# chaitjo/efficient-gnns

Measured on NVIDIA H100. Metric: edges aggregated/s (fwd+bwd), 3-layer GCN student + logit-KD, ARXIV-shape, higher is better.
Workload: dtype f32

## Files before the change

efficient-gnns_b200/csrc/common.cuh:

```cuda
#pragma once
#include <cuda_runtime.h>
#include <stdint.h>

#include "b200gnn.h"

namespace b200gnn {

void set_cuda_error(cudaError_t e);
void count_launch(int n = 1);

inline int check_launch() {
  cudaError_t e = cudaGetLastError();
  if (e != cudaSuccess) {
    set_cuda_error(e);
    return B200GNN_ERR_CUDA;
  }
  count_launch();
  return B200GNN_OK;
}

constexpr unsigned FULL_MASK = 0xffffffffu;

__device__ __forceinline__ void adam_update(float& p, float& m, float& v, float g, float b1, float b2, float eps,
                                            float step_size, float inv_sqrt_bc2) {
  const float mi = b1 * m + (1.f - b1) * g;
  const float vi = b2 * v + (1.f - b2) * g * g;
  m = mi; v = vi;
  p -= step_size * mi / (sqrtf(vi) * inv_sqrt_bc2 + eps);
}

template <typename V> struct VecTraits;
template <> struct VecTraits<float> { static constexpr int W = 1; };
template <> struct VecTraits<float2> { static constexpr int W = 2; };
template <> struct VecTraits<float4> { static constexpr int W = 4; };

__device__ __forceinline__ void vzero(float& a) { a = 0.f; }
__device__ __forceinline__ void vzero(float2& a) { a.x = a.y = 0.f; }
__device__ __forceinline__ void vzero(float4& a) { a.x = a.y = a.z = a.w = 0.f; }

__device__ __forceinline__ void vfma(float& acc, float s, const float& x) { acc = fmaf(s, x, acc); }
__device__ __forceinline__ void vfma(float2& acc, float s, const float2& x) {
  acc.x = fmaf(s, x.x, acc.x); acc.y = fmaf(s, x.y, acc.y);
}
__device__ __forceinline__ void vfma(float4& acc, float s, const float4& x) {
  acc.x = fmaf(s, x.x, acc.x); acc.y = fmaf(s, x.y, acc.y);
  acc.z = fmaf(s, x.z, acc.z); acc.w = fmaf(s, x.w, acc.w);
}
__device__ __forceinline__ void vadd(float& a, const float& b) { a += b; }
__device__ __forceinline__ void vadd(float2& a, const float2& b) { a.x += b.x; a.y += b.y; }
__device__ __forceinline__ void vadd(float4& a, const float4& b) {
  a.x += b.x; a.y += b.y; a.z += b.z; a.w += b.w;
}
__device__ __forceinline__ void vdiv(float& a, float d) { a /= d; }
__device__ __forceinline__ void vdiv(float2& a, float d) { a.x /= d; a.y /= d; }
__device__ __forceinline__ void vdiv(float4& a, float d) { a.x /= d; a.y /= d; a.z /= d; a.w /= d; }
__device__ __forceinline__ void vstat(float& s, float& q, const float& y) { s += y; q = fmaf(y, y, q); }
__device__ __forceinline__ void vstat(float2& s, float2& q, const float2& y) {
  s.x += y.x; s.y += y.y; q.x = fmaf(y.x, y.x, q.x); q.y = fmaf(y.y, y.y, q.y);
}
__device__ __forceinline__ void vstat(float4& s, float4& q, const float4& y) {
  s.x += y.x; s.y += y.y; s.z += y.z; s.w += y.w;
  q.x = fmaf(y.x, y.x, q.x); q.y = fmaf(y.y, y.y, q.y);
  q.z = fmaf(y.z, y.z, q.z); q.w = fmaf(y.w, y.w, q.w);
}

__device__ __forceinline__ float vshfl_down(float v, int d) { return __shfl_down_sync(FULL_MASK, v, d); }
__device__ __forceinline__ float2 vshfl_down(float2 v, int d) {
  return make_float2(__shfl_down_sync(FULL_MASK, v.x, d), __shfl_down_sync(FULL_MASK, v.y, d));
}
__device__ __forceinline__ float4 vshfl_down(float4 v, int d) {
  return make_float4(__shfl_down_sync(FULL_MASK, v.x, d), __shfl_down_sync(FULL_MASK, v.y, d),
                     __shfl_down_sync(FULL_MASK, v.z, d), __shfl_down_sync(FULL_MASK, v.w, d));
}

__device__ __forceinline__ float vldg(const float* p) { return __ldg(p); }
__device__ __forceinline__ float2 vldg(const float2* p) { return __ldg(p); }
__device__ __forceinline__ float4 vldg(const float4* p) { return __ldg(p); }

__device__ __forceinline__ void vstcs(float* p, const float& v) { __stcs(p, v); }
__device__ __forceinline__ void vstcs(float2* p, const float2& v) { __stcs(p, v); }
__device__ __forceinline__ void vstcs(float4* p, const float4& v) { __stcs(p, v); }

static __global__ void __launch_bounds__(256) sum_partials_kernel(const float* __restrict__ partial, int n, double scale,
                                                                  float* __restrict__ out) {
  __shared__ double s[256];
  double a = 0.0;
  for (int i = threadIdx.x; i < n; i += 256) a += (double)partial[i];
  s[threadIdx.x] = a;
  __syncthreads();
  for (int d = 128; d > 0; d >>= 1) {
    if (threadIdx.x < d) s[threadIdx.x] += s[threadIdx.x + d];
    __syncthreads();
  }
  if (threadIdx.x == 0) out[0] = (float)(s[0] * scale);
}

inline bool aligned_to(const void* p, size_t a) { return (reinterpret_cast<uintptr_t>(p) % a) == 0; }

}
```

efficient-gnns_b200/csrc/dense_rows.cu:

```cuda
#include "common.cuh"
#include "philox.cuh"

namespace b200gnn {

constexpr int ROWS_THREADS = 256;

struct RowMap {
  int nvec, rows_per_iter, cv, rg;
  bool active;
};
__device__ __forceinline__ RowMap make_row_map(int K) {
  RowMap m;
  m.nvec = K >> 2;
  m.rows_per_iter = ROWS_THREADS / m.nvec;
  m.rg = threadIdx.x / m.nvec;
  m.cv = threadIdx.x - m.rg * m.nvec;
  m.active = m.rg < m.rows_per_iter;
  return m;
}

__device__ __forceinline__ float4 ld4(const float* p) { return *reinterpret_cast<const float4*>(p); }
__device__ __forceinline__ float4 ld4s(const float* p) { return __ldcs(reinterpret_cast<const float4*>(p)); }
__device__ __forceinline__ void st4(float* p, const float4& v) { *reinterpret_cast<float4*>(p) = v; }

// ... 61 lines not shown
    const double mean = s / (double)n;
    double var = q / (double)n - mean * mean;
    if (var < 0.0) var = 0.0;
    const float invstd = (float)(1.0 / sqrt(var + (double)eps));
    const float sc = gamma[k] * invstd;
    mean_out[k] = (float)mean;
    invstd_out[k] = invstd;
    scale_out[k] = sc;
    shift_out[k] = beta[k] - (float)mean * sc;
    if (running_mean) {
      const double unbiased = n > 1 ? var * (double)n / (double)(n - 1) : var;
      running_mean[k] = (1.f - momentum) * running_mean[k] + momentum * (float)mean;
      running_var[k] = (1.f - momentum) * running_var[k] + momentum * (float)unbiased;
    }
  }
}

__device__ __forceinline__ float4 affine_relu4(float4 y, const float* __restrict__ scale, const float* __restrict__ shift,
                                               int cv, int relu) {
  if (scale) {
    const float4 sc = ld4(scale + 4 * cv), sh = ld4(shift + 4 * cv);
    y.x = fmaf(y.x, sc.x, sh.x); y.y = fmaf(y.y, sc.y, sh.y);
    y.z = fmaf(y.z, sc.z, sh.z); y.w = fmaf(y.w, sc.w, sh.w);
  }
  if (relu) { y.x = fmaxf(y.x, 0.f); y.y = fmaxf(y.y, 0.f); y.z = fmaxf(y.z, 0.f); y.w = fmaxf(y.w, 0.f); }
  return y;
}

template <bool P16>
__global__ void __launch_bounds__(256) affine_relu_dropout_kernel(const float* __restrict__ Y, float* __restrict__ out,
                                                                  int64_t n_vec, int nvec_row,
                                                                  const float* __restrict__ scale,
                                                                  const float* __restrict__ shift, int relu, float p,
                                                                  uint32_t thr16, uint64_t seed, uint64_t offset,
                                                                  const int32_t* __restrict__ step_dev,
                                                                  uint64_t step_mul, uint64_t index_offset) {
  const float inv_keep = p > 0.f ? 1.f / (1.f - p) : 1.f;
  if (step_dev) offset += (uint64_t)(*step_dev) * step_mul;
  const int64_t tid = (int64_t)blockIdx.x * blockDim.x + threadIdx.x, stride = (int64_t)gridDim.x * blockDim.x;
  if (P16) {
    const uint64_t g0 = index_offset, g1 = index_offset + (uint64_t)n_vec;
    for (uint64_t b = (g0 >> 1) + (uint64_t)tid; b < ((g1 + 1) >> 1); b += (uint64_t)stride) {
      const uint4 r = philox4x32(seed, offset, b);
#pragma unroll
      for (int half = 0; half < 2; ++half) {
        const uint64_t g = 2 * b + half;
        if (g < g0 || g >= g1) continue;
        const int64_t i = (int64_t)(g - g0);
        float4 y = affine_relu4(ld4s(Y + 4 * i), scale, shift, (int)(i % nvec_row), relu);
        const uchar4 m = keep16(half ? r.z : r.x, half ? r.w : r.y, thr16);
        y.x = m.x ? y.x * inv_keep : 0.f; y.y = m.y ? y.y * inv_keep : 0.f;
        y.z = m.z ? y.z * inv_keep : 0.f; y.w = m.w ? y.w * inv_keep : 0.f;
        st4(out + 4 * i, y);
      }
    }
  } else {
    for (int64_t i = tid; i < n_vec; i += stride) {
      float4 y = affine_relu4(ld4s(Y + 4 * i), scale, shift, (int)(i % nvec_row), relu);
      if (p > 0.f) {
        const uchar4 m = keep24(philox4x32(seed, offset, (uint64_t)i + index_offset), p);
        y.x = m.x ? y.x * inv_keep : 0.f; y.y = m.y ? y.y * inv_keep : 0.f;
        y.z = m.z ? y.z * inv_keep : 0.f; y.w = m.w ? y.w * inv_keep : 0.f;
      }
      st4(out + 4 * i, y);
    }
  }
}

struct RowScatter {
  float* ptr[16];
  int32_t off[17];
  int32_t n;
  int64_t ld, col;
};
__device__ __forceinline__ float* scatter_row(const RowScatter& sc, int64_t r) {
  int q = 0;
#pragma unroll 1
  while (q + 1 < sc.n && r >= sc.off[q + 1]) ++q;
  return sc.ptr[q] + (size_t)(r - sc.off[q]) * (size_t)sc.ld + sc.col;
}

template <bool P16>
__global__ void __launch_bounds__(256) affine_relu_dropout_mapped_kernel(
    const float* __restrict__ Y, float* __restrict__ out, int64_t n_rows, int nvec_l, const float* __restrict__ scale,
    const float* __restrict__ shift, int relu, float p, uint32_t thr16, uint64_t seed, uint64_t offset,
    const int32_t* __restrict__ step_dev, uint64_t step_mul, const int32_t* __restrict__ rowmap, uint64_t row_offset,
    uint64_t nvec_g, uint64_t cv_off, int paired, const RowScatter sc) {
  const float inv_keep = p > 0.f ? 1.f / (1.f - p) : 1.f;
  if (step_dev) offset += (uint64_t)(*step_dev) * step_mul;
  const int64_t tid = (int64_t)blockIdx.x * blockDim.x + threadIdx.x, stride = (int64_t)gridDim.x * blockDim.x;
  if (P16 && paired) {
    const int half_l = nvec_l >> 1;
    for (int64_t u = tid; u < n_rows * half_l; u += stride) {
      const int64_t r = u / half_l;
      const int cv = (int)(u - r * half_l) * 2;
      const uint64_t gid = rowmap ? (uint64_t)rowmap[r] : (uint64_t)r + row_offset;
      const uint64_t g = gid * nvec_g + cv_off + (uint64_t)cv;
      const uint4 rnd = philox4x32(seed, offset, g >> 1);
#pragma unroll
      for (int half = 0; half < 2; ++half) {
        const int64_t i = r * nvec_l + cv + half;
        float4 y = affine_relu4(ld4s(Y + 4 * i), scale, shift, cv + half, relu);
        const uchar4 m = keep16(half ? rnd.z : rnd.x, half ? rnd.w : rnd.y, thr16);
        y.x = m.x ? y.x * inv_keep : 0.f; y.y = m.y ? y.y * inv_keep : 0.f;
        y.z = m.z ? y.z * inv_keep : 0.f; y.w = m.w ? y.w * inv_keep : 0.f;
        st4(out + 4 * i, y);
        if (sc.n) st4(scatter_row(sc, r) + 4 * (cv + half), y);
      }
    }
    return;
  }
  for (int64_t i = tid; i < n_rows * nvec_l; i += stride) {
    const int64_t r = i / nvec_l;
    const int cv = (int)(i - r * nvec_l);
    float4 y = affine_relu4(ld4s(Y + 4 * i), scale, shift, cv, relu);
    if (p > 0.f) {
      const uint64_t gid = rowmap ? (uint64_t)rowmap[r] : (uint64_t)r + row_offset;
      const uint64_t g = gid * nvec_g + cv_off + (uint64_t)cv;
      uchar4 m;
      if (P16) {
        const uint4 rnd = philox4x32(seed, offset, g >> 1);
        m = keep16((g & 1) ? rnd.z : rnd.x, (g & 1) ? rnd.w : rnd.y, thr16);
      } else {
        m = keep24(philox4x32(seed, offset, g), p);
      }
      y.x = m.x ? y.x * inv_keep : 0.f; y.y = m.y ? y.y * inv_keep : 0.f;
      y.z = m.z ? y.z * inv_keep : 0.f; y.w = m.w ? y.w * inv_keep : 0.f;
    }
    st4(out + 4 * i, y);
    if (sc.n) st4(scatter_row(sc, r) + 4 * cv, y);
  }
}

__global__ void __launch_bounds__(256) dropout_mask_kernel(uint8_t* __restrict__ mask, int64_t n_vec, float p, int p16,
                                                           uint32_t thr16, uint64_t seed, uint64_t offset) {
  for (int64_t i = (int64_t)blockIdx.x * blockDim.x + threadIdx.x; i < n_vec; i += (int64_t)gridDim.x * blockDim.x) {
    uchar4 m;
    if (p16) {
      const uint4 r = philox4x32(seed, offset, (uint64_t)i >> 1);
      m = keep16((i & 1) ? r.z : r.x, (i & 1) ? r.w : r.y, thr16);
    } else {
      m = keep24(philox4x32(seed, offset, (uint64_t)i), p);
    }
    reinterpret_cast<uchar4*>(mask)[i] = m;
  }
}

__global__ void __launch_bounds__(256) dropout_mask_step_kernel(uint8_t* __restrict__ mask, int64_t n_vec, float p, int p16,
                                                                uint32_t thr16, uint64_t seed, uint64_t offset,
                                                                const int32_t* __restrict__ step_dev, uint64_t step_mul) {
  const uint64_t off = offset + (uint64_t)(*step_dev) * step_mul;
  for (int64_t i = (int64_t)blockIdx.x * blockDim.x + threadIdx.x; i < n_vec; i += (int64_t)gridDim.x * blockDim.x) {
    uchar4 m;
    if (p16) {
      const uint4 r = philox4x32(seed, off, (uint64_t)i >> 1);
      m = keep16((i & 1) ? r.z : r.x, (i & 1) ? r.w : r.y, thr16);
    } else {
      m = keep24(philox4x32(seed, off, (uint64_t)i), p);
    }
    reinterpret_cast<uchar4*>(mask)[i] = m;
  }
}

__global__ void __launch_bounds__(256) dropout_bits_kernel(uint32_t* __restrict__ bits, int n_layers, int64_t n_rows, int nvec_row,
                                                           int words, float p, int p16, uint32_t thr16, uint64_t seed,
                                                           uint64_t offset, const int32_t* __restrict__ step_dev,
                                                           uint64_t step_mul) {
  if (step_dev) offset += (uint64_t)(*step_dev) * step_mul;
  const int64_t per_layer = n_rows * words;
  for (int64_t t = (int64_t)blockIdx.x * blockDim.x + threadIdx.x; t < per_layer * n_layers; t += (int64_t)gridDim.x * blockDim.x) {
    const int layer = (int)(t / per_layer);
    const int64_t e = t - layer * per_layer, row = e / words;
    const int w = (int)(e - row * words);
    const uint64_t off = offset + (uint64_t)layer;
    uint32_t out = 0u;
    uint64_t blk = ~0ull;
    uint4 r = make_uint4(0u, 0u, 0u, 0u);
#pragma unroll
    for (int j = 0; j < 8; ++j) {
      const int cv = 8 * w + j;
      if (cv >= nvec_row) break;
      const uint64_t g = (uint64_t)row * nvec_row + cv;
      uchar4 m;
      if (p16) {
        if ((g >> 1) != blk) { blk = g >> 1; r = philox4x32(seed, off, blk); }
        m = keep16((g & 1) ? r.z : r.x, (g & 1) ? r.w : r.y, thr16);
      } else {
        m = keep24(philox4x32(seed, off, g), p);
      }
      out |= ((uint32_t)m.x | ((uint32_t)m.y << 1) | ((uint32_t)m.z << 2) | ((uint32_t)m.w << 3)) << (4 * j);
    }
    bits[t] = out;
  }
}

__global__ void __launch_bounds__(256) affine_relu_bits_kernel(const float* __restrict__ Y, const uint32_t* __restrict__ bits,
                                                               const float* __restrict__ scale, const float* __restrict__ shift,
                                                               float* __restrict__ out, int64_t n_vec, int nvec_row, int words,
                                                               float p) {
  const float inv_keep = p > 0.f ? 1.f / (1.f - p) : 1.f;
  for (int64_t i = (int64_t)blockIdx.x * blockDim.x + threadIdx.x; i < n_vec; i += (int64_t)gridDim.x * blockDim.x) {
    const int64_t row = i / nvec_row;
    const int cv = (int)(i - row * nvec_row);
    float4 y = affine_relu4(ld4(Y + 4 * i), scale, shift, cv, 1);
    const uint32_t b = bits[row * words + (cv >> 3)] >> (4 * (cv & 7));
    y.x = (b & 1u) ? y.x * inv_keep : 0.f; y.y = (b & 2u) ? y.y * inv_keep : 0.f;
    y.z = (b & 4u) ? y.z * inv_keep : 0.f; y.w = (b & 8u) ? y.w * inv_keep : 0.f;
    st4(out + 4 * i, y);
  }
}

__global__ void __launch_bounds__(256) gather_rows_act_kernel(const float* __restrict__ X, int64_t ldx, const int64_t* __restrict__ idx,
                                                              const uint32_t* __restrict__ bits, const float* __restrict__ scale,
                                                              const float* __restrict__ shift, float* __restrict__ out,
                                                              int64_t n_vec, int nvec_row, int words, float p) {
  const float inv_keep = p > 0.f ? 1.f / (1.f - p) : 1.f;
  for (int64_t i = (int64_t)blockIdx.x * blockDim.x + threadIdx.x; i < n_vec; i += (int64_t)gridDim.x * blockDim.x) {
    const int64_t r = i / nvec_row;
    const int cv = (int)(i - r * nvec_row);
    const int64_t row = __ldg(idx + r);
    float4 y = ld4(X + row * ldx + 4 * cv);
    if (bits) {
      y = affine_relu4(y, scale, shift, cv, 1);
      const uint32_t b = bits[row * words + (cv >> 3)] >> (4 * (cv & 7));
      y.x = (b & 1u) ? y.x * inv_keep : 0.f; y.y = (b & 2u) ? y.y * inv_keep : 0.f;
      y.z = (b & 4u) ? y.z * inv_keep : 0.f; y.w = (b & 8u) ? y.w * inv_keep : 0.f;
    }
    st4(out + 4 * i, y);
  }
}

__global__ void __launch_bounds__(256) relu_dropout_bwd_kernel(const float4* __restrict__ dOut, const float4* __restrict__ Xout,
                                                               float4* dY, int64_t n_vec, float inv_keep) {
  for (int64_t i = (int64_t)blockIdx.x * blockDim.x + threadIdx.x; i < n_vec; i += (int64_t)gridDim.x * blockDim.x) {
    const float4 g = dOut[i], x = Xout[i];
    float4 d;
    d.x = x.x > 0.f ? g.x * inv_keep : 0.f; d.y = x.y > 0.f ? g.y * inv_keep : 0.f;
    d.z = x.z > 0.f ? g.z * inv_keep : 0.f; d.w = x.w > 0.f ? g.w * inv_keep : 0.f;
    dY[i] = d;
  }
}

__global__ void __launch_bounds__(ROWS_THREADS) bn_act_bwd_reduce_kernel(
    const float* __restrict__ dOut, const float* __restrict__ Xout, const float* __restrict__ Y,
    const float* __restrict__ mean, const float* __restrict__ invstd, int64_t n_rows, int K, float inv_keep,
    float* __restrict__ partial, int slots) {
  extern __shared__ float smem[];
  const RowMap m = make_row_map(K);
  const int64_t per = (n_rows + slots - 1) / slots;
  const int64_t r0 = (int64_t)blockIdx.x * per, r1 = min(n_rows, r0 + per);
  float4 s = make_float4(0, 0, 0, 0), q = s;
  if (m.active) {
    const float4 mu = ld4(mean + 4 * m.cv), is = ld4(invstd + 4 * m.cv);
    for (int64_t r = r0 + m.rg; r < r1; r += m.rows_per_iter) {
      const size_t o = (size_t)r * K + 4 * m.cv;
      const float4 g = ld4(dOut + o), x = ld4(Xout + o), y = ld4(Y + o);
      const float dx = x.x > 0.f ? g.x * inv_keep : 0.f, dy = x.y > 0.f ? g.y * inv_keep : 0.f;
      const float dz = x.z > 0.f ? g.z * inv_keep : 0.f, dw = x.w > 0.f ? g.w * inv_keep : 0.f;
      s.x += dx; s.y += dy; s.z += dz; s.w += dw;
      q.x = fmaf(dx, (y.x - mu.x) * is.x, q.x); q.y = fmaf(dy, (y.y - mu.y) * is.y, q.y);
      q.z = fmaf(dz, (y.z - mu.z) * is.z, q.z); q.w = fmaf(dw, (y.w - mu.w) * is.w, q.w);
    }
  }
  reduce_store_2xK(m, K, s, q, smem, partial + (size_t)blockIdx.x * 2 * K);
}

__global__ void __launch_bounds__(256) bn_bwd_finalize_kernel(const float* __restrict__ partial, int slots, int K,
                                                              int64_t n, const float* __restrict__ gamma,
                                                              const float* __restrict__ invstd, float* dgamma,
                                                              float* dbeta, float* coef ) {
  double s, q; int k;
  if (finalize_reduce(partial, slots, K, true, s, q, k)) {
    dbeta[k] = (float)s;
    dgamma[k] = (float)q;
    coef[k] = gamma[k] * invstd[k];
    coef[K + k] = (float)(s / (double)n);
    coef[2 * K + k] = (float)(q / (double)n);
  }
}

template <bool DZ>
__global__ void __launch_bounds__(ROWS_THREADS) bn_act_bwd_apply_kernel(
    const float* __restrict__ dOut, const float* __restrict__ Xout, const float* __restrict__ Y,
    const float* __restrict__ mean, const float* __restrict__ invstd, const float* __restrict__ coef, int64_t n_rows,
    int K, float inv_keep, float* __restrict__ dY, float* __restrict__ colsum_partial, int slots) {
  extern __shared__ float smem[];
  const RowMap m = make_row_map(K);
  const int64_t per = (n_rows + slots - 1) / slots;
  const int64_t r0 = (int64_t)blockIdx.x * per, r1 = min(n_rows, r0 + per);
  float4 s = make_float4(0, 0, 0, 0), q = s;
  if (m.active) {
    const float4 mu = ld4(mean + 4 * m.cv), is = ld4(invstd + 4 * m.cv);
    const float4 c1 = ld4(coef + 4 * m.cv), c2 = ld4(coef + K + 4 * m.cv), c3 = ld4(coef + 2 * K + 4 * m.cv);
    for (int64_t r = r0 + m.rg; r < r1; r += m.rows_per_iter) {
      const size_t o = (size_t)r * K + 4 * m.cv;
      float4 g = ld4s(dOut + o);
      const float4 y = ld4s(Y + o);
      if (!DZ) {
        const float4 x = ld4s(Xout + o);
        g.x = x.x > 0.f ? g.x * inv_keep : 0.f; g.y = x.y > 0.f ? g.y * inv_keep : 0.f;
        g.z = x.z > 0.f ? g.z * inv_keep : 0.f; g.w = x.w > 0.f ? g.w * inv_keep : 0.f;
      }
      float4 d;
      d.x = c1.x * (g.x - c2.x - (y.x - mu.x) * is.x * c3.x);
      d.y = c1.y * (g.y - c2.y - (y.y - mu.y) * is.y * c3.y);
      d.z = c1.z * (g.z - c2.z - (y.z - mu.z) * is.z * c3.z);
      d.w = c1.w * (g.w - c2.w - (y.w - mu.w) * is.w * c3.w);
      st4(dY + o, d);
      s.x += d.x; s.y += d.y; s.z += d.z; s.w += d.w;
    }
  }
  if (colsum_partial) reduce_store_2xK(m, K, s, q, smem, colsum_partial + (size_t)blockIdx.x * 2 * K);
}

__global__ void __launch_bounds__(256) partial_reduce_kernel(const float* __restrict__ partial, int slots, int K2,
                                                             float* __restrict__ out) {
  __shared__ double sh[FIN_GROUPS][FIN_COLS];
  const int c = threadIdx.x % FIN_COLS, g = threadIdx.x / FIN_COLS;
  const int k = blockIdx.x * FIN_COLS + c;
  double s = 0.0;
  if (k < K2)
    for (int j = g; j < slots; j += FIN_GROUPS) s += (double)partial[(size_t)j * K2 + k];
  sh[g][c] = s;
  __syncthreads();
  if (g == 0 && k < K2) {
    s = 0.0;
    for (int j = 0; j < FIN_GROUPS; ++j) s += sh[j][c];
    out[k] = (float)s;
  }
}

__global__ void __launch_bounds__(256) colsum_finalize_kernel(const float* __restrict__ partial, int slots, int K,
                                                              float* __restrict__ out) {
  double s, q; int k;
  if (finalize_reduce(partial, slots, K, false, s, q, k)) out[k] = (float)s;
}

__global__ void __launch_bounds__(256) adam_kernel(float* __restrict__ p, const float* __restrict__ g,
                                                   float* __restrict__ m, float* __restrict__ v, int64_t n, float lr,
                                                   float b1, float b2, float eps, const int32_t* __restrict__ step) {
  const float t = (float)(*step + 1);
  const float bc1 = 1.f - powf(b1, t), bc2 = 1.f - powf(b2, t);
  const float step_size = lr / bc1, inv_sqrt_bc2 = rsqrtf(bc2);
  for (int64_t i = (int64_t)blockIdx.x * blockDim.x + threadIdx.x; i < n; i += (int64_t)gridDim.x * blockDim.x)
    adam_update(p[i], m[i], v[i], g[i], b1, b2, eps, step_size, inv_sqrt_bc2);
}
__global__ void adam_tick_kernel(int32_t* step) { *step += 1; }

__global__ void __launch_bounds__(256) rmsprop_kernel(float* __restrict__ p, const float* __restrict__ g, float* __restrict__ sq,
                                                      int64_t n, double lr, int warmup, float alpha, float one_minus_alpha,
                                                      float eps, float wd, const int32_t* __restrict__ step) {
  const int e = *step + 1;
  const float neg_lr = -(float)(warmup > 0 ? lr * (double)(e < warmup ? e : warmup) / (double)warmup : lr);
  for (int64_t i = (int64_t)blockIdx.x * blockDim.x + threadIdx.x; i < n; i += (int64_t)gridDim.x * blockDim.x) {
    const float pi = p[i];
    float gi = g[i];
    if (wd != 0.f) gi = __fadd_rn(gi, __fmul_rn(wd, pi));
    const float s = __fadd_rn(__fmul_rn(sq[i], alpha), __fmul_rn(__fmul_rn(one_minus_alpha, gi), gi));
    sq[i] = s;
    p[i] = __fadd_rn(pi, __fdiv_rn(__fmul_rn(neg_lr, gi), __fadd_rn(__fsqrt_rn(s), eps)));
  }
}

static inline int grid_for(int64_t n_items, int per_cta, int cap = 132 * 8) {
  int64_t g = (n_items + per_cta - 1) / per_cta;
  if (g > cap) g = cap;
  if (g < 1) g = 1;
  return (int)g;
}

}

using namespace b200gnn;

static bool rows_ok(int64_t n_rows, int64_t K) { return n_rows >= 0 && K > 0 && K % 4 == 0 && K <= 1024; }

extern "C" int64_t b200gnn_rows_slots(int64_t n_rows) {
  int64_t s = (n_rows + 255) / 256;
  if (s > 132 * 4) s = 132 * 4;
  return s < 1 ? 1 : s;
}

extern "C" int b200gnn_col_stats_f32(const float* Y, int64_t n_rows, int64_t K, float* partial, int64_t slots,
                                     void* stream) {
  if (!rows_ok(n_rows, K) || !Y || !partial || slots < 1 || !aligned_to(Y, 16)) return B200GNN_ERR_BAD_ARG;
  col_stats4_kernel<<<(int)slots, ROWS_THREADS, 2 * K * sizeof(float), (cudaStream_t)stream>>>(Y, n_rows, (int)K, partial,
                                                                                             (int)slots);
  return check_launch();
}

extern "C" int b200gnn_bn_finalize_f32(const float* partial, int64_t slots, int64_t K, int64_t n_rows,
                                       const float* gamma, const float* beta, float eps, float momentum,
                                       float* running_mean, float* running_var, float* mean_out, float* invstd_out,
                                       float* scale_out, float* shift_out, void* stream) {
  if (!partial || slots < 1 || K <= 0 || n_rows <= 0 || !gamma || !beta || !mean_out || !invstd_out || !scale_out ||
      !shift_out || ((running_mean == nullptr) != (running_var == nullptr)))
    return B200GNN_ERR_BAD_ARG;
  bn_finalize_kernel<<<(int)((K + FIN_COLS - 1) / FIN_COLS), 256, 0, (cudaStream_t)stream>>>(
      partial, (int)slots, (int)K, n_rows, gamma, beta, eps, momentum, running_mean, running_var, mean_out, invstd_out,
      scale_out, shift_out);
  return check_launch();
}

extern "C" int b200gnn_affine_relu_dropout_f32(const float* Y, float* out, int64_t n_rows, int64_t K,
                                               const float* scale, const float* shift, int relu, float p, uint64_t seed,
                                               uint64_t offset, const int32_t* step_dev, uint64_t step_mul,
                                               uint64_t row_offset, void* stream) {
  if (!rows_ok(n_rows, K) || !Y || !out || p < 0.f || p >= 1.f || ((scale == nullptr) != (shift == nullptr)) ||
      !aligned_to(Y, 16) || !aligned_to(out, 16))
    return B200GNN_ERR_BAD_ARG;
  if (n_rows == 0) return B200GNN_OK;
  const int64_t n_vec = n_rows * (K / 4);
  uint32_t thr16 = 0;
  if (dropout_p16(p, thr16))
    affine_relu_dropout_kernel<true><<<grid_for((n_vec + 1) / 2 + 1, 256 * 2), 256, 0, (cudaStream_t)stream>>>(
        Y, out, n_vec, (int)(K / 4), scale, shift, relu, p, thr16, seed, offset, step_dev, step_mul,
        row_offset * (uint64_t)(K / 4));
  else
    affine_relu_dropout_kernel<false><<<grid_for(n_vec, 256 * 4), 256, 0, (cudaStream_t)stream>>>(
        Y, out, n_vec, (int)(K / 4), scale, shift, relu, p, 0u, seed, offset, step_dev, step_mul,
        row_offset * (uint64_t)(K / 4));
  return check_launch();
}

static int mapped_launch(const float* Y, float* out, int64_t n_rows, int64_t K, const float* scale, const float* shift, int relu,
                         float p, uint64_t seed, uint64_t offset, const int32_t* step_dev, uint64_t step_mul, const int32_t* rowmap,
                         uint64_t row_offset, int64_t K_global, int64_t col_offset, const RowScatter& sc, void* stream) {
  if (!rows_ok(n_rows, K) || !Y || !out || p < 0.f || p >= 1.f || ((scale == nullptr) != (shift == nullptr)) ||
      !aligned_to(Y, 16) || !aligned_to(out, 16) || K_global < K || K_global % 4 || col_offset < 0 || col_offset % 4 ||
      col_offset + K > K_global)
    return B200GNN_ERR_BAD_ARG;
  if (n_rows == 0) return B200GNN_OK;
  const int nvec_l = (int)(K / 4);
  const uint64_t nvec_g = (uint64_t)(K_global / 4), cv_off = (uint64_t)(col_offset / 4);
  const int paired = (nvec_l % 2 == 0 && nvec_g % 2 == 0 && cv_off % 2 == 0) ? 1 : 0;
  const int64_t n_vec = n_rows * nvec_l;
  uint32_t thr16 = 0;
  if (dropout_p16(p, thr16))
    affine_relu_dropout_mapped_kernel<true><<<grid_for(paired ? n_vec / 2 : n_vec, 256 * 2), 256, 0, (cudaStream_t)stream>>>(
        Y, out, n_rows, nvec_l, scale, shift, relu, p, thr16, seed, offset, step_dev, step_mul, rowmap, row_offset, nvec_g,
        cv_off, paired, sc);
  else
    affine_relu_dropout_mapped_kernel<false><<<grid_for(n_vec, 256 * 4), 256, 0, (cudaStream_t)stream>>>(
        Y, out, n_rows, nvec_l, scale, shift, relu, p, 0u, seed, offset, step_dev, step_mul, rowmap, row_offset, nvec_g,
        cv_off, 0, sc);
  return check_launch();
}

extern "C" int b200gnn_affine_relu_dropout_mapped_f32(const float* Y, float* out, int64_t n_rows, int64_t K,
                                                      const float* scale, const float* shift, int relu, float p,
                                                      uint64_t seed, uint64_t offset, const int32_t* step_dev,
                                                      uint64_t step_mul, const int32_t* rowmap, uint64_t row_offset,
                                                      int64_t K_global, int64_t col_offset, void* stream) {
  RowScatter sc;
  sc.n = 0; sc.ld = 0; sc.col = 0;
  return mapped_launch(Y, out, n_rows, K, scale, shift, relu, p, seed, offset, step_dev, step_mul, rowmap, row_offset, K_global,
                       col_offset, sc, stream);
}

extern "C" int b200gnn_affine_relu_dropout_scatter_f32(const float* Y, float* out, int64_t n_rows, int64_t K,
                                                       const float* scale, const float* shift, int relu, float p,
                                                       uint64_t seed, uint64_t offset, const int32_t* step_dev,
                                                       uint64_t step_mul, const int32_t* rowmap, uint64_t row_offset,
                                                       int64_t K_global, int64_t col_offset, float* const* dst_ptrs,
                                                       const int32_t* row_off, int32_t world, int64_t ld_dst, void* stream) {
  if (!dst_ptrs || !row_off || world <= 0 || world > 16 || ld_dst < K_global || ld_dst % 4 || row_off[0] != 0 ||
      row_off[world] != n_rows)
    return B200GNN_ERR_BAD_ARG;
  RowScatter sc;
  sc.n = world; sc.ld = ld_dst; sc.col = col_offset;
  for (int q = 0; q < world; ++q) {
    if (!dst_ptrs[q] || !aligned_to(dst_ptrs[q], 16) || row_off[q + 1] < row_off[q]) return B200GNN_ERR_BAD_ARG;
    sc.ptr[q] = dst_ptrs[q]; sc.off[q] = row_off[q];
  }
  sc.off[world] = row_off[world];
  return mapped_launch(Y, out, n_rows, K, scale, shift, relu, p, seed, offset, step_dev, step_mul, rowmap, row_offset, K_global,
                       col_offset, sc, stream);
}

extern "C" int b200gnn_dropout_mask_u8(uint8_t* mask, int64_t n_rows, int64_t K, float p, uint64_t seed,
                                       uint64_t offset, void* stream) {
  if (!rows_ok(n_rows, K) || !mask || p < 0.f || p >= 1.f) return B200GNN_ERR_BAD_ARG;
  if (n_rows == 0) return B200GNN_OK;
  const int64_t n_vec = n_rows * (K / 4);
  uint32_t thr16 = 0;
  const int p16 = dropout_p16(p, thr16) ? 1 : 0;
  dropout_mask_kernel<<<grid_for(n_vec, 256 * 4), 256, 0, (cudaStream_t)stream>>>(mask, n_vec, p, p16, thr16, seed, offset);
  return check_launch();
}

extern "C" int b200gnn_dropout_mask_step_u8(uint8_t* mask, int64_t n_rows, int64_t K, float p, uint64_t seed, uint64_t offset,
                                            const int32_t* step_dev, uint64_t step_mul, void* stream) {
  if (!rows_ok(n_rows, K) || !mask || !step_dev || p < 0.f || p >= 1.f) return B200GNN_ERR_BAD_ARG;
  if (n_rows == 0) return B200GNN_OK;
  const int64_t n_vec = n_rows * (K / 4);
  uint32_t thr16 = 0;
  const int p16 = dropout_p16(p, thr16) ? 1 : 0;
  dropout_mask_step_kernel<<<grid_for(n_vec, 256 * 4), 256, 0, (cudaStream_t)stream>>>(mask, n_vec, p, p16, thr16, seed, offset,
                                                                                      step_dev, step_mul);
  return check_launch();
}

extern "C" int b200gnn_dropout_bits_u32(uint32_t* bits, int64_t n_layers, int64_t n_rows, int64_t K, float p, uint64_t seed,
                                        uint64_t offset, const int32_t* step_dev, uint64_t step_mul, void* stream) {
  if (!rows_ok(n_rows, K) || !bits || n_layers < 1 || p < 0.f || p >= 1.f) return B200GNN_ERR_BAD_ARG;
  if (n_rows == 0) return B200GNN_OK;
  const int words = (int)((K + 31) / 32);
  uint32_t thr16 = 0;
  const int p16 = dropout_p16(p, thr16) ? 1 : 0;
  dropout_bits_kernel<<<grid_for(n_layers * n_rows * words, 256 * 2), 256, 0, (cudaStream_t)stream>>>(
      bits, (int)n_layers, n_rows, (int)(K / 4), words, p, p16, thr16, seed, offset, step_dev, step_mul);
  return check_launch();
}

extern "C" int b200gnn_affine_relu_bits_f32(const float* Y, const uint32_t* bits, const float* scale, const float* shift,
                                            float p, float* out, int64_t n_rows, int64_t K, void* stream) {
  if (!rows_ok(n_rows, K) || !Y || !bits || !scale || !shift || !out || p < 0.f || p >= 1.f || !aligned_to(Y, 16) ||
      !aligned_to(out, 16) || !aligned_to(scale, 16) || !aligned_to(shift, 16))
    return B200GNN_ERR_BAD_ARG;
  if (n_rows == 0) return B200GNN_OK;
  const int64_t n_vec = n_rows * (K / 4);
  affine_relu_bits_kernel<<<grid_for(n_vec, 256 * 4), 256, 0, (cudaStream_t)stream>>>(Y, bits, scale, shift, out, n_vec,
                                                                                     (int)(K / 4), (int)((K + 31) / 32), p);
  return check_launch();
}

extern "C" int b200gnn_gather_rows_act_f32(const float* X, int64_t ldx, const int64_t* idx, int64_t n_idx, int64_t K,
                                            const uint32_t* bits, const float* scale, const float* shift, float p, float* out,
                                            void* stream) {
  if (!rows_ok(n_idx, K) || !X || !idx || !out || ldx < K || ldx % 4 || p < 0.f || p >= 1.f || !aligned_to(X, 16) ||
      !aligned_to(out, 16))
    return B200GNN_ERR_BAD_ARG;
  if (bits && (!scale || !shift || !aligned_to(scale, 16) || !aligned_to(shift, 16))) return B200GNN_ERR_BAD_ARG;
  if (n_idx == 0) return B200GNN_OK;
  const int64_t n_vec = n_idx * (K / 4);
  gather_rows_act_kernel<<<grid_for(n_vec, 256 * 4), 256, 0, (cudaStream_t)stream>>>(X, ldx, idx, bits, scale, shift, out, n_vec,
                                                                                    (int)(K / 4), (int)((K + 31) / 32), p);
  return check_launch();
}

extern "C" int b200gnn_relu_dropout_bwd_f32(const float* dOut, const float* Xout, float* dY, int64_t n_rows, int64_t K,
                                            float p, void* stream) {
  if (!rows_ok(n_rows, K) || p < 0.f || p >= 1.f) return B200GNN_ERR_BAD_ARG;
  if (n_rows == 0) return B200GNN_OK;
  if (!dOut || !Xout || !dY || !aligned_to(dOut, 16) || !aligned_to(Xout, 16) || !aligned_to(dY, 16)) return B200GNN_ERR_BAD_ARG;
  const int64_t n_vec = n_rows * (K / 4);
  const float inv_keep = p > 0.f ? 1.f / (1.f - p) : 1.f;
  relu_dropout_bwd_kernel<<<grid_for(n_vec, 256 * 4), 256, 0, (cudaStream_t)stream>>>(
      reinterpret_cast<const float4*>(dOut), reinterpret_cast<const float4*>(Xout), reinterpret_cast<float4*>(dY), n_vec, inv_keep);
  return check_launch();
}

extern "C" int b200gnn_bn_act_bwd_reduce_f32(const float* dOut, const float* Xout, const float* Y, const float* mean,
                                             const float* invstd, int64_t n_rows, int64_t K, float p, float* partial,
                                             int64_t slots, void* stream) {
  if (!rows_ok(n_rows, K) || n_rows == 0 || !dOut || !Xout || !Y || !mean || !invstd || !partial || slots < 1 ||
      p < 0.f || p >= 1.f)
    return B200GNN_ERR_BAD_ARG;
  if (!aligned_to(dOut, 16) || !aligned_to(Xout, 16) || !aligned_to(Y, 16) || !aligned_to(mean, 16) || !aligned_to(invstd, 16))
    return B200GNN_ERR_BAD_ARG;
  if (ROWS_THREADS / (K / 4) < 1) return B200GNN_ERR_UNSUPPORTED;
  const float inv_keep = p > 0.f ? 1.f / (1.f - p) : 1.f;
  bn_act_bwd_reduce_kernel<<<(int)slots, ROWS_THREADS, 2 * K * sizeof(float), (cudaStream_t)stream>>>(
      dOut, Xout, Y, mean, invstd, n_rows, (int)K, inv_keep, partial, (int)slots);
  return check_launch();
}

extern "C" int b200gnn_bn_act_bwd_apply_f32(const float* dOut, const float* Xout, const float* Y, const float* mean,
                                            const float* invstd, const float* gamma, const float* sums,
                                            int64_t sum_slots, int64_t n_norm, int64_t n_rows, int64_t K, float p,
                                            float* dY, float* dgamma, float* dbeta, float* dbias, float* partial,
                                            int64_t slots, float* coef, void* stream) {
  if (!rows_ok(n_rows, K) || n_rows == 0 || !dOut || !Y || !mean || !invstd || !gamma || !sums || !dY ||
      !dgamma || !dbeta || !partial || !coef || slots < 1 || sum_slots < 1 || n_norm < 1 || p < 0.f || p >= 1.f)
    return B200GNN_ERR_BAD_ARG;
  if (!aligned_to(dOut, 16) || (Xout && !aligned_to(Xout, 16)) || !aligned_to(Y, 16) || !aligned_to(mean, 16) ||
      !aligned_to(invstd, 16) || !aligned_to(coef, 16) || !aligned_to(dY, 16))
    return B200GNN_ERR_BAD_ARG;
  cudaStream_t st = (cudaStream_t)stream;
  const float inv_keep = p > 0.f ? 1.f / (1.f - p) : 1.f;
  const size_t smem = 2 * K * sizeof(float);
  int rc;
  bn_bwd_finalize_kernel<<<(int)((K + FIN_COLS - 1) / FIN_COLS), 256, 0, st>>>(sums, (int)sum_slots, (int)K, n_norm, gamma,
                                                                              invstd, dgamma, dbeta, coef);
  if ((rc = check_launch())) return rc;
  if (Xout)
    bn_act_bwd_apply_kernel<false><<<(int)slots, ROWS_THREADS, smem, st>>>(dOut, Xout, Y, mean, invstd, coef, n_rows, (int)K,
                                                                          inv_keep, dY, dbias ? partial : nullptr, (int)slots);
  else
    bn_act_bwd_apply_kernel<true><<<(int)slots, ROWS_THREADS, smem, st>>>(dOut, nullptr, Y, mean, invstd, coef, n_rows, (int)K,
                                                                         inv_keep, dY, dbias ? partial : nullptr, (int)slots);
  if ((rc = check_launch())) return rc;
  if (dbias) {
    colsum_finalize_kernel<<<(int)((K + FIN_COLS - 1) / FIN_COLS), 256, 0, st>>>(partial, (int)slots, (int)K, dbias);
    if ((rc = check_launch())) return rc;
  }
  return B200GNN_OK;
}

extern "C" int b200gnn_bn_act_bwd_f32(const float* dOut, const float* Xout, const float* Y, const float* mean,
                                      const float* invstd, const float* gamma, int64_t n_rows, int64_t K, float p,
                                      float* dY, float* dgamma, float* dbeta, float* dbias, float* partial,
                                      int64_t slots, float* coef, void* stream) {
  int rc = b200gnn_bn_act_bwd_reduce_f32(dOut, Xout, Y, mean, invstd, n_rows, K, p, partial, slots, stream);
  if (rc) return rc;
  return b200gnn_bn_act_bwd_apply_f32(dOut, Xout, Y, mean, invstd, gamma, partial, slots, n_rows, n_rows, K, p, dY,
                                      dgamma, dbeta, dbias, partial, slots, coef, stream);
}

extern "C" int b200gnn_partial_reduce_f32(const float* partial, int64_t slots, int64_t K2, float* out, void* stream) {
  if (!partial || !out || slots < 1 || K2 < 1) return B200GNN_ERR_BAD_ARG;
  partial_reduce_kernel<<<(int)((K2 + FIN_COLS - 1) / FIN_COLS), 256, 0, (cudaStream_t)stream>>>(partial, (int)slots, (int)K2,
                                                                                               out);
  return check_launch();
}

extern "C" int b200gnn_col_sum_f32(const float* Y, int64_t n_rows, int64_t K, float* out, float* partial,
                                   int64_t slots, void* stream) {
  if (!rows_ok(n_rows, K) || !Y || !out || !partial || slots < 1) return B200GNN_ERR_BAD_ARG;
  cudaStream_t st = (cudaStream_t)stream;
  int rc;
  col_stats4_kernel<<<(int)slots, ROWS_THREADS, 2 * K * sizeof(float), st>>>(Y, n_rows, (int)K, partial, (int)slots);
  if ((rc = check_launch())) return rc;
  colsum_finalize_kernel<<<(int)((K + FIN_COLS - 1) / FIN_COLS), 256, 0, st>>>(partial, (int)slots, (int)K, out);
  return check_launch();
}

extern "C" int b200gnn_adam_step_f32(float* params, const float* grads, float* exp_avg, float* exp_avg_sq, int64_t n,
                                     float lr, float beta1, float beta2, float eps, int32_t* step, void* stream) {
  if (!params || !grads || !exp_avg || !exp_avg_sq || !step || n < 0) return B200GNN_ERR_BAD_ARG;
  cudaStream_t st = (cudaStream_t)stream;
  int rc;
  if (n > 0) {
    adam_kernel<<<grid_for(n, 256), 256, 0, st>>>(params, grads, exp_avg, exp_avg_sq, n, lr, beta1, beta2, eps, step);
    if ((rc = check_launch())) return rc;
  }
  adam_tick_kernel<<<1, 1, 0, st>>>(step);
  return check_launch();
}

extern "C" int b200gnn_rmsprop_step_f32(float* params, const float* grads, float* square_avg, int64_t n, double lr,
                                        int64_t warmup, double alpha, double eps, double weight_decay, int32_t* step,
                                        void* stream) {
  if (!params || !grads || !square_avg || !step || n < 0 || !(lr >= 0.0) || !(alpha >= 0.0) || !(eps >= 0.0) ||
      !(weight_decay >= 0.0) || warmup < 0 || warmup > (1 << 30))
    return B200GNN_ERR_BAD_ARG;
  cudaStream_t st = (cudaStream_t)stream;
  int rc;
  if (n > 0) {
    rmsprop_kernel<<<grid_for(n, 256), 256, 0, st>>>(params, grads, square_avg, n, lr, (int)warmup, (float)alpha,
                                                     (float)(1.0 - alpha), (float)eps, (float)weight_decay, step);
    if ((rc = check_launch())) return rc;
  }
  adam_tick_kernel<<<1, 1, 0, st>>>(step);
  return check_launch();
}
```

efficient-gnns_b200/csrc/gemm_wgrad_tf32x3.cu:

```cuda
#include "common.cuh"
#include "tc_common.cuh"

namespace b200gnn {
namespace wgrad {
using namespace tc;

constexpr int BKN = 32;
constexpr int TM = 128, TN = 128;
constexpr int THREADS = 384;
constexpr int STAGES = 5;
constexpr int X_BOX = 8;
constexpr int RAW_BYTES = BKN * (TM + TN) * 4;
constexpr int OP_BYTES = 128 * BKN * 4;
constexpr int T_BYTES = 2 * OP_BYTES;
constexpr int SS_BYTES = TM / 2 * 16;
constexpr int SMEM_BYTES = STAGES * RAW_BYTES + 2 * T_BYTES + 256 + SS_BYTES + 1024;
constexpr int MAX_RANGES = 132;
constexpr int64_t MAX_PARTIAL_FLOATS = (int64_t)MAX_RANGES * 256 * 256;
constexpr int MAX_KIN = 2048, MAX_NOUT = 512;
static_assert(SMEM_BYTES <= 232448, "shared memory");

struct Params {
  float* partial;
  int32_t Nn, Kin, Kpad, Nout, Npad, num_kb;
  int32_t n_tn, n_ranges;
  const float* act_scale;
  const float* act_shift;
  const uint32_t* act_bits;
  int32_t act_words;
  float inv_keep;
  const float* act_slope;
  int32_t act_ld;
};

template <bool ACT, bool PRELU = false>
__global__ void __launch_bounds__(THREADS, 1)
wgrad_tf32x3_kernel(const __grid_constant__ CUtensorMap tmX, const __grid_constant__ CUtensorMap tmG, const Params p) {
  extern __shared__ uint8_t smem_raw[];
  uint8_t* smem = reinterpret_cast<uint8_t*>((reinterpret_cast<uintptr_t>(smem_raw) + 1023) & ~(uintptr_t)1023);
  uint8_t* tbuf = smem + STAGES * RAW_BYTES;
  uint64_t* full = reinterpret_cast<uint64_t*>(tbuf + 2 * T_BYTES);
  uint64_t* empty = full + STAGES;
  float4* act_ss = reinterpret_cast<float4*>(tbuf + 2 * T_BYTES + 256);

  const int tiles = (p.Kpad / TM) * p.n_tn;
  const int tile = (int)blockIdx.x % tiles, range = (int)blockIdx.x / tiles;
  const int mt = tile / p.n_tn, nt = tile % p.n_tn;
  const int kb0 = (int)((int64_t)p.num_kb * range / p.n_ranges);
  const int kb1 = (int)((int64_t)p.num_kb * (range + 1) / p.n_ranges);

  const int warp = threadIdx.x >> 5, lane = threadIdx.x & 31;
  if (threadIdx.x == 0) {
    for (int s = 0; s < STAGES; ++s) { mbar_init(&full[s], 1); mbar_init(&empty[s], 256); }
    asm volatile("fence.mbarrier_init.release.cluster;" ::: "memory");
  }
  __syncthreads();

  if (warp < 4) {
    regs_dec<40>();
    if (threadIdx.x == 0) {
      int s = 0; uint32_t ph = 0;
      for (int kb = kb0; kb < kb1; ++kb) {
        mbar_wait(&empty[s], ph ^ 1);
        uint8_t* st = smem + s * RAW_BYTES;
        mbar_expect_tx(&full[s], RAW_BYTES);
        for (int j = 0; j < TM / X_BOX; ++j)
          tma_load_2d(&tmX, &full[s], st + j * BKN * X_BOX * 4, mt * TM + j * X_BOX, kb * BKN);
        tma_load_2d(&tmG, &full[s], st + BKN * TM * 4, nt * TN, kb * BKN);
        if (++s == STAGES) { s = 0; ph ^= 1; }
      }
    }
    return;
  }
  regs_inc<232>();

  const int cw = (warp >> 2) - 1;
  const int ct = threadIdx.x - 128;
  const uint32_t xfrag = (8 * cw + 2 * (warp & 3)) * (BKN * X_BOX * 4) + (lane & 3) * (X_BOX * 4) + (lane >> 2) * 4;
  const int pair = cw * 32 + (warp & 3) * 8 + (lane >> 2);
  const int c0 = mt * TM + cw * 64 + (warp & 3) * 16 + (lane >> 2);
  uint32_t wnext = 0u;
  const int bits_ld = PRELU ? p.act_ld : p.act_words;
  auto act_word = [&](int kb) {
    const int node = kb * BKN + lane;
    return node < p.Nn && (c0 >> 5) < p.act_words ? __ldg(p.act_bits + (size_t)node * bits_ld + (c0 >> 5)) : 0u;
  };
  const float slope = PRELU ? __ldg(p.act_slope) : 0.f;
  if (PRELU && kb0 < kb1) wnext = act_word(kb0);
  if (ACT) {
    if (ct < TM / 2) {
      const int c = mt * TM + (ct >> 3) * 16 + (ct & 7);
      float4 v = make_float4(0.f, 0.f, 0.f, 0.f);
      if (c < p.Kin) { v.x = __ldg(p.act_scale + c); v.y = __ldg(p.act_shift + c); }
      if (c + 8 < p.Kin) { v.z = __ldg(p.act_scale + c + 8); v.w = __ldg(p.act_shift + c + 8); }
      act_ss[ct] = v;
    }
    if (kb0 < kb1) wnext = act_word(kb0);
    named_sync(1, 256);
  }
  float acc[64], sum[64];
#pragma unroll
  for (int i = 0; i < 64; ++i) sum[i] = acc[i] = 0.f;
  uint32_t xh0[BKN / 8][4], xl0[BKN / 8][4], xh1[BKN / 8][4], xl1[BKN / 8][4];
  int s = 0; uint32_t ph = 0;
  auto block = [&](int i, uint32_t (&h)[BKN / 8][4], uint32_t (&l)[BKN / 8][4]) {
    uint32_t wcur = 0u;
    if (ACT || PRELU) {
      wcur = wnext;
      if (kb0 + i + 1 < kb1) wnext = act_word(kb0 + i + 1);
    }
    mbar_wait(&full[s], ph);
    float4 ss = make_float4(0.f, 0.f, 0.f, 0.f);
    int l4 = lane & 3;
    if (ACT) {
      ss = act_ss[pair];
      asm volatile("" : "+r"(l4));
    }
    if (PRELU) asm volatile("" : "+r"(l4));
    const uint32_t sraw = smem_u32(smem + s * RAW_BYTES);
    const float* rg = reinterpret_cast<const float*>(smem + s * RAW_BYTES + BKN * TM * 4);
    uint8_t* T = tbuf + (i & 1) * T_BYTES;
#pragma unroll
    for (int u = 0; u < 4; ++u) {
      const int idx = u * 256 + ct;
      const int r = idx & 127, c = idx >> 7;
      const float* src = rg + (4 * c) * 128 + r;
      const uint4 v = make_uint4(__float_as_uint(src[0]), __float_as_uint(src[128]), __float_as_uint(src[256]),
                                 __float_as_uint(src[384]));
      uint4 hv, lv;
      split4(v, hv, lv);
      *reinterpret_cast<uint4*>(T + swz128(r, c)) = hv;
      *reinterpret_cast<uint4*>(T + OP_BYTES + swz128(r, c)) = lv;
    }
#pragma unroll
    for (int k = 0; k < BKN / 8; ++k)
#pragma unroll
      for (int j = 0; j < 4; ++j) {
        uint32_t v = lds32(sraw + xfrag + (j & 1) * (BKN * X_BOX * 4) + (8 * k + 4 * (j >> 1)) * (X_BOX * 4));
        if (ACT) {
          const uint32_t w = __shfl_sync(0xffffffffu, wcur, 8 * k + l4 + 4 * (j >> 1));
          const float y = fmaxf(fmaf(__uint_as_float(v), (j & 1) ? ss.z : ss.x, (j & 1) ? ss.w : ss.y), 0.f) * p.inv_keep;
          v = (w >> ((c0 & 31) + 8 * (j & 1))) & 1u ? __float_as_uint(y) : 0u;
        }
        if (PRELU) {
          const uint32_t w = __shfl_sync(0xffffffffu, wcur, 8 * k + l4 + 4 * (j >> 1));
          const float z = __uint_as_float(v);
          const float y = (z > 0.f ? z : slope * z) * p.inv_keep;
          v = (w >> ((c0 & 31) + 8 * (j & 1))) & 1u ? __float_as_uint(y) : 0u;
        }
        split1(v, h[k][j], l[k][j]);
      }
    asm volatile("fence.proxy.async.shared::cta;" ::: "memory");
    mbar_arrive(&empty[s]);
    if (i > 0) {
      wgmma_wait<0>();
      acc_fence(acc);
#pragma unroll
      for (int j = 0; j < 64; ++j) sum[j] += acc[j];
    }
    named_sync(1, 256);
    reg_fence(h); reg_fence(l);
    wgmma_fence();
    const uint32_t sa = smem_u32(T);
#pragma unroll
    for (int k = 0; k < BKN / 8; ++k) {
      const uint32_t koff = k * 32;
      wgmma_tf32_n128_rs(acc, l[k], make_desc_k128(sa + koff), k != 0);
      wgmma_tf32_n128_rs(acc, h[k], make_desc_k128(sa + OP_BYTES + koff), 1);
    }
#pragma unroll
    for (int k = 0; k < BKN / 8; ++k) wgmma_tf32_n128_rs(acc, h[k], make_desc_k128(sa + k * 32), 1);
    wgmma_commit();
    if (++s == STAGES) { s = 0; ph ^= 1; }
  };
  for (int i = 0; i < kb1 - kb0; i += 2) {
    block(i, xh0, xl0);
    if (i + 1 < kb1 - kb0) block(i + 1, xh1, xl1);
  }
  if (kb1 > kb0) {
    wgmma_wait<0>();
    acc_fence(acc);
#pragma unroll
    for (int j = 0; j < 64; ++j) sum[j] += acc[j];
  }
  float* out = p.partial + (size_t)range * p.Kpad * p.Npad;
  const int row0 = mt * TM + cw * 64 + (warp & 3) * 16 + (lane >> 2);
#pragma unroll
  for (int j = 0; j < 16; ++j) {
    const int col = nt * TN + 8 * j + 2 * (lane & 3);
    if (col < p.Npad) {
      *reinterpret_cast<float2*>(out + (size_t)row0 * p.Npad + col) = make_float2(sum[4 * j], sum[4 * j + 1]);
      *reinterpret_cast<float2*>(out + (size_t)(row0 + 8) * p.Npad + col) = make_float2(sum[4 * j + 2], sum[4 * j + 3]);
    }
  }
}

constexpr int RED_VECS = 32, RED_GROUPS = 8;
__global__ void __launch_bounds__(RED_VECS * RED_GROUPS) wgrad_reduce_kernel(const float4* __restrict__ partial, int n_part,
                                                                             int Kin, int Kpad, int Nout, int Npad,
                                                                             float* __restrict__ out) {
  __shared__ float4 sh[RED_GROUPS][RED_VECS];
  const int64_t n_vec = (int64_t)Kpad * Npad / 4;
  const int v = threadIdx.x % RED_VECS, g = threadIdx.x / RED_VECS;
  const int64_t i = (int64_t)blockIdx.x * RED_VECS + v;
  float4 acc = make_float4(0.f, 0.f, 0.f, 0.f);
  if (i < n_vec)
    for (int c = g; c < n_part; c += RED_GROUPS) {
      const float4 x = __ldcs(partial + (size_t)c * n_vec + i);
      acc.x += x.x; acc.y += x.y; acc.z += x.z; acc.w += x.w;
    }
  sh[g][v] = acc;
  __syncthreads();
  if (g != 0 || i >= n_vec) return;
  const int row = (int)(i / (Npad / 4)), c4 = (int)(i % (Npad / 4)) * 4;
  if (c4 >= Nout || row >= Kin) return;
#pragma unroll
  for (int j = 1; j < RED_GROUPS; ++j) {
    const float4 x = sh[j][v];
    acc.x += x.x; acc.y += x.y; acc.z += x.z; acc.w += x.w;
  }
  *reinterpret_cast<float4*>(out + (size_t)row * Nout + c4) = acc;
}

static bool make_map_rows(CUtensorMap* m, const float* base, int64_t rows, int64_t width, int64_t ld, int box_cols) {
  EncodeTiledFn fn = encode_fn();
  if (!fn) return false;
  cuuint64_t dims[2] = {(cuuint64_t)width, (cuuint64_t)rows};
  cuuint64_t strides[1] = {(cuuint64_t)ld * 4};
  cuuint32_t box[2] = {(cuuint32_t)box_cols, (cuuint32_t)BKN};
  cuuint32_t estr[2] = {1, 1};
  return fn(m, CU_TENSOR_MAP_DATA_TYPE_FLOAT32, 2, const_cast<float*>(base), dims, strides, box, estr,
            CU_TENSOR_MAP_INTERLEAVE_NONE, CU_TENSOR_MAP_SWIZZLE_NONE, CU_TENSOR_MAP_L2_PROMOTION_L2_256B,
            CU_TENSOR_MAP_FLOAT_OOB_FILL_NONE) == CUDA_SUCCESS;
}

static int64_t pad_k(int64_t Kin) { return (Kin + TM - 1) / TM * TM; }
static int64_t pad_n(int64_t Nout) { return (Nout + 31) / 32 * 32; }
static int range_cap(int64_t Kin, int64_t Nout) {
  const int64_t c = MAX_PARTIAL_FLOATS / (pad_k(Kin) * pad_n(Nout));
  return (int)(c > MAX_RANGES ? MAX_RANGES : (c < 1 ? 1 : c));
}

}
}

using namespace b200gnn;

extern "C" int64_t b200gnn_wgrad_workspace_floats(int64_t Kin, int64_t Nout) {
  if (Kin <= 0 || Nout <= 0) return B200GNN_ERR_BAD_ARG;
  if (Kin > wgrad::MAX_KIN || Nout > wgrad::MAX_NOUT) return B200GNN_ERR_UNSUPPORTED;
  return wgrad::range_cap(Kin, Nout) * wgrad::pad_k(Kin) * wgrad::pad_n(Nout);
}

template <bool ACT, bool PRELU = false>
static int wgrad_launch(const float* X, int64_t ldx, const float* G, int64_t ldg, float* dW, int64_t Nn, int64_t Kin, int64_t Nout,
                        float* workspace, const wgrad::Params& act, void* stream) {
  if (!X || !G || !dW || !workspace || Nn <= 0 || Kin <= 0 || Nout <= 0 || ldx < Kin || ldg < Nout || Nn >= INT32_MAX)
    return B200GNN_ERR_BAD_ARG;
  if (Kin % 4 || Kin > wgrad::MAX_KIN || Nout % 4 || Nout > wgrad::MAX_NOUT || ldx % 4 || ldg % 4 || !aligned_to(X, 16) || !aligned_to(G, 16) ||
      !aligned_to(dW, 16) || !aligned_to(workspace, 16))
    return B200GNN_ERR_UNSUPPORTED;
  CUtensorMap tX, tG;
  if (!wgrad::make_map_rows(&tX, X, Nn, Kin, ldx, wgrad::X_BOX) || !wgrad::make_map_rows(&tG, G, Nn, Nout, ldg, wgrad::TN))
    return B200GNN_ERR_UNSUPPORTED;
  int dev = 0, sms = 132;
  cudaGetDevice(&dev);
  static bool attr_set[64] = {};
  if (dev >= 0 && dev < 64 && !attr_set[dev]) {
    cudaError_t e = cudaFuncSetAttribute(wgrad::wgrad_tf32x3_kernel<ACT, PRELU>, cudaFuncAttributeMaxDynamicSharedMemorySize,
                                         wgrad::SMEM_BYTES);
    if (e != cudaSuccess) { set_cuda_error(e); return B200GNN_ERR_CUDA; }
    attr_set[dev] = true;
  }
  cudaDeviceGetAttribute(&sms, cudaDevAttrMultiProcessorCount, dev);
  cudaStream_t st = (cudaStream_t)stream;
  wgrad::Params p = act;
  p.partial = workspace; p.Nn = (int32_t)Nn; p.Kin = (int32_t)Kin; p.Nout = (int32_t)Nout;
  p.Kpad = (int32_t)wgrad::pad_k(Kin);
  p.Npad = (int32_t)wgrad::pad_n(Nout);
  p.num_kb = (int32_t)((Nn + wgrad::BKN - 1) / wgrad::BKN);
  p.n_tn = (p.Npad + wgrad::TN - 1) / wgrad::TN;
  const int tiles = (int)(p.Kpad / wgrad::TM) * p.n_tn;
  int ranges = sms / tiles;
  const int cap = wgrad::range_cap(Kin, Nout);
  if (ranges > cap) ranges = cap;
  if (ranges > p.num_kb) ranges = p.num_kb;
  if (ranges < 1) ranges = 1;
  p.n_ranges = ranges;
  int rc;
  wgrad::wgrad_tf32x3_kernel<ACT, PRELU><<<tiles * ranges, wgrad::THREADS, wgrad::SMEM_BYTES, st>>>(tX, tG, p);
  if ((rc = check_launch())) return rc;
  const int64_t n_vec = (int64_t)p.Kpad * p.Npad / 4;
  wgrad::wgrad_reduce_kernel<<<(int)((n_vec + wgrad::RED_VECS - 1) / wgrad::RED_VECS), wgrad::RED_VECS * wgrad::RED_GROUPS, 0, st>>>(
      reinterpret_cast<const float4*>(workspace), ranges, (int)Kin, p.Kpad, (int)Nout, p.Npad, dW);
  return check_launch();
}

extern "C" int b200gnn_gemm_wgrad_tf32x3_f32(const float* X, int64_t ldx, const float* G, int64_t ldg, float* dW,
                                             int64_t Nn, int64_t Kin, int64_t Nout, float* workspace, void* stream) {
  return wgrad_launch<false>(X, ldx, G, ldg, dW, Nn, Kin, Nout, workspace, wgrad::Params{}, stream);
}

extern "C" int b200gnn_gemm_wgrad_tf32x3_act_f32(const float* Y, int64_t ldx, const float* G, int64_t ldg, float* dW,
                                                 int64_t Nn, int64_t Kin, int64_t Nout, const float* scale, const float* shift,
                                                 const uint32_t* bits, float p_drop, float* workspace, void* stream) {
  if (!scale || !shift || !bits || p_drop < 0.f || p_drop >= 1.f) return B200GNN_ERR_BAD_ARG;
  wgrad::Params act{};
  act.act_scale = scale; act.act_shift = shift; act.act_bits = bits; act.act_words = (int32_t)((Kin + 31) / 32);
  act.inv_keep = p_drop > 0.f ? 1.f / (1.f - p_drop) : 1.f;
  return wgrad_launch<true>(Y, ldx, G, ldg, dW, Nn, Kin, Nout, workspace, act, stream);
}

extern "C" int b200gnn_gemm_wgrad_tf32x3_prelu_f32(const float* Z, int64_t ldz, const float* G, int64_t ldg, float* dW,
                                                   int64_t Nn, int64_t Kin, int64_t Nout, const float* slope,
                                                   const uint32_t* bits, int64_t ldbits, float p_drop, float* workspace,
                                                   void* stream) {
  if (!slope || !bits || ldbits < (Kin + 31) / 32 || ldbits >= INT32_MAX || p_drop < 0.f || p_drop >= 1.f)
    return B200GNN_ERR_BAD_ARG;
  wgrad::Params act{};
  act.act_slope = slope; act.act_bits = bits; act.act_words = (int32_t)((Kin + 31) / 32); act.act_ld = (int32_t)ldbits;
  act.inv_keep = p_drop > 0.f ? 1.f / (1.f - p_drop) : 1.f;
  return wgrad_launch<false, true>(Z, ldz, G, ldg, dW, Nn, Kin, Nout, workspace, act, stream);
}
```

efficient-gnns_b200/engine.py:

```python
from __future__ import annotations

import math
from typing import Dict, List, Optional

import torch

from . import lib, ops
from .sparse import CsrGraph, SparseTensor
from .trainer import FlatParams, FullBatchStudent, one_objective


def gcn_norm(adj: SparseTensor) -> SparseTensor:
    if not adj.has_value():
        adj = adj.fill_value(1.0)
    adj = adj.fill_diag(1.0)
    deg = adj.sum(dim=1)
    dis = deg.pow(-0.5)
    dis.masked_fill_(dis == float("inf"), 0.0)
    row, col, val = adj.coo()
    return adj.set_value(dis[row] * val * dis[col])


def _is_symmetric(adj: SparseTensor) -> bool:
    st = adj.storage
    if st.sparse_sizes()[0] != st.sparse_sizes()[1]:
        return False
    perm = st.csr2csc()
    same = torch.equal(st.col()[perm], st.row()) and torch.equal(st.row()[perm], st.col())
    if same and st.value() is not None:
        same = torch.equal(st.value()[perm], st.value())
    return bool(same)


class GCNStudentTrainer(FullBatchStudent):

    def __init__(self, adj: SparseTensor, dims: List[int], dropout: float = 0.5, lr: float = 0.01, seed: int = 0,
                 alpha: float = 0.9, kd_T: float = 4.0, bn_eps: float = 1e-5, bn_momentum: float = 0.1,
                 aggregate_first: Optional[bool] = None, tensor_core_gemm: bool = True, overlap_wgrad: bool = True,
                 fuse_row_passes: bool = True, fuse_activations: bool = True, _prebuilt_graph: Optional[CsrGraph] = None, _rows_alloc: Optional[int] = None,
                 gcrd=None, lsp=None, gsp=None):
        self.objective = one_objective(gcrd, lsp, gsp)
        assert adj.is_cuda(), "the engine runs on a CUDA device"
        self.device = adj.device
        self.dims, self.L = list(dims), len(dims) - 1
        self.p, self.lr, self.alpha, self.kd_T = float(dropout), float(lr), float(alpha), float(kd_T)
        self.bn_eps, self.bn_momentum = bn_eps, bn_momentum
        self.seed = int(seed)
        self.tc_gemm = bool(tensor_core_gemm) and all(d % 4 == 0 for d in dims)
        for d in dims[1:]:
            assert d % 4 == 0 and d <= 1024, "layer widths must be multiples of 4 (128-bit rows)"
        self.N = adj.size(0)
        self.agg_first = (dims[0] < dims[1] and dims[0] % 4 == 0) if aggregate_first is None else bool(aggregate_first)
        if self.L < 2:
            self.agg_first = False

        if _prebuilt_graph is not None:
            self.G = self.Gt = _prebuilt_graph
            self.N = _prebuilt_graph.n_rows
        else:
            norm = gcn_norm(adj)
            self.G: CsrGraph = norm.storage.engine_csr()
            self.Gt: CsrGraph = self.G if _is_symmetric(norm) else norm.storage.engine_csc("value")
        self.nnz = self.G.nnz

        shapes = []
        for l in range(self.L):
            shapes += [(dims[l], dims[l + 1]), (dims[l + 1],)]
            if l < self.L - 1:
                shapes += [(dims[l + 1],), (dims[l + 1],)]
        dev = self.device
        self.store = FlatParams(shapes, dev).attach(self)
        self.W, self.b, self.gamma, self.beta = [], [], [], []
        self.gW, self.gb, self.ggamma, self.gbeta = [], [], [], []
        views = iter(self.store.views)
        for l in range(self.L):
            (w, gw), (b, gb) = next(views), next(views)
            self.W.append(w); self.gW.append(gw); self.b.append(b); self.gb.append(gb)
            if l < self.L - 1:
                (g, gg), (be, gbe) = next(views), next(views)
                self.gamma.append(g); self.ggamma.append(gg); self.beta.append(be); self.gbeta.append(gbe)
        self.Wt_split = [(torch.empty(dims[l + 1], dims[l], device=dev), torch.empty(dims[l + 1], dims[l], device=dev))
                         for l in range(self.L)]
        self.W_split = [(torch.empty(dims[l], dims[l + 1], device=dev), torch.empty(dims[l], dims[l + 1], device=dev))
                        for l in range(self.L)]
        wg = [ops.wgrad_supported(dims[l], dims[l + 1]) for l in range(self.L)]
        self.wgrad_ws = (torch.empty(max(ops.wgrad_workspace_floats(dims[l], dims[l + 1]) for l in range(self.L) if wg[l]), device=dev)
                         if self.tc_gemm and any(wg) else None)
        self.running_mean = [torch.zeros(d, device=dev) for d in dims[1:-1]]
        self.running_var = [torch.ones(d, device=dev) for d in dims[1:-1]]
        self.reset_parameters(seed)

        N = self.N
        rows_alloc = N if _rows_alloc is None else _rows_alloc
        self._blocks = []

        def buf(k):
            blk = torch.zeros(rows_alloc, k, device=dev)
            self._blocks.append(blk)
            return blk[:N]
        self.H = [buf(dims[l + 1]) for l in range(self.L)]
        self.Y = [buf(dims[l + 1]) for l in range(self.L)]
        self._A = [buf(dims[l + 1]) for l in range(self.L - 1)]
        self.dY = [buf(dims[l + 1]) for l in range(self.L)]
        self.dH = [buf(dims[l + 1]) for l in range(self.L)]
        self.dA = [buf(dims[l + 1]) for l in range(self.L - 1)]
        self.AX = buf(dims[0]) if self.agg_first else None
        slots_spmm = ops.stat_slots(self.G)
        self.stat_part = [torch.empty(slots_spmm, 2, dims[l + 1], device=dev) for l in range(self.L - 1)]
        self.bn = [torch.empty(4, dims[l + 1], device=dev) for l in range(self.L - 1)]
        self.rs = ops.rows_slots(N)
        self.fuse_rows = bool(fuse_row_passes) and self.tc_gemm
        self._gemm_part = {k: torch.empty(ops.gemm_stat_slots(N, k), 2, k, device=dev)
                           for k in set(dims[1:-1]) if self.fuse_rows and ops.gemm_stats_supported(k)}
        hid = dims[1:-1]
        self.fuse_act = (bool(fuse_activations) and self.fuse_rows and self.L >= 2 and len(set(hid)) == 1
                         and ops.gemm_stats_supported(hid[0]) and hid[0] <= 2048
                         and all(ops.wgrad_supported(dims[l], dims[l + 1]) for l in range(1, self.L)))
        self.keep_bits = (torch.zeros(self.L - 1, N, (hid[0] + 31) // 32, dtype=torch.int32, device=dev)
                          if self.fuse_act else None)
        self._act_stale = False
        self._fwd_fused = False
        self._ev_bits = torch.cuda.Event()
        self.kd_part = torch.empty(2 * int(lib.load().b200gnn_kd_partials(N)), device=dev)
        self.overlap_wgrad = overlap_wgrad
        self._side = torch.cuda.Stream(device=dev) if overlap_wgrad else None
        self._ev_fork, self._ev_join = torch.cuda.Event(), torch.cuda.Event()
        self._static: Dict[str, torch.Tensor] = {}
        for k in set(dims[1:]):
            self._part(k); self._coef(k)
        if self.objective is not None:
            self.objective.bind(self)

    def reset_parameters(self, seed: int = 0):
        g = torch.Generator().manual_seed(seed)
        for l in range(self.L):
            fan_in, fan_out = self.dims[l], self.dims[l + 1]
            a = math.sqrt(6.0 / (fan_in + fan_out))
            self.W[l].copy_((torch.rand(fan_in, fan_out, generator=g) * 2 - 1) * a)
            self.b[l].zero_()
        for l in range(self.L - 1):
            self.gamma[l].fill_(1.0); self.beta[l].zero_()
            self.running_mean[l].zero_(); self.running_var[l].fill_(1.0)
        self.exp_avg.zero_(); self.exp_avg_sq.zero_(); self.step_count.zero_()

    def state_dict(self) -> Dict[str, torch.Tensor]:
        sd = {}
        for l in range(self.L):
            sd[f"convs.{l}.weight"] = self.W[l].detach().clone()
            sd[f"convs.{l}.bias"] = self.b[l].detach().clone()
        for l in range(self.L - 1):
            sd[f"bns.{l}.weight"] = self.gamma[l].detach().clone()
            sd[f"bns.{l}.bias"] = self.beta[l].detach().clone()
            sd[f"bns.{l}.running_mean"] = self.running_mean[l].clone()
            sd[f"bns.{l}.running_var"] = self.running_var[l].clone()
        return sd

    def load_state_dict(self, sd: Dict[str, torch.Tensor]):
        for l in range(self.L):
            self.W[l].copy_(sd[f"convs.{l}.weight"]); self.b[l].copy_(sd[f"convs.{l}.bias"])
        for l in range(self.L - 1):
            self.gamma[l].copy_(sd[f"bns.{l}.weight"]); self.beta[l].copy_(sd[f"bns.{l}.bias"])
            if f"bns.{l}.running_mean" in sd:
                self.running_mean[l].copy_(sd[f"bns.{l}.running_mean"]); self.running_var[l].copy_(sd[f"bns.{l}.running_var"])

    @property
    def A(self) -> List[torch.Tensor]:
        if self._act_stale:
            self._act_stale = False
            for l in range(self.L - 1):
                ops.affine_relu_bits(self.Y[l], self.keep_bits[l], self.bn[l][2], self.bn[l][3], self.p, out=self._A[l])
        return self._A

    def _act(self, l: int):
        return self.Y[l], self.bn[l][2], self.bn[l][3], self.keep_bits[l]

    def activation_pattern(self, l: int) -> torch.Tensor:
        return self.A[l] > 0

    def out_feat(self) -> torch.Tensor:
        return self.A[-1]

    def forward(self, x: torch.Tensor, training: bool = True) -> torch.Tensor:
        fused = training and self.fuse_act
        self._act_stale = False
        if fused:
            if self._side is not None:
                self._ev_fork.record(torch.cuda.current_stream())
                self._side.wait_event(self._ev_fork)
                with torch.cuda.stream(self._side):
                    ops.dropout_bits(self.keep_bits, self.p, self.seed, 0, step_dev=self.step_count, step_mul=self.L)
                self._ev_bits.record(self._side)
            else:
                ops.dropout_bits(self.keep_bits, self.p, self.seed, 0, step_dev=self.step_count, step_mul=self.L)
        A = self._A
        inp = x
        for l in range(self.L):
            last = l == self.L - 1
            if l == 0 and self.agg_first:
                ops.spmm_csr(self.G, x, "sum", out=self.AX)
                if training:
                    gp = self._gemm_part.get(self.dims[1])
                    if gp is not None:
                        hi, lo = ops.split_tf32(self.W[0], transpose=True, hi=self.Wt_split[0][0], lo=self.Wt_split[0][1])
                        ops.gemm_tf32x3_stats(self.AX, hi, lo, self.b[0], self.Y[0], gp)
                        part = gp
                    else:
                        self._linear(0, self.AX, self.Y[0], bias=self.b[0])
                        part = ops.col_stats(self.Y[0], partial=self._part(self.dims[1]))
                    ops.bn_finalize(part, self.N, self.gamma[0], self.beta[0], self.bn_eps,
                                    self.bn_momentum, self.running_mean[0], self.running_var[0], out=self.bn[0])
                    if not fused:
                        ops.affine_relu_dropout(self.Y[0], self.bn[0][2], self.bn[0][3], True, self.p, self.seed, 0,
                                                out=A[0], step_dev=self.step_count, step_mul=self.L)
                else:
                    self._linear(0, self.AX, self.Y[0], bias=self.b[0])
                    scale = self.gamma[0] * torch.rsqrt(self.running_var[0] + self.bn_eps)
                    shift = self.beta[0] - self.running_mean[0] * scale
                    ops.affine_relu_dropout(self.Y[0], scale, shift, True, 0.0, out=A[0])
                inp = A[0]
                continue
            if fused and l > 0:
                if l == 1 and self._side is not None:
                    torch.cuda.current_stream().wait_event(self._ev_bits)
                self._linear(l, None, self.H[l], act=self._act(l - 1))
            else:
                self._linear(l, inp, self.H[l])
            if last:
                ops.spmm_csr(self.G, self.H[l], "sum", bias=self.b[l], out=self.Y[l])
            elif training:
                ops.spmm_csr(self.G, self.H[l], "sum", bias=self.b[l], out=self.Y[l], stat_partial=self.stat_part[l])
                ops.bn_finalize(self.stat_part[l], self.N, self.gamma[l], self.beta[l], self.bn_eps, self.bn_momentum,
                                self.running_mean[l], self.running_var[l], out=self.bn[l])
                if not fused:
                    ops.affine_relu_dropout(self.Y[l], self.bn[l][2], self.bn[l][3], True, self.p, self.seed, l,
                                            out=A[l], step_dev=self.step_count, step_mul=self.L)
                inp = A[l]
            else:
                ops.spmm_csr(self.G, self.H[l], "sum", bias=self.b[l], out=self.Y[l])
                scale = self.gamma[l] * torch.rsqrt(self.running_var[l] + self.bn_eps)
                shift = self.beta[l] - self.running_mean[l] * scale
                ops.affine_relu_dropout(self.Y[l], scale, shift, True, 0.0, out=A[l])
                inp = A[l]
        self._act_stale = self._fwd_fused = fused
        return self.Y[-1]

    def backward(self, x: torch.Tensor, d_out_feat: Optional[torch.Tensor] = None):
        fused = self._fwd_fused
        for l in range(self.L - 1, -1, -1):
            act = self._act(l - 1) if fused and l > 0 else None
            inp = x if l == 0 else (None if act else self._A[l - 1])
            if l == self.L - 1:
                ops.col_sum(self.dY[l], out=self.gb[l], partial=self._part(self.dims[l + 1]))
            if l == 0 and self.agg_first:
                self._wgrad_async(0, self.AX, self.dY[0])
                continue
            ops.spmm_csr(self.Gt, self.dY[l], "sum", out=self.dH[l])
            d_prev = self.dA[l - 1] if l > 0 else None
            gp = self._gemm_part.get(self.dims[l]) if l > 0 else None
            if l > 0:
                acc = d_out_feat is not None and l == self.L - 1
                if acc:
                    d_prev = d_out_feat
                if gp is not None:
                    hi, lo = ops.split_tf32(self.W[l], transpose=False, hi=self.W_split[l][0], lo=self.W_split[l][1])
                    if act:
                        ops.gemm_tf32x3_bnbwd_bits(self.dH[l], hi, lo, d_prev, act[3], self.Y[l - 1], self.bn[l - 1][0],
                                                   self.bn[l - 1][1], act[1], act[2], self.p, gp, accumulate=acc)
                    else:
                        ops.gemm_tf32x3_bnbwd(self.dH[l], hi, lo, d_prev, self._A[l - 1], self.Y[l - 1], self.bn[l - 1][0],
                                              self.bn[l - 1][1], self.p, gp, accumulate=acc)
                else:
                    self._linear_dgrad(l, self.dH[l], d_prev, accumulate=acc)
            self._wgrad_async(l, inp, self.dH[l], act=act)
            if l > 0:
                k = self.dims[l]
                part = self._part(k)
                if gp is not None:
                    ops.bn_act_bwd_apply(d_prev, None, self.Y[l - 1], self.bn[l - 1][0], self.bn[l - 1][1], self.gamma[l - 1],
                                         gp, self.N, self.p, self.dY[l - 1], self.ggamma[l - 1], self.gbeta[l - 1],
                                         self.gb[l - 1], part, self._coef(k))
                else:
                    ops.bn_act_bwd(d_prev, self._A[l - 1], self.Y[l - 1], self.bn[l - 1][0], self.bn[l - 1][1],
                                   self.gamma[l - 1], self.p, d_y=self.dY[l - 1], d_gamma=self.ggamma[l - 1],
                                   d_beta=self.gbeta[l - 1], d_bias=self.gb[l - 1], partial=part, coef=self._coef(k))
        self._wgrad_join()

    def _wgrad_async(self, l: int, inp: Optional[torch.Tensor], d_out: torch.Tensor, act=None):
        if self._side is None:
            return self._linear_wgrad(l, inp, d_out, act)
        self._ev_fork.record(torch.cuda.current_stream())
        self._side.wait_event(self._ev_fork)
        with torch.cuda.stream(self._side):
            self._linear_wgrad(l, inp, d_out, act)

    def _wgrad_join(self):
        if self._side is not None:
            self._ev_join.record(self._side)
            torch.cuda.current_stream().wait_event(self._ev_join)

    def _linear(self, l: int, inp: Optional[torch.Tensor], out: torch.Tensor, bias: Optional[torch.Tensor] = None, act=None):
        if act is not None:
            hi, lo = ops.split_tf32(self.W[l], transpose=True, hi=self.Wt_split[l][0], lo=self.Wt_split[l][1])
            ops.gemm_tf32x3_act(*act, self.p, hi, lo, bias=bias, out=out)
        elif self.tc_gemm:
            hi, lo = ops.split_tf32(self.W[l], transpose=True, hi=self.Wt_split[l][0], lo=self.Wt_split[l][1])
            ops.gemm_tf32x3(inp, hi, lo, bias=bias, out=out)
        elif bias is not None:
            torch.addmm(bias, inp, self.W[l], out=out)
        else:
            torch.mm(inp, self.W[l], out=out)

    def _linear_dgrad(self, l: int, d_out: torch.Tensor, d_inp: torch.Tensor, accumulate: bool = False):
        if self.tc_gemm:
            hi, lo = ops.split_tf32(self.W[l], transpose=False, hi=self.W_split[l][0], lo=self.W_split[l][1])
            ops.gemm_tf32x3(d_out, hi, lo, out=d_inp, accumulate=accumulate)
        elif accumulate:
            d_inp.addmm_(d_out, self.W[l].t())
        else:
            torch.mm(d_out, self.W[l].t(), out=d_inp)

    def _linear_wgrad(self, l: int, inp: Optional[torch.Tensor], d_out: torch.Tensor, act=None):
        if act is not None:
            ops.gemm_wgrad_tf32x3_act(*act, self.p, d_out, out=self.gW[l], workspace=self.wgrad_ws)
        elif self.tc_gemm and ops.wgrad_supported(self.dims[l], self.dims[l + 1]):
            ops.gemm_wgrad_tf32x3(inp, d_out, out=self.gW[l], workspace=self.wgrad_ws)
        else:
            torch.mm(inp.t(), d_out, out=self.gW[l])

    def replay(self, key: int = 0) -> torch.Tensor:
        super().replay(key)
        self._act_stale = self.fuse_act
        return self.loss_out

    def aggregations_per_step(self) -> Dict[int, int]:
        out: Dict[int, int] = {}
        for l in range(self.L):
            if l == 0 and self.agg_first:
                out[self.dims[0]] = out.get(self.dims[0], 0) + 1
            else:
                out[self.dims[l + 1]] = out.get(self.dims[l + 1], 0) + 2
        return out

    def spmm_algorithmic_bytes(self) -> Dict[int, int]:
        return {k: 2 * self.N * k * 4 + self.nnz * 8 + (self.N + 1) * 4 for k in set(self.dims)}
```

efficient-gnns_b200/lib.py:

```python
from __future__ import annotations

import ctypes as C
import os
from pathlib import Path

import torch

PKG_DIR = Path(__file__).resolve().parent
LIB_PATH = PKG_DIR / "libb200gnn.so"

OK = 0
REDUCE_SUM = 0
REDUCE_MEAN = 1
LSP_MAX_F = 512
GSP_ROWS_MAX_F = 2048

_i32p = C.c_void_p
_f32p = C.c_void_p
_ptr = C.c_void_p
_i64 = C.c_int64
_i32 = C.c_int32
_int = C.c_int
_f32 = C.c_float
_f64 = C.c_double
_u64 = C.c_uint64

SIGNATURES = {
    "b200gnn_abi_version": (_int, []),
    "b200gnn_error_string": (C.c_char_p, [_int]),
    "b200gnn_last_cuda_error": (C.c_char_p, []),
    "b200gnn_launch_count": (_i64, []),
    "b200gnn_reset_launch_count": (None, []),
    "b200gnn_csr_chunk_count": (_i64, [_i64, _i64, _i32, _i32]),
    "b200gnn_csr_chunk_plan": (_int, [_i32p, _i64, _i64, _i32, _i32, _i32p, _ptr]),
    "b200gnn_csr_hub_count": (_int, [_i32p, _i64, _i32, _i32, _i32p, _ptr]),
    "b200gnn_csr_hub_fill": (_int, [_i32p, _i64, _i32, _i32, _i32p, _i32p, _i64, _ptr]),
    "b200gnn_spmm_stat_slots": (_i64, [_i64, _i64]),
    "b200gnn_spmm_set_variant": (None, [_int]),
    "b200gnn_spmm_csr_f32": (_int, [_i32p, _i32p, _f32p, _f32p, _i64, _f32p, _i64, _i64, _i64, _i64, _int,
                                    _f32p, _f32p, _i32p, _i64, _i32, _i32, _i32p, _i32p, _i64, _i64, _f32p, _ptr]),
    "b200gnn_spmm_csr_scatter_f32": (_int, [_i32p, _i32p, _f32p, _f32p, _i64, _ptr, _ptr, _i32, _i64, _i64, _i64, _i64, _i64, _int,
                                            _f32p, _i32p, _i64, _i32, _i32, _i32p, _i32p, _i64, _i64, _f32p, _ptr]),
    "b200gnn_rows_slots": (_i64, [_i64]),
    "b200gnn_col_stats_f32": (_int, [_f32p, _i64, _i64, _f32p, _i64, _ptr]),
    "b200gnn_col_sum_f32": (_int, [_f32p, _i64, _i64, _f32p, _f32p, _i64, _ptr]),
    "b200gnn_bn_finalize_f32": (_int, [_f32p, _i64, _i64, _i64, _f32p, _f32p, _f32, _f32, _f32p, _f32p,
                                       _f32p, _f32p, _f32p, _f32p, _ptr]),
    "b200gnn_affine_relu_dropout_f32": (_int, [_f32p, _f32p, _i64, _i64, _f32p, _f32p, _int, _f32, _u64, _u64,
                                               _i32p, _u64, _u64, _ptr]),
    "b200gnn_affine_relu_dropout_mapped_f32": (_int, [_f32p, _f32p, _i64, _i64, _f32p, _f32p, _int, _f32, _u64, _u64,
                                                      _i32p, _u64, _i32p, _u64, _i64, _i64, _ptr]),
    "b200gnn_affine_relu_dropout_scatter_f32": (_int, [_f32p, _f32p, _i64, _i64, _f32p, _f32p, _int, _f32, _u64, _u64,
                                                       _i32p, _u64, _i32p, _u64, _i64, _i64, _ptr, _ptr, _i32, _i64, _ptr]),
    "b200gnn_dropout_mask_u8": (_int, [_ptr, _i64, _i64, _f32, _u64, _u64, _ptr]),
    "b200gnn_dropout_mask_step_u8": (_int, [_ptr, _i64, _i64, _f32, _u64, _u64, _i32p, _u64, _ptr]),
    "b200gnn_dropout_bits_u32": (_int, [_ptr, _i64, _i64, _i64, _f32, _u64, _u64, _i32p, _u64, _ptr]),
    "b200gnn_affine_relu_bits_f32": (_int, [_f32p, _ptr, _f32p, _f32p, _f32, _f32p, _i64, _i64, _ptr]),
    "b200gnn_gather_rows_act_f32": (_int, [_f32p, _i64, _ptr, _i64, _i64, _ptr, _f32p, _f32p, _f32, _f32p, _ptr]),
    "b200gnn_relu_dropout_bwd_f32": (_int, [_f32p, _f32p, _f32p, _i64, _i64, _f32, _ptr]),
    "b200gnn_bn_act_bwd_f32": (_int, [_f32p, _f32p, _f32p, _f32p, _f32p, _f32p, _i64, _i64, _f32, _f32p, _f32p,
                                      _f32p, _f32p, _f32p, _i64, _f32p, _ptr]),
    "b200gnn_bn_act_bwd_reduce_f32": (_int, [_f32p, _f32p, _f32p, _f32p, _f32p, _i64, _i64, _f32, _f32p, _i64, _ptr]),
    "b200gnn_bn_act_bwd_apply_f32": (_int, [_f32p, _f32p, _f32p, _f32p, _f32p, _f32p, _f32p, _i64, _i64, _i64, _i64, _f32,
                                            _f32p, _f32p, _f32p, _f32p, _f32p, _i64, _f32p, _ptr]),
    "b200gnn_partial_reduce_f32": (_int, [_f32p, _i64, _i64, _f32p, _ptr]),
    "b200gnn_adam_step_f32": (_int, [_f32p, _f32p, _f32p, _f32p, _i64, _f32, _f32, _f32, _f32, _i32p, _ptr]),
    "b200gnn_rmsprop_step_f32": (_int, [_f32p, _f32p, _f32p, _i64, _f64, _i64, _f64, _f64, _f64, _i32p, _ptr]),
    "b200gnn_teacher_slots": (_i64, [_i64]),
    "b200gnn_label_inputs_f32": (_int, [_f32p, _i64, _i64, _i64, _i64, _i32p, _ptr, _int, _f32, _u64, _u64, _i32p, _u64, _ptr,
                                        _int, _ptr, _i32p, _ptr]),
    "b200gnn_label_softmax_f32": (_int, [_f32p, _i64, _i64, _i64, _ptr, _int, _f32p, _i64, _ptr]),
    "b200gnn_logce_fwd_bwd_f32": (_int, [_f32p, _i64, _i64, _ptr, _i64, _ptr, _ptr, _i32p, _i64, _f32p, _i64, _f32p, _f32p,
                                         _ptr, _ptr]),
    "b200gnn_split_eval_f32": (_int, [_f32p, _i64, _i64, _ptr, _i64, _i64, _i64, _ptr, _f32p, _f32p, _ptr, _ptr]),
    "b200gnn_snapshot_if_better_f32": (_int, [_f32p, _f32p, _f32p, _f32p, _i64, _f32p, _f32p, _i64, _f32p, _f32p, _i64, _ptr]),
    "b200gnn_kd_partials": (_i64, [_i64]),
    "b200gnn_kd_loss_fwd_bwd_f32": (_int, [_f32p, _i64, _ptr, _i64, _ptr, _f32p, _i64, _i64, _f32, _f32, _i64, _f32p,
                                           _i64, _f32p, _f32p, _ptr]),
    "b200gnn_split_tf32_f32": (_int, [_f32p, _i64, _i64, _int, _f32p, _f32p, _ptr]),
    "b200gnn_gemm_tf32x3_f32": (_int, [_f32p, _i64, _f32p, _f32p, _i64, _f32p, _i64, _i64, _i64, _i64, _f32p, _ptr]),
    "b200gnn_random_walk_i64": (_int, [_i32p, _i32p, _i64, _ptr, _i64, _i32, _u64, _u64, _ptr, _ptr]),
    "b200gnn_saint_subgraph_count_i64": (_int, [_i32p, _i32p, _ptr, _i64, _i32p, _ptr, _ptr]),
    "b200gnn_saint_subgraph_fill_i64": (_int, [_i32p, _i32p, _ptr, _ptr, _i64, _i32p, _ptr, _ptr, _ptr, _ptr, _ptr]),
    "b200gnn_gemm_stat_slots": (_i64, [_i64, _i64]),
    "b200gnn_gemm_set_bnbwd_variant": (None, [_int]),
    "b200gnn_gemm_tf32x3_stats_f32": (_int, [_f32p, _i64, _f32p, _f32p, _i64, _f32p, _i64, _i64, _i64, _i64, _f32p, _int, _f32p, _i64,
                                             _ptr]),
    "b200gnn_gemm_tf32x3_bnbwd_f32": (_int, [_f32p, _i64, _f32p, _f32p, _i64, _f32p, _i64, _i64, _i64, _i64, _int,
                                             _f32p, _f32p, _f32p, _f32p, _f32, _f32p, _i64, _ptr]),
    "b200gnn_gemm_tf32x3_bnbwd_bits_f32": (_int, [_f32p, _i64, _f32p, _f32p, _i64, _f32p, _i64, _i64, _i64, _i64, _int,
                                                  _ptr, _f32p, _f32p, _f32p, _f32p, _f32p, _f32, _f32p, _i64, _ptr]),
    "b200gnn_gemm_tf32x3_act_f32": (_int, [_f32p, _i64, _f32p, _f32p, _i64, _f32p, _i64, _i64, _i64, _i64, _f32p,
                                           _f32p, _f32p, _ptr, _f32, _ptr]),
    "b200gnn_gemm_tf32x3_acc_f32": (_int, [_f32p, _i64, _f32p, _f32p, _i64, _f32p, _i64, _i64, _i64, _i64, _ptr]),
    "b200gnn_gemm_tf32x3_rowidx_f32": (_int, [_f32p, _i64, _f32p, _f32p, _i64, _f32p, _i64, _i64, _i64, _i64, _ptr, _ptr]),
    "b200gnn_gemm_tf32x3_scatter_f32": (_int, [_f32p, _i64, _f32p, _f32p, _i64, _ptr, _i32, _i64, _i64, _i64, _i64, _f32p, _ptr]),
    "b200gnn_gemm_tf32x3_bcast_f32": (_int, [_f32p, _i64, _f32p, _f32p, _i64, _ptr, _i32, _i64, _i64, _i64, _i64, _i64, _f32p, _ptr]),
    "b200gnn_wgrad_workspace_floats": (_i64, [_i64, _i64]),
    "b200gnn_gemm_wgrad_tf32x3_f32": (_int, [_f32p, _i64, _f32p, _i64, _f32p, _i64, _i64, _i64, _f32p, _ptr]),
    "b200gnn_gemm_wgrad_tf32x3_act_f32": (_int, [_f32p, _i64, _f32p, _i64, _f32p, _i64, _i64, _i64, _f32p, _f32p, _ptr, _f32,
                                                 _f32p, _ptr]),
    "b200gnn_gemm_tf32x3_prelu_f32": (_int, [_f32p, _i64, _f32p, _f32p, _i64, _f32p, _i64, _i64, _i64, _i64, _f32p,
                                             _f32p, _ptr, _f32, _ptr]),
    "b200gnn_gemm_tf32x3_prelu_bwd_f32": (_int, [_f32p, _i64, _f32p, _f32p, _i64, _f32p, _i64, _i64, _i64, _i64, _int,
                                                 _f32p, _ptr, _f32p, _f32, _f32p, _int, _ptr, _i64, _ptr]),
    "b200gnn_gemm_wgrad_tf32x3_prelu_f32": (_int, [_f32p, _i64, _f32p, _i64, _f32p, _i64, _i64, _i64, _f32p, _ptr, _i64, _f32,
                                                   _f32p, _ptr]),
    "b200gnn_prelu_bits_f32": (_int, [_f32p, _i64, _ptr, _i64, _f32p, _f32, _f32p, _i64, _i64, _i64, _ptr]),
    "b200gnn_sign_gather_f32": (_int, [_ptr, _i32, _i64, _i64, _ptr, _i64, _f32, _u64, _u64, _i32p, _u64, _f32p, _ptr, _ptr,
                                       _f32p, _i64, _i64, _f32p, _ptr]),
    "b200gnn_col_sum_ld_slots": (_i64, [_i64]),
    "b200gnn_col_sum_ld_f32": (_int, [_f32p, _i64, _i64, _i64, _f32p, _f32p, _i64, _ptr]),
    "b200gnn_row_normalize_fwd_f32": (_int, [_f32p, _i64, _i64, _f32, _f32, _f32p, _f32p, _ptr]),
    "b200gnn_row_normalize_bwd_f32": (_int, [_f32p, _f32p, _f32p, _i64, _i64, _f32, _f32, _f32p, _int, _ptr]),
    "b200gnn_reduce_slots": (_i64, [_i64]),
    "b200gnn_mse_fwd_bwd_f32": (_int, [_f32p, _f32p, _i64, _f32, _f32p, _f32p, _f32p, _ptr]),
    "b200gnn_bce_logits_fwd_bwd_f32": (_int, [_f32p, _f32p, _int, _i64, _f32, _f32p, _f32p, _f32p, _ptr]),
    "b200gnn_row_sqnorm_f32": (_int, [_f32p, _i64, _i64, _f32p, _ptr]),
    "b200gnn_row_sqnorm_bwd_f32": (_int, [_f32p, _f32p, _i64, _i64, _f32p, _ptr]),
    "b200gnn_nce_rows_f32": (_int, [_f32p, _i64, _f32p, _f32p, _ptr]),
    "b200gnn_nce_rows_chunk_f32": (_int, [_f32p, _i64, _i64, _i64, _i64, _f32p, _ptr]),
    "b200gnn_nce_finish_f32": (_int, [_f32p, _i64, _f32p, _ptr]),
    "b200gnn_gcrd_sample_workspace_bytes": (_i64, [_i64]),
    "b200gnn_gcrd_sample_i32": (_int, [_i64, _u64, _u64, _i32p, _i32p, _ptr, _ptr]),
    "b200gnn_gcrd_operands_f32": (_int, [_i32p, _i64, _i64, _f32p, _f32p, _f32p, _f32p, _f32, _f32, _f32p, _f32p, _f32p, _f32p,
                                         _ptr]),
    "b200gnn_gcrd_bwd_slots": (_i64, []),
    "b200gnn_gcrd_backward_f32": (_int, [_i32p, _i64, _i64, _f32p, _f32p, _f32p, _f32p, _f32p, _f32p, _f32, _f32, _f32p, _f32p,
                                         _f32p, _f32p, _f32, _f32p, _f32p, _f32p, _f32p, _f32p, _f32p, _ptr]),
    "b200gnn_transpose_f32": (_int, [_f32p, _i64, _i64, _f32p, _ptr]),
    "b200gnn_gsp_pair_f32": (_int, [_f32p, _f32p, _f32p, _f32p, _i64, _int, _f32p, _f32p, _f32p, _ptr]),
    "b200gnn_gsp_pair_chunk_f32": (_int, [_f32p, _f32p, _i64, _i64, _i64, _i64, _f32p, _f32p, _int, _f32p, _f32p, _f32p, _ptr]),
    "b200gnn_gsp_finish_f32": (_int, [_f32p, _i64, _f32p, _ptr]),
    "b200gnn_gsp_operands_f32": (_int, [_i32p, _i64, _i64, _int, _f32p, _f32p, _f32p, _f32p, _f32, _f32p, _f32p, _f32p, _f32p,
                                        _ptr]),
    "b200gnn_gsp_backward_f32": (_int, [_i32p, _i64, _i64, _int, _f32p, _f32p, _f32p, _f32p, _f32p, _f32p, _f32p, _f32p, _f32,
                                        _f32p, _f32p, _f32p, _f32p, _f32, _f32p, _f32p, _f32p, _f32p, _f32p, _f32p, _ptr]),
    "b200gnn_row_axpy_f32": (_int, [_f32p, _f32p, _i64, _i64, _f32, _f32p, _ptr]),
    "b200gnn_gsp_sim_chunk_f32": (_int, [_f32p, _i64, _i64, _i64, _i64, _f32p, _int, _f32p, _i64, _ptr]),
    "b200gnn_gsp_pair_fixed_chunk_f32": (_int, [_f32p, _i64, _i64, _i64, _i64, _f32p, _f32p, _i64, _i64, _i32p, _int, _f32p,
                                                _f32p, _ptr]),
    "b200gnn_gsp_rows_operands_f32": (_int, [_f32p, _i64, _i32p, _i64, _i64, _int, _f32, _f32p, _i64, _f32p, _ptr]),
    "b200gnn_gsp_rows_backward_f32": (_int, [_i32p, _i64, _i64, _int, _f32p, _f32p, _i64, _f32p, _f32p, _f32, _f32, _f32p, _i64,
                                             _f32p, _f32p, _ptr]),
    "b200gnn_edge_sim_f32": (_int, [_f32p, _i64, _i32p, _i32p, _i64, _int, _f32p, _ptr]),
    "b200gnn_lsp_partials": (_i64, [_i64]),
    "b200gnn_lsp_segment_f32": (_int, [_f32p, _f32p, _i32p, _i64, _i64, _int, _f32p, _f32p, _f32p, _ptr]),
    "b200gnn_edge_sim_bwd_f32": (_int, [_f32p, _i64, _i32p, _i32p, _i64, _int, _f32p, _f32p, _f32p, _ptr]),
    "b200gnn_lsp_bwd_values_f32": (_int, [_f32p, _i64, _i32p, _i32p, _i64, _int, _f32p, _f32p, _i32p, _i32p, _i32p, _i32p, _i64,
                                          _f32p, _f32p, _ptr]),
    "b200gnn_lsp_student_f32": (_int, [_f32p, _i64, _i32p, _i32p, _i32p, _i64, _i64, _f32p, _int, _i32p, _i32p, _i32p, _i32p,
                                       _i64, _f32p, _f32p, _f32p, _f32p, _f32p, _f32p, _ptr]),
    "b200gnn_scatter_rows_scaled_f32": (_int, [_f32p, _ptr, _i64, _i64, _f32, _f32p, _i64, _f32p, _f32p, _ptr]),
    "b200gnn_gat_edge_softmax_f32": (_int, [_i32p, _i32p, _f32p, _f32p, _i64, _i64, _f32, _f32, _f32p, _ptr, _ptr]),
    "b200gnn_gat_aggregate_f32": (_int, [_i32p, _i32p, _i32p, _f32p, _f32p, _i64, _f32p, _i64, _i64, _i64, _i64, _i32p, _i64,
                                         _i32, _i32, _i32p, _i32p, _i64, _i64, _f32p, _ptr]),
    "b200gnn_gat_bwd_rows_f32": (_int, [_i32p, _i32p, _f32p, _f32p, _i64, _f32p, _i64, _f32p, _f32p, _i64, _i64, _i64, _f32,
                                        _f32p, _f32p, _i32p, _i64, _i32, _i32, _i32p, _i32p, _i64, _i64, _f32p, _f32p, _ptr]),
    "b200gnn_segment_sum_heads_f32": (_int, [_i32p, _i32p, _f32p, _i64, _i64, _f32p, _ptr]),
    "b200gnn_gat_scores_f32": (_int, [_f32p, _i64, _f32p, _f32p, _f32p, _i64, _i64, _i64, _f32p, _f32p, _ptr]),
    "b200gnn_gat_scores_slots": (_i64, [_i64]),
    "b200gnn_gat_scores_bwd_f32": (_int, [_f32p, _i64, _f32p, _f32p, _f32p, _f32p, _f32p, _i64, _i64, _i64, _f32p, _i64,
                                          _f32p, _f32p, _f32p, _i64, _ptr]),
    "b200gnn_gat_stat_slots": (_i64, [_i64, _i64]),
    "b200gnn_gat_aggregate_epi_f32": (_int, [_i32p, _i32p, _i32p, _f32p, _f32p, _i64, _f32p, _i64, _i64, _i64, _i64,
                                             _f32p, _f32p, _f32p, _i64, _f32p, _f32p, _i64, _i32p, _i64, _i32, _i32,
                                             _i32p, _i32p, _i64, _i64, _f32p, _ptr]),
    "b200gnn_gat_aggregate_elu_f32": (_int, [_i32p, _i32p, _i32p, _f32p, _f32p, _i64, _f32p, _i64, _f32p, _i64, _i64, _i64,
                                             _i64, _f32p, _i64, _f32p, _i32p, _i64, _i32, _i32, _i32p, _i32p, _i64, _i64,
                                             _f32p, _ptr]),
    "b200gnn_elu_bwd_f32": (_int, [_f32p, _i64, _f32p, _i64, _f32p, _i64, _i64, _i64, _ptr]),
    "b200gnn_ppi_tail_slots": (_i64, [_i64]),
    "b200gnn_ppi_logits_loss_f32": (_int, [_f32p, _i64, _f32p, _i64, _f32p, _f32p, _i64, _i64, _i64, _i64, _f32p, _i64, _f32p,
                                           _i64, _f32p, _i64, _f32, _f32, _f32p, _i64, _f32p, _i64, _f32p, _ptr, _i64, _ptr]),
    "b200gnn_graph_sort_workspace_bytes": (_i64, [_i64]),
    "b200gnn_graph_argsort_i64": (_int, [_ptr, _ptr, _i64, _i64, _i64, _i32p, _ptr, _ptr]),
    "b200gnn_graph_coalesce_i64": (_int, [_ptr, _ptr, _i64, _i64, _i64, _ptr, _ptr, _i32p, _ptr, _ptr, _ptr, _ptr]),
    "b200gnn_typed_gather_f32": (_int, [_ptr, _ptr, _i32, _ptr, _ptr, _i64, _i64, _f32p, _i64, _i32p, _ptr]),
    "b200gnn_typed_scatter_f32": (_int, [_f32p, _i64, _ptr, _ptr, _ptr, _i64, _i64, _ptr, _ptr, _i32, _ptr]),
    "b200gnn_embedding_adam_f32": (_int, [_f32p, _i64, _ptr, _ptr, _ptr, _i64, _i64, _f32p, _f32p, _f32p, _i64, _i64, _i32p,
                                          _f32, _f32, _f32, _f32, _i32p, _ptr]),
    "b200gnn_arena_alloc": (_int, [_i64, C.POINTER(C.c_void_p)]),
    "b200gnn_arena_free": (_int, [_ptr]),
    "b200gnn_ipc_get_handle": (_int, [_ptr, _ptr]),
    "b200gnn_ipc_open_handle": (_int, [_ptr, C.POINTER(C.c_void_p)]),
    "b200gnn_ipc_close_handle": (_int, [_ptr]),
    "b200gnn_peer_copy2d_f32": (_int, [_ptr, _i32, _i64, _ptr]),
    "b200gnn_peer_barrier": (_int, [_ptr, _i32, _i32, _ptr, _ptr, _ptr]),
    "b200gnn_peer_exchange_f32": (_int, [_ptr, _i32, _i64, _ptr, _i32, _i32, _ptr, _ptr, _ptr, _ptr]),
}


class Copy2D(C.Structure):
    _fields_ = [("dst", C.c_void_p), ("src", C.c_void_p), ("ld_dst", C.c_int64), ("ld_src", C.c_int64), ("rows", C.c_int64)]

_lib = None


class B200GnnError(RuntimeError):
    pass


def load() -> C.CDLL:
    global _lib
    if _lib is not None:
        return _lib
    if not LIB_PATH.exists():
        raise B200GnnError(
            f"{LIB_PATH} is missing: build it with `python -c 'import __graft_entry__ as g; g.build()'` "
            "(nvcc, sm_90a). There is no CPU or PyTorch fallback for the b200gnn operators.")
    lib = C.CDLL(str(LIB_PATH))
    for name, (res, args) in SIGNATURES.items():
        fn = getattr(lib, name)
        fn.restype = res
        fn.argtypes = args
    if lib.b200gnn_abi_version() != 2:
        raise B200GnnError("libb200gnn.so ABI version mismatch; rebuild")
    _lib = lib
    report = os.environ.get("B200GNN_LAUNCH_REPORT")
    if report:
        import atexit
        atexit.register(lambda: Path(report).write_text(str(int(lib.b200gnn_launch_count()))))
    return lib


def check(rc: int, what: str) -> None:
    if rc != OK:
        lib = load()
        msg = lib.b200gnn_error_string(rc).decode()
        if rc == -3:
            msg += ": " + lib.b200gnn_last_cuda_error().decode()
        raise B200GnnError(f"{what} failed: {msg}")


def stream_ptr() -> int:
    return torch.cuda.current_stream().cuda_stream


def dptr(t: torch.Tensor | None, dtype: torch.dtype, name: str) -> int | None:
    if t is None:
        return None
    if not isinstance(t, torch.Tensor):
        raise TypeError(f"{name}: expected a tensor")
    if not t.is_cuda:
        raise B200GnnError(f"{name}: b200gnn operators need CUDA tensors (got {t.device}); there is no CPU fallback")
    if t.dtype != dtype:
        raise B200GnnError(f"{name}: expected dtype {dtype}, got {t.dtype}")
    if not t.is_contiguous():
        raise B200GnnError(f"{name}: tensor must be contiguous")
    return t.data_ptr()


def launch_count() -> int:
    return int(load().b200gnn_launch_count())


def reset_launch_count() -> None:
    load().b200gnn_reset_launch_count()
```

efficient-gnns_b200/ops.py:

```python
from __future__ import annotations

from typing import Optional, Tuple

import torch

from . import lib
from .sparse import CsrGraph, SparseTensor

_REDUCE = {"sum": lib.REDUCE_SUM, "add": lib.REDUCE_SUM, "mean": lib.REDUCE_MEAN}


def set_spmm_variant(variant: int) -> None:
    lib.load().b200gnn_spmm_set_variant(int(variant))


def stat_slots(g: CsrGraph) -> int:
    return int(lib.load().b200gnn_spmm_stat_slots(g.n_chunks, g.n_hub))


def spmm_csr(g: CsrGraph, x: torch.Tensor, reduce: str = "sum", bias: Optional[torch.Tensor] = None,
             out: Optional[torch.Tensor] = None, stat_partial: Optional[torch.Tensor] = None) -> torch.Tensor:
    if reduce not in _REDUCE:
        raise ValueError(f"reduce={reduce!r}: the engine implements sum/add/mean (what the reference path uses)")
    if x.dim() != 2:
# ... 149 lines not shown
    n, K = y.shape
    lib.check(lib.load().b200gnn_affine_relu_dropout_scatter_f32(
        _f32(y, "y"), _f32(out, "out"), n, K, _f32(scale, "scale"), _f32(shift, "shift"), int(relu), p, seed, offset,
        lib.dptr(step_dev, torch.int32, "step_dev"), step_mul, lib.dptr(rowmap, torch.int32, "rowmap"), 0, k_global, col_offset,
        _host_ptr_array(dst_ptrs), _host_i32_array(row_off), len(dst_ptrs), int(ld_dst), lib.stream_ptr()),
        "affine_relu_dropout_scatter_f32")
    return out


def dropout_mask(n_rows: int, K: int, p: float, seed: int, offset: int, device="cuda") -> torch.Tensor:
    mask = torch.empty(n_rows, K, dtype=torch.uint8, device=device)
    lib.check(lib.load().b200gnn_dropout_mask_u8(mask.data_ptr(), n_rows, K, p, seed, offset, lib.stream_ptr()),
              "dropout_mask_u8")
    return mask


def dropout_bits(bits: torch.Tensor, p: float, seed: int, offset: int, step_dev: Optional[torch.Tensor] = None,
                 step_mul: int = 0, K: Optional[int] = None) -> torch.Tensor:
    n_layers, n, words = bits.shape
    K = 32 * words if K is None else K
    assert bits.dtype == torch.int32 and bits.is_contiguous() and words == (K + 31) // 32
    lib.check(lib.load().b200gnn_dropout_bits_u32(bits.data_ptr(), n_layers, n, K, p, seed, offset,
                                                  lib.dptr(step_dev, torch.int32, "step_dev"), step_mul, lib.stream_ptr()),
              "dropout_bits_u32")
    return bits


def _bits(bits: torch.Tensor, n: int, K: int) -> int:
    if bits.dtype != torch.int32 or not bits.is_cuda or not bits.is_contiguous() or tuple(bits.shape) != (n, (K + 31) // 32):
        raise lib.B200GnnError(f"keep bits: expected a contiguous CUDA int32 [{n}, {(K + 31) // 32}] tensor")
    return bits.data_ptr()


def affine_relu_bits(y: torch.Tensor, bits: torch.Tensor, scale: torch.Tensor, shift: torch.Tensor, p: float,
                     out: Optional[torch.Tensor] = None) -> torch.Tensor:
    n, K = y.shape
    if out is None:
        out = torch.empty_like(y)
    lib.check(lib.load().b200gnn_affine_relu_bits_f32(_f32(y, "y"), _bits(bits, n, K), _f32(scale, "scale"), _f32(shift, "shift"),
                                                      p, _f32(out, "out"), n, K, lib.stream_ptr()), "affine_relu_bits_f32")
    return out


def gather_rows_act(x: torch.Tensor, idx: torch.Tensor, out: torch.Tensor, bits: Optional[torch.Tensor] = None,
                    scale: Optional[torch.Tensor] = None, shift: Optional[torch.Tensor] = None, p: float = 0.0) -> torch.Tensor:
    n, K = out.shape
    assert x.shape[1] == K and idx.numel() == n
    lib.check(lib.load().b200gnn_gather_rows_act_f32(
        _f32(x, "x"), x.stride(0), lib.dptr(idx, torch.int64, "idx"),
        n, K, None if bits is None else _bits(bits, x.shape[0], K), _f32(scale, "scale"), _f32(shift, "shift"), float(p),
        _f32(out, "out"), lib.stream_ptr()), "gather_rows_act_f32")
    return out


def lsp_student(feat: torch.Tensor, src: torch.Tensor, dst: torch.Tensor, rowptr: torch.Tensor, sim_t: torch.Tensor, kernel: int,
                pos_dst: torch.Tensor, pos_src: torch.Tensor, comb_rowptr: torch.Tensor, diag_pos: torch.Tensor,
                sim_s: torch.Tensor, scratch: torch.Tensor, val: torch.Tensor, selfc: torch.Tensor, loss: torch.Tensor,
                partial: torch.Tensor) -> None:
    E, n_seg, n_nodes = src.numel(), rowptr.numel() - 1, comb_rowptr.numel() - 1
    assert dst.numel() == E and sim_t.numel() == E and sim_s.numel() == E and scratch.numel() >= 2 * E
    assert pos_dst.numel() == E and pos_src.numel() == E and diag_pos.numel() == n_nodes and feat.shape[0] >= n_nodes
    assert val.numel() == selfc.numel() == 2 * E + n_nodes and partial.numel() >= int(lib.load().b200gnn_lsp_partials(n_seg))
    i32 = lambda t, name: lib.dptr(t, torch.int32, name)
    lib.check(lib.load().b200gnn_lsp_student_f32(
        _f32(feat, "feat"), feat.shape[1], i32(src, "src"), i32(dst, "dst"), i32(rowptr, "rowptr"), n_seg, E,
        _f32(sim_t, "sim_t"), int(kernel), i32(pos_dst, "pos_dst"), i32(pos_src, "pos_src"), i32(comb_rowptr, "comb_rowptr"),
        i32(diag_pos, "diag_pos"), n_nodes, _f32(sim_s, "sim_s"), _f32(scratch, "scratch"), _f32(val, "val"),
        _f32(selfc, "selfc"), _f32(loss, "loss"), _f32(partial, "partial"), lib.stream_ptr()), "lsp_student_f32")


def scatter_rows_scaled(src: torch.Tensor, idx: torch.Tensor, scale: float, out: torch.Tensor,
                        loss_aux: Optional[torch.Tensor] = None, loss_total: Optional[torch.Tensor] = None) -> torch.Tensor:
    n, K = src.shape
    assert idx.numel() == n and out.dim() == 2 and out.shape[1] == K and out.stride(1) == 1
    if out.dtype != torch.float32 or not out.is_cuda:
        raise lib.B200GnnError("scatter_rows_scaled: out must be a float32 CUDA tensor")
    lib.check(lib.load().b200gnn_scatter_rows_scaled_f32(
        _f32(src, "src"), lib.dptr(idx, torch.int64, "idx"), n, K, float(scale), out.data_ptr(), out.stride(0),
        _f32(loss_aux, "loss_aux"), _f32(loss_total, "loss_total"), lib.stream_ptr()), "scatter_rows_scaled_f32")
    return out


def bn_act_bwd(d_out, x_out, y, mean, invstd, gamma, p: float, d_y=None, d_gamma=None, d_beta=None, d_bias=None,
               partial=None, coef=None, want_dbias: bool = True):
    n, K = y.shape
    dev = y.device
    slots = rows_slots(n)
    d_y = torch.empty_like(y) if d_y is None else d_y
    d_gamma = torch.empty(K, device=dev) if d_gamma is None else d_gamma
    d_beta = torch.empty(K, device=dev) if d_beta is None else d_beta
    if want_dbias and d_bias is None:
        d_bias = torch.empty(K, device=dev)
    partial = torch.empty(slots, 2, K, device=dev) if partial is None else partial
    coef = torch.empty(3, K, device=dev) if coef is None else coef
    lib.check(lib.load().b200gnn_bn_act_bwd_f32(
        _f32(d_out, "d_out"), _f32(x_out, "x_out"), _f32(y, "y"), _f32(mean, "mean"), _f32(invstd, "invstd"),
        _f32(gamma, "gamma"), n, K, p, _f32(d_y, "d_y"), _f32(d_gamma, "d_gamma"), _f32(d_beta, "d_beta"),
        _f32(d_bias, "d_bias") if want_dbias else None, _f32(partial, "partial"), slots, _f32(coef, "coef"),
        lib.stream_ptr()), "bn_act_bwd_f32")
    return d_y, d_gamma, d_beta, d_bias


def adam_step(params, grads, exp_avg, exp_avg_sq, step: torch.Tensor, lr: float, betas=(0.9, 0.999), eps: float = 1e-8):
    lib.check(lib.load().b200gnn_adam_step_f32(
        _f32(params, "params"), _f32(grads, "grads"), _f32(exp_avg, "exp_avg"), _f32(exp_avg_sq, "exp_avg_sq"),
        params.numel(), lr, betas[0], betas[1], eps, lib.dptr(step, torch.int32, "step"), lib.stream_ptr()),
        "adam_step_f32")


def kd_loss_fwd_bwd(logits, labels, train_idx, teacher_logits=None, alpha: float = 0.9, T: float = 4.0,
                    d_logits=None, loss_out=None, partial=None, n_norm: int = 0):
    N, C = logits.shape
    n_train = train_idx.numel() if train_idx is not None else N
    L = lib.load()
    if d_logits is None:
        d_logits = torch.zeros_like(logits)
    if loss_out is None:
        loss_out = torch.empty(3, dtype=torch.float32, device=logits.device)
    if partial is None:
        partial = torch.empty(2 * int(L.b200gnn_kd_partials(max(n_train, 1))), dtype=torch.float32, device=logits.device)
    lib.check(L.b200gnn_kd_loss_fwd_bwd_f32(
        _f32(logits, "logits"), logits.stride(0), lib.dptr(train_idx, torch.int64, "train_idx"), n_train,
        lib.dptr(labels, torch.int64, "labels"), _f32(teacher_logits, "teacher_logits"),
        teacher_logits.stride(0) if teacher_logits is not None else 0, C, alpha, T, n_norm, _f32(d_logits, "d_logits"),
        d_logits.stride(0), _f32(loss_out, "loss_out"), _f32(partial, "partial"), lib.stream_ptr()), "kd_loss_fwd_bwd_f32")
    return loss_out, d_logits


def split_tf32(w: torch.Tensor, transpose: bool = False, hi: Optional[torch.Tensor] = None,
               lo: Optional[torch.Tensor] = None) -> Tuple[torch.Tensor, torch.Tensor]:
    rows, cols = w.shape
    shape = (cols, rows) if transpose else (rows, cols)
    hi = torch.empty(shape, dtype=torch.float32, device=w.device) if hi is None else hi
    lo = torch.empty(shape, dtype=torch.float32, device=w.device) if lo is None else lo
    lib.check(lib.load().b200gnn_split_tf32_f32(_f32(w, "w"), rows, cols, int(transpose), _f32(hi, "hi"), _f32(lo, "lo"),
                                                lib.stream_ptr()), "split_tf32_f32")
    return hi, lo


def gemm_tf32x3(a: torch.Tensor, b_hi: torch.Tensor, b_lo: torch.Tensor, bias: Optional[torch.Tensor] = None,
                out: Optional[torch.Tensor] = None, accumulate: bool = False) -> torch.Tensor:
    M, K = a.shape
    N = b_hi.shape[0]
    assert b_hi.shape == b_lo.shape and b_hi.shape[1] == K
    if out is None:
        assert not accumulate
        out = torch.empty(M, N, dtype=torch.float32, device=a.device)
    L = lib.load()
    if accumulate:
        assert bias is None
        lib.check(L.b200gnn_gemm_tf32x3_acc_f32(_f32(a, "a"), a.stride(0), _f32(b_hi, "b_hi"), _f32(b_lo, "b_lo"),
                                                b_hi.stride(0), _f32(out, "out"), out.stride(0), M, N, K, lib.stream_ptr()),
                  "gemm_tf32x3_acc_f32")
        return out
    lib.check(L.b200gnn_gemm_tf32x3_f32(_f32(a, "a"), a.stride(0), _f32(b_hi, "b_hi"), _f32(b_lo, "b_lo"),
                                        b_hi.stride(0), _f32(out, "out"), out.stride(0), M, N, K,
                                        _f32(bias, "bias"), lib.stream_ptr()), "gemm_tf32x3_f32")
    return out


def gemm_stat_slots(m: int, n: int) -> int:
    return int(lib.load().b200gnn_gemm_stat_slots(m, n))


def gemm_stats_supported(n: int) -> bool:
    return n % 32 == 0 and 48 < n <= 256


def gemm_tf32x3_stats(a: torch.Tensor, b_hi: torch.Tensor, b_lo: torch.Tensor, bias: Optional[torch.Tensor], out: torch.Tensor,
                      partial: torch.Tensor, accumulate: bool = False) -> torch.Tensor:
    M, K = a.shape
    N = b_hi.shape[0]
    lib.check(lib.load().b200gnn_gemm_tf32x3_stats_f32(_f32(a, "a"), a.stride(0), _f32(b_hi, "b_hi"), _f32(b_lo, "b_lo"),
                                                       b_hi.stride(0), _f32(out, "out"), out.stride(0), M, N, K, _f32(bias, "bias"),
                                                       int(accumulate), _f32(partial, "partial"), partial.shape[0], lib.stream_ptr()),
              "gemm_tf32x3_stats_f32")
    return out


def gemm_tf32x3_bnbwd(a: torch.Tensor, b_hi: torch.Tensor, b_lo: torch.Tensor, out: torch.Tensor, x_out: torch.Tensor,
                      y: torch.Tensor, mean: torch.Tensor, invstd: torch.Tensor, p: float, partial: torch.Tensor,
                      accumulate: bool = False) -> torch.Tensor:
    M, K = a.shape
    N = b_hi.shape[0]
    assert out.shape == x_out.shape == y.shape and out.stride(0) == x_out.stride(0) == y.stride(0)
    lib.check(lib.load().b200gnn_gemm_tf32x3_bnbwd_f32(_f32(a, "a"), a.stride(0), _f32(b_hi, "b_hi"), _f32(b_lo, "b_lo"),
                                                       b_hi.stride(0), _f32(out, "out"), out.stride(0), M, N, K, int(accumulate),
                                                       _f32(x_out, "x_out"), _f32(y, "y"), _f32(mean, "mean"),
                                                       _f32(invstd, "invstd"), float(p), _f32(partial, "partial"),
                                                       partial.shape[0], lib.stream_ptr()), "gemm_tf32x3_bnbwd_f32")
    return out


def gemm_tf32x3_bnbwd_bits(a: torch.Tensor, b_hi: torch.Tensor, b_lo: torch.Tensor, out: torch.Tensor, bits: torch.Tensor,
                           y: torch.Tensor, mean: torch.Tensor, invstd: torch.Tensor, scale: torch.Tensor, shift: torch.Tensor,
                           p: float, partial: torch.Tensor, accumulate: bool = False) -> torch.Tensor:
    M, K = a.shape
    N = b_hi.shape[0]
    assert out.shape == y.shape and out.stride(0) == y.stride(0)
    lib.check(lib.load().b200gnn_gemm_tf32x3_bnbwd_bits_f32(_f32(a, "a"), a.stride(0), _f32(b_hi, "b_hi"), _f32(b_lo, "b_lo"),
                                                            b_hi.stride(0), _f32(out, "out"), out.stride(0), M, N, K, int(accumulate),
                                                            _bits(bits, M, N), _f32(y, "y"), _f32(mean, "mean"), _f32(invstd, "invstd"),
                                                            _f32(scale, "scale"), _f32(shift, "shift"), float(p),
                                                            _f32(partial, "partial"), partial.shape[0], lib.stream_ptr()),
              "gemm_tf32x3_bnbwd_bits_f32")
    return out


def gemm_tf32x3_act(y: torch.Tensor, scale: torch.Tensor, shift: torch.Tensor, bits: torch.Tensor, p: float, b_hi: torch.Tensor,
                    b_lo: torch.Tensor, bias: Optional[torch.Tensor] = None, out: Optional[torch.Tensor] = None) -> torch.Tensor:
    M, K = y.shape
    N = b_hi.shape[0]
    assert b_hi.shape == b_lo.shape and b_hi.shape[1] == K
    if out is None:
        out = torch.empty(M, N, dtype=torch.float32, device=y.device)
    lib.check(lib.load().b200gnn_gemm_tf32x3_act_f32(_f32(y, "y"), y.stride(0), _f32(b_hi, "b_hi"), _f32(b_lo, "b_lo"),
                                                     b_hi.stride(0), _f32(out, "out"), out.stride(0), M, N, K, _f32(bias, "bias"),
                                                     _f32(scale, "scale"), _f32(shift, "shift"), _bits(bits, M, K), float(p),
                                                     lib.stream_ptr()), "gemm_tf32x3_act_f32")
    return out


def gemm_tf32x3_rowidx(a: torch.Tensor, b_hi: torch.Tensor, b_lo: torch.Tensor, out: torch.Tensor,
                       row_idx: torch.Tensor) -> torch.Tensor:
    M, K = a.shape
    N = b_hi.shape[0]
    assert b_hi.shape == b_lo.shape and b_hi.shape[1] == K and row_idx.numel() == M and out.shape[1] == N
    lib.check(lib.load().b200gnn_gemm_tf32x3_rowidx_f32(_f32(a, "a"), a.stride(0), _f32(b_hi, "b_hi"), _f32(b_lo, "b_lo"),
                                                        b_hi.stride(0), _f32(out, "out"), out.stride(0), M, N, K,
                                                        lib.dptr(row_idx, torch.int64, "row_idx"), lib.stream_ptr()),
              "gemm_tf32x3_rowidx_f32")
    return out


def gemm_tf32x3_scatter(a: torch.Tensor, b_hi: torch.Tensor, b_lo: torch.Tensor, dst_ptrs, row_off: int,
                        bias: Optional[torch.Tensor] = None) -> None:
    import ctypes as C
    M, K = a.shape
    N = b_hi.shape[0]
    world = len(dst_ptrs)
    arr = (C.c_void_p * world)(*[C.c_void_p(int(p)) for p in dst_ptrs])
    lib.check(lib.load().b200gnn_gemm_tf32x3_scatter_f32(_f32(a, "a"), a.stride(0), _f32(b_hi, "b_hi"), _f32(b_lo, "b_lo"),
                                                         b_hi.stride(0), arr, world, int(row_off), M, N, K, _f32(bias, "bias"),
                                                         lib.stream_ptr()), "gemm_tf32x3_scatter_f32")


def gemm_tf32x3_bcast(a: torch.Tensor, b_hi: torch.Tensor, b_lo: torch.Tensor, dst_ptrs, row_off: int, ldc: int,
                      bias: Optional[torch.Tensor] = None) -> None:
    M, K = a.shape
    N = b_hi.shape[0]
    lib.check(lib.load().b200gnn_gemm_tf32x3_bcast_f32(_f32(a, "a"), a.stride(0), _f32(b_hi, "b_hi"), _f32(b_lo, "b_lo"),
                                                       b_hi.stride(0), _host_ptr_array(dst_ptrs), len(dst_ptrs), int(row_off), int(ldc),
                                                       M, N, K, _f32(bias, "bias"), lib.stream_ptr()), "gemm_tf32x3_bcast_f32")


def wgrad_supported(k_in: int, n_out: int) -> bool:
    return k_in in (128, 256) and n_out % 4 == 0 and 0 < n_out <= 256


def wgrad_workspace_floats(k_in: int, n_out: int) -> int:
    return int(lib.load().b200gnn_wgrad_workspace_floats(k_in, n_out))


def gemm_wgrad_tf32x3(x: torch.Tensor, g: torch.Tensor, out: Optional[torch.Tensor] = None,
                      workspace: Optional[torch.Tensor] = None, wide: bool = False) -> torch.Tensor:
    nn_, k_in = x.shape
    n_out = g.shape[1]
    assert g.shape[0] == nn_
    if not wide and not wgrad_supported(k_in, n_out):
        raise lib.B200GnnError(f"gemm_wgrad_tf32x3: Kin={k_in}, Nout={n_out} is outside the 128/256-row tilings "
                               "(pass wide=True for the padded ones)")
    L = lib.load()
    if out is None:
        out = torch.empty(k_in, n_out, dtype=torch.float32, device=x.device)
    if workspace is None:
        n_ws = int(L.b200gnn_wgrad_workspace_floats(k_in, n_out))
        if n_ws < 0:
            lib.check(n_ws, "wgrad_workspace_floats")
        workspace = torch.empty(n_ws, dtype=torch.float32, device=x.device)
    lib.check(L.b200gnn_gemm_wgrad_tf32x3_f32(_f32(x, "x"), x.stride(0), _f32(g, "g"), g.stride(0), _f32(out, "out"), nn_,
                                              k_in, n_out, _f32(workspace, "workspace"), lib.stream_ptr()),
              "gemm_wgrad_tf32x3_f32")
    return out


def gemm_wgrad_tf32x3_act(y: torch.Tensor, scale: torch.Tensor, shift: torch.Tensor, bits: torch.Tensor, p: float,
                          g: torch.Tensor, out: Optional[torch.Tensor] = None,
                          workspace: Optional[torch.Tensor] = None) -> torch.Tensor:
    nn_, k_in = y.shape
    n_out = g.shape[1]
    assert g.shape[0] == nn_
    if not wgrad_supported(k_in, n_out):
        raise lib.B200GnnError(f"gemm_wgrad_tf32x3_act: Kin={k_in}, Nout={n_out} is outside the 128/256-row tilings")
    L = lib.load()
    if out is None:
        out = torch.empty(k_in, n_out, dtype=torch.float32, device=y.device)
    if workspace is None:
        workspace = torch.empty(int(L.b200gnn_wgrad_workspace_floats(k_in, n_out)), dtype=torch.float32, device=y.device)
    lib.check(L.b200gnn_gemm_wgrad_tf32x3_act_f32(_f32(y, "y"), y.stride(0), _f32(g, "g"), g.stride(0), _f32(out, "out"), nn_,
                                                  k_in, n_out, _f32(scale, "scale"), _f32(shift, "shift"), _bits(bits, nn_, k_in),
                                                  float(p), _f32(workspace, "workspace"), lib.stream_ptr()),
              "gemm_wgrad_tf32x3_act_f32")
    return out


def partial_reduce(partial: torch.Tensor, out: Optional[torch.Tensor] = None) -> torch.Tensor:
    slots = partial.shape[0]
    k2 = partial.numel() // slots
    if out is None:
        out = torch.empty(partial.shape[1:], dtype=torch.float32, device=partial.device)
    lib.check(lib.load().b200gnn_partial_reduce_f32(_f32(partial, "partial"), slots, k2, _f32(out, "out"), lib.stream_ptr()),
              "partial_reduce_f32")
    return out


def bn_act_bwd_reduce(d_out, x_out, y, mean, invstd, p: float, partial: torch.Tensor) -> torch.Tensor:
    n, K = y.shape
    lib.check(lib.load().b200gnn_bn_act_bwd_reduce_f32(_f32(d_out, "d_out"), _f32(x_out, "x_out"), _f32(y, "y"),
                                                       _f32(mean, "mean"), _f32(invstd, "invstd"), n, K, p,
                                                       _f32(partial, "partial"), partial.shape[0], lib.stream_ptr()),
              "bn_act_bwd_reduce_f32")
    return partial


def bn_act_bwd_apply(d_out, x_out, y, mean, invstd, gamma, sums, n_norm: int, p: float, d_y, d_gamma, d_beta, d_bias,
                     partial, coef):
    n, K = y.shape
    sum_slots = sums.numel() // (2 * K)
    lib.check(lib.load().b200gnn_bn_act_bwd_apply_f32(
        _f32(d_out, "d_out"), _f32(x_out, "x_out"), _f32(y, "y"), _f32(mean, "mean"), _f32(invstd, "invstd"),
        _f32(gamma, "gamma"), _f32(sums, "sums"), sum_slots, n_norm, n, K, p, _f32(d_y, "d_y"), _f32(d_gamma, "d_gamma"),
        _f32(d_beta, "d_beta"), _f32(d_bias, "d_bias"), _f32(partial, "partial"), partial.shape[0], _f32(coef, "coef"),
        lib.stream_ptr()), "bn_act_bwd_apply_f32")


def relu_dropout_bwd(d_out: torch.Tensor, x_out: torch.Tensor, p: float, out: Optional[torch.Tensor] = None) -> torch.Tensor:
    n, K = x_out.shape
    assert d_out.shape == x_out.shape and d_out.is_contiguous() and x_out.is_contiguous()
    out = torch.empty_like(x_out) if out is None else out
    lib.check(lib.load().b200gnn_relu_dropout_bwd_f32(_f32(d_out, "d_out"), _f32(x_out, "x_out"), _f32(out, "out"), n, K, float(p),
                                                      lib.stream_ptr()), "relu_dropout_bwd_f32")
    return out


def _table_arrays(tables: dict, n_tables: int):
    import ctypes as C
    ptrs = (C.c_void_p * n_tables)()
    rows = (C.c_int64 * n_tables)()
    for k, t in tables.items():
        ptrs[k], rows[k] = t.data_ptr(), t.shape[0]
    return ptrs, rows


def typed_gather(tables: dict, n_tables: int, node_type: torch.Tensor, local_idx: torch.Tensor, out: torch.Tensor) -> torch.Tensor:
    ptrs, rows = _table_arrays(tables, n_tables)
    err = torch.zeros(1, dtype=torch.int32, device=out.device)
    lib.check(lib.load().b200gnn_typed_gather_f32(ptrs, rows, n_tables, lib.dptr(node_type, torch.int64, "node_type"),
                                                  lib.dptr(local_idx, torch.int64, "local_idx"), out.shape[0], out.shape[1],
                                                  _f32(out, "out"), out.stride(0), err.data_ptr(), lib.stream_ptr()),
              "typed_gather_f32")
    return out


def typed_scatter(d_out: torch.Tensor, node_type: torch.Tensor, local_idx: torch.Tensor, order: torch.Tensor, grads: dict,
                  n_tables: int) -> None:
    ptrs, rows = _table_arrays(grads, n_tables)
    lib.check(lib.load().b200gnn_typed_scatter_f32(_f32(d_out, "d_out"), d_out.stride(0), lib.dptr(node_type, torch.int64, "node_type"),
                                                   lib.dptr(local_idx, torch.int64, "local_idx"), lib.dptr(order, torch.int64, "order"),
                                                   d_out.shape[0], d_out.shape[1], ptrs, rows, n_tables, lib.stream_ptr()),
              "typed_scatter_f32")


def embedding_adam(d_out: torch.Tensor, node_type: torch.Tensor, local_idx: torch.Tensor, order: torch.Tensor, table_type: int,
                   table: torch.Tensor, exp_avg: torch.Tensor, exp_avg_sq: torch.Tensor, head: torch.Tensor, step: torch.Tensor,
                   lr: float, betas=(0.9, 0.999), eps: float = 1e-8) -> None:
    rows, F_ = table.shape
    assert exp_avg.shape == table.shape == exp_avg_sq.shape and head.numel() >= rows and d_out.shape[1] == F_
    lib.check(lib.load().b200gnn_embedding_adam_f32(
        _f32(d_out, "d_out"), d_out.stride(0), lib.dptr(node_type, torch.int64, "node_type"),
        lib.dptr(local_idx, torch.int64, "local_idx"), lib.dptr(order, torch.int64, "order"), d_out.shape[0], int(table_type),
        _f32(table, "table"), _f32(exp_avg, "exp_avg"), _f32(exp_avg_sq, "exp_avg_sq"), rows, F_,
        lib.dptr(head, torch.int32, "head"), lr, betas[0], betas[1], eps, lib.dptr(step, torch.int32, "step"), lib.stream_ptr()),
        "embedding_adam_f32")


def _rows(t: torch.Tensor, name: str):
    if not isinstance(t, torch.Tensor) or not t.is_cuda or t.dtype != torch.float32 or t.dim() != 2 or t.stride(1) != 1:
        raise lib.B200GnnError(f"{name}: expected a CUDA float32 matrix with contiguous rows")
    return t.data_ptr(), t.stride(0)


def _bits_rows(bits: torch.Tensor, n: int, K: int):
    if bits.dtype != torch.int32 or not bits.is_cuda or bits.dim() != 2 or bits.stride(1) != 1 or bits.shape[0] != n \
            or bits.shape[1] < (K + 31) // 32:
        raise lib.B200GnnError(f"keep bits: expected CUDA int32 [{n}, >= {(K + 31) // 32}] with contiguous rows")
    return bits.data_ptr(), bits.stride(0)


def prelu_bits(z: torch.Tensor, bits: torch.Tensor, slope: torch.Tensor, p: float, out: Optional[torch.Tensor] = None) -> torch.Tensor:
    n, K = z.shape
    if out is None:
        out = torch.empty(n, K, dtype=torch.float32, device=z.device)
    zp, ldz = _rows(z, "z")
    op, ldo = _rows(out, "out")
    bp, ldb = _bits_rows(bits, n, K)
    lib.check(lib.load().b200gnn_prelu_bits_f32(zp, ldz, bp, ldb, _f32(slope, "slope"), float(p), op, ldo, n, K, lib.stream_ptr()),
              "prelu_bits_f32")
    return out


def gemm_tf32x3_prelu(z: torch.Tensor, slope: torch.Tensor, bits: torch.Tensor, p: float, b_hi: torch.Tensor, b_lo: torch.Tensor,
                      bias: Optional[torch.Tensor] = None, out: Optional[torch.Tensor] = None) -> torch.Tensor:
    M, K = z.shape
    N = b_hi.shape[0]
    assert b_hi.shape == b_lo.shape and b_hi.shape[1] == K
    if out is None:
        out = torch.empty(M, N, dtype=torch.float32, device=z.device)
    zp, lda = _rows(z, "z")
    op, ldc = _rows(out, "out")
    if bits.shape[1] != (K + 31) // 32:
        raise lib.B200GnnError("gemm_tf32x3_prelu: keep bits must be [M, ceil(K/32)]")
    lib.check(lib.load().b200gnn_gemm_tf32x3_prelu_f32(zp, lda, _f32(b_hi, "b_hi"), _f32(b_lo, "b_lo"), b_hi.stride(0), op, ldc, M, N, K,
                                                       _f32(bias, "bias"), _f32(slope, "slope"), _bits(bits, M, K), float(p),
                                                       lib.stream_ptr()), "gemm_tf32x3_prelu_f32")
    return out


def gemm_tf32x3_prelu_bwd(a: torch.Tensor, b_hi: torch.Tensor, b_lo: torch.Tensor, out: torch.Tensor, z: torch.Tensor,
                          bits: torch.Tensor, slope: torch.Tensor, p: float, slope_grad: torch.Tensor, partial: torch.Tensor,
                          accumulate: bool = False, slope_accumulate: bool = False) -> torch.Tensor:
    M, K = a.shape
    N = b_hi.shape[0]
    assert out.shape == z.shape == (M, N) and out.stride(0) == z.stride(0)
    if partial.dtype != torch.float64 or not partial.is_cuda or partial.numel() < gemm_stat_slots(M, N):
        raise lib.B200GnnError("gemm_tf32x3_prelu_bwd: partial must be CUDA float64 [>= gemm_stat_slots(M, N)]")
    ap, lda = _rows(a, "a")
    op, ldc = _rows(out, "out")
    lib.check(lib.load().b200gnn_gemm_tf32x3_prelu_bwd_f32(ap, lda, _f32(b_hi, "b_hi"), _f32(b_lo, "b_lo"), b_hi.stride(0), op, ldc,
                                                           M, N, K, int(accumulate), _rows(z, "z")[0], _bits(bits, M, N),
                                                           _f32(slope, "slope"), float(p), slope_grad.data_ptr(),
                                                           int(slope_accumulate), partial.data_ptr(), partial.numel(),
                                                           lib.stream_ptr()), "gemm_tf32x3_prelu_bwd_f32")
    return out


WGRAD_PRELU_BLOCK = 512


def gemm_wgrad_tf32x3_prelu(z: torch.Tensor, slope: torch.Tensor, bits: torch.Tensor, p: float, g: torch.Tensor,
                            out: Optional[torch.Tensor] = None, workspace: Optional[torch.Tensor] = None) -> torch.Tensor:
    nn_, k_in = z.shape
    n_out = g.shape[1]
    assert g.shape[0] == nn_
    if k_in % 4 or n_out % 4:
        raise lib.B200GnnError(f"gemm_wgrad_tf32x3_prelu: Kin={k_in}, Nout={n_out} must be multiples of 4")
    L = lib.load()
    if out is None:
        out = torch.empty(k_in, n_out, dtype=torch.float32, device=z.device)
    blk = k_in if k_in <= 2048 else WGRAD_PRELU_BLOCK
    if workspace is None:
        workspace = torch.empty(wgrad_workspace_floats(blk, n_out), dtype=torch.float32, device=z.device)
    bp, ldb = _bits_rows(bits, nn_, k_in)
    gp, ldg = _rows(g, "g")
    assert out.is_contiguous()
    for c0 in range(0, k_in, blk):
        kb = min(blk, k_in - c0)
        zb, ldz = _rows(z[:, c0:c0 + kb], "z")
        lib.check(L.b200gnn_gemm_wgrad_tf32x3_prelu_f32(zb, ldz, gp, ldg, out[c0:c0 + kb].data_ptr(), nn_, kb, n_out,
                                                        _f32(slope, "slope"), bp + 4 * (c0 // 32), ldb, float(p),
                                                        _f32(workspace, "workspace"), lib.stream_ptr()),
                  "gemm_wgrad_tf32x3_prelu_f32")
    return out


def gemm_wgrad_tf32x3_rows(x: torch.Tensor, g: torch.Tensor, out: torch.Tensor, workspace: torch.Tensor) -> torch.Tensor:
    nn_, k_in = x.shape
    xp, ldx = _rows(x, "x")
    gp, ldg = _rows(g, "g")
    lib.check(lib.load().b200gnn_gemm_wgrad_tf32x3_f32(xp, ldx, gp, ldg, _f32(out, "out"), nn_, k_in, g.shape[1],
                                                       _f32(workspace, "workspace"), lib.stream_ptr()), "gemm_wgrad_tf32x3_f32")
    return out


def gemm_tf32x3_rows(a: torch.Tensor, b_hi: torch.Tensor, b_lo: torch.Tensor, out: torch.Tensor,
                     bias: Optional[torch.Tensor] = None) -> torch.Tensor:
    M, K = a.shape
    N = b_hi.shape[0]
    ap, lda = _rows(a, "a")
    op, ldc = _rows(out, "out")
    lib.check(lib.load().b200gnn_gemm_tf32x3_f32(ap, lda, _f32(b_hi, "b_hi"), _f32(b_lo, "b_lo"), b_hi.stride(0), op, ldc, M, N, K,
                                                 _f32(bias, "bias"), lib.stream_ptr()), "gemm_tf32x3_f32")
    return out


def col_sum_ld(y: torch.Tensor, out: torch.Tensor, partial: Optional[torch.Tensor] = None) -> torch.Tensor:
    n, K = y.shape
    L = lib.load()
    slots = int(L.b200gnn_col_sum_ld_slots(n))
    if partial is None:
        partial = torch.empty(slots * K, dtype=torch.float32, device=y.device)
    yp, ldy = _rows(y, "y")
    lib.check(L.b200gnn_col_sum_ld_f32(yp, ldy, n, K, _f32(out, "out"), partial.data_ptr(), partial.numel() // K, lib.stream_ptr()),
              "col_sum_ld_f32")
    return out


def sign_gather(feats, idx: torch.Tensor, p: float, seed: int, offset: int, out: torch.Tensor,
                step_dev: Optional[torch.Tensor] = None, step_mul: int = 0, labels: Optional[torch.Tensor] = None,
                labels_out: Optional[torch.Tensor] = None, teacher: Optional[torch.Tensor] = None,
                teacher_out: Optional[torch.Tensor] = None) -> torch.Tensor:
    H = len(feats)
    B = idx.numel()
    n, F_ = feats[0].shape
    for f in feats:
        if f.shape != (n, F_):
            raise lib.B200GnnError("sign_gather: every hop feature matrix must have the same shape")
        _f32(f, "feats")
    assert out.shape == (H, B, F_)
    C = teacher.shape[1] if teacher is not None else 0
    lib.check(lib.load().b200gnn_sign_gather_f32(
        _host_ptr_array([f.data_ptr() for f in feats]), H, n, F_, lib.dptr(idx, torch.int64, "idx"), B, float(p), int(seed),
        int(offset), lib.dptr(step_dev, torch.int32, "step_dev"), int(step_mul), _f32(out, "out"),
        lib.dptr(labels, torch.int64, "labels"), lib.dptr(labels_out, torch.int64, "labels_out"),
        _f32(teacher, "teacher"), teacher.stride(0) if teacher is not None else 0, C, _f32(teacher_out, "teacher_out"),
        lib.stream_ptr()), "sign_gather_f32")
    return out


def dropout_mask_step(mask: torch.Tensor, p: float, seed: int, offset: int, step_dev: torch.Tensor, step_mul: int) -> torch.Tensor:
    assert mask.dtype == torch.uint8 and mask.is_contiguous() and mask.numel() % 4 == 0
    lib.check(lib.load().b200gnn_dropout_mask_step_u8(mask.data_ptr(), mask.numel() // 4, 4, p, seed, offset,
                                                      lib.dptr(step_dev, torch.int32, "step_dev"), step_mul, lib.stream_ptr()),
              "dropout_mask_step_u8")
    return mask


def gat_scores(ft: torch.Tensor, attn_l: torch.Tensor, attn_r: Optional[torch.Tensor], src_scale: Optional[torch.Tensor],
               H: int, el: Optional[torch.Tensor] = None, er: Optional[torch.Tensor] = None):
    n, K = ft.shape
    fp, ldf = _rows(ft, "ft")
    el = torch.empty(n, H, dtype=torch.float32, device=ft.device) if el is None else el
    if attn_r is not None and er is None:
        er = torch.empty(n, H, dtype=torch.float32, device=ft.device)
    lib.check(lib.load().b200gnn_gat_scores_f32(fp, ldf, _f32(attn_l, "attn_l"), _f32(attn_r, "attn_r"), _f32(src_scale, "src_scale"),
                                                n, H, K // H, _f32(el, "el"), _f32(er, "er") if attn_r is not None else None,
                                                lib.stream_ptr()), "gat_scores_f32")
    return el, (er if attn_r is not None else None)


def gat_scores_slots(n_rows: int) -> int:
    return int(lib.load().b200gnn_gat_scores_slots(n_rows))


def gat_scores_bwd(ft: torch.Tensor, attn_l: torch.Tensor, attn_r: Optional[torch.Tensor], src_scale: Optional[torch.Tensor],
                   d_el: torch.Tensor, d_er: Optional[torch.Tensor], H: int, dft: torch.Tensor, d_attn_l: torch.Tensor,
                   d_attn_r: Optional[torch.Tensor], partial: Optional[torch.Tensor] = None) -> None:
    n, K = ft.shape
    fp, ldf = _rows(ft, "ft")
    dp, ldd = _rows(dft, "dft")
    if partial is None:
        partial = torch.empty(gat_scores_slots(n), 2, K, dtype=torch.float32, device=ft.device)
    lib.check(lib.load().b200gnn_gat_scores_bwd_f32(
        fp, ldf, _f32(attn_l, "attn_l"), _f32(attn_r, "attn_r"), _f32(src_scale, "src_scale"), _f32(d_el, "d_el"),
        _f32(d_er, "d_er") if attn_r is not None else None, n, H, K // H, dp, ldd, _f32(d_attn_l, "d_attn_l"),
        _f32(d_attn_r, "d_attn_r") if attn_r is not None else None, _f32(partial, "partial"), partial.shape[0],
        lib.stream_ptr()), "gat_scores_bwd_f32")


def gat_stat_slots(g: CsrGraph) -> int:
    return int(lib.load().b200gnn_gat_stat_slots(g.n_chunks, g.n_hub))


def gat_aggregate_epi(g: CsrGraph, eidx: Optional[torch.Tensor], a: torch.Tensor, ft: torch.Tensor, out: torch.Tensor, H: int,
                      src_scale: Optional[torch.Tensor] = None, row_scale: Optional[torch.Tensor] = None,
                      res: Optional[torch.Tensor] = None, bias: Optional[torch.Tensor] = None,
                      stat_partial: Optional[torch.Tensor] = None) -> torch.Tensor:
    K = ft.shape[1]
    fp, ldf = _rows(ft, "ft")
    op, ldo = _rows(out, "out")
    rp, ldr = _rows(res, "res") if res is not None else (None, 0)
    ws = g.hub_workspace(K)
    lib.check(lib.load().b200gnn_gat_aggregate_epi_f32(
        g.rowptr.data_ptr(), g.col.data_ptr(), lib.dptr(eidx, torch.int32, "eidx"), _f32(a, "a"), fp, ldf, op, ldo, g.n_rows, H,
        K // H, _f32(src_scale, "src_scale"), _f32(row_scale, "row_scale"), rp, ldr, _f32(bias, "bias"),
        _f32(stat_partial, "stat_partial"), 0 if stat_partial is None else stat_partial.shape[0],
        g.chunk_rowptr.data_ptr(), g.n_chunks, g.hub_threshold, g.seg_len,
        g.hub_rows.data_ptr() if g.n_hub else None, g.hub_segptr.data_ptr() if g.n_hub else None, g.n_hub, g.n_seg,
        None if ws is None else ws.data_ptr(), lib.stream_ptr()), "gat_aggregate_epi_f32")
    return out


def gat_aggregate_elu(g: CsrGraph, a: torch.Tensor, ft: torch.Tensor, out: torch.Tensor, act: torch.Tensor, H: int,
                      res: Optional[torch.Tensor] = None, bias: Optional[torch.Tensor] = None) -> Tuple[torch.Tensor, torch.Tensor]:
    K = ft.shape[1]
    fp, ldf = _rows(ft, "ft")
    op, ldo = _rows(out, "out")
    ap, lda = _rows(act, "act")
    rp, ldr = _rows(res, "res") if res is not None else (None, 0)
    ws = g.hub_workspace(K)
    lib.check(lib.load().b200gnn_gat_aggregate_elu_f32(
        g.rowptr.data_ptr(), g.col.data_ptr(), None, _f32(a, "a"), fp, ldf, op, ldo, ap, lda, g.n_rows, H, K // H, rp, ldr,
        _f32(bias, "bias"), g.chunk_rowptr.data_ptr(), g.n_chunks, g.hub_threshold, g.seg_len,
        g.hub_rows.data_ptr() if g.n_hub else None, g.hub_segptr.data_ptr() if g.n_hub else None, g.n_hub, g.n_seg,
        None if ws is None else ws.data_ptr(), lib.stream_ptr()), "gat_aggregate_elu_f32")
    return out, act

# ... 121 lines not shown
```

include/b200gnn.h:

```cpp
#ifndef B200GNN_H_
#define B200GNN_H_

#include <stdint.h>

#ifdef __cplusplus
extern "C" {
#endif

#define B200GNN_OK 0
#define B200GNN_ERR_BAD_ARG (-1)
#define B200GNN_ERR_UNSUPPORTED (-2)
#define B200GNN_ERR_CUDA (-3)

#define B200GNN_REDUCE_SUM 0
#define B200GNN_REDUCE_MEAN 1

#define B200GNN_ABI_VERSION 2

int b200gnn_abi_version(void);
const char* b200gnn_error_string(int code);
const char* b200gnn_last_cuda_error(void);
int64_t b200gnn_launch_count(void);
void b200gnn_reset_launch_count(void);

int64_t b200gnn_csr_chunk_count(int64_t n_rows, int64_t nnz, int32_t chunk_nnz,
                                int32_t row_cost);
int b200gnn_csr_chunk_plan(const int32_t* rowptr, int64_t n_rows, int64_t nnz,
                           int32_t chunk_nnz, int32_t row_cost,
                           int32_t* chunk_rowptr, void* stream);

int b200gnn_csr_hub_count(const int32_t* rowptr, int64_t n_rows,
                          int32_t hub_threshold, int32_t seg_len,
                          int32_t* counts_out, void* stream);
int b200gnn_csr_hub_fill(const int32_t* rowptr, int64_t n_rows,
                         int32_t hub_threshold, int32_t seg_len,
                         int32_t* hub_rows, int32_t* hub_segptr,
                         int64_t n_hub, void* stream);

int64_t b200gnn_spmm_stat_slots(int64_t n_chunks, int64_t n_hub);
void b200gnn_spmm_set_variant(int variant);
int b200gnn_spmm_csr_f32(const int32_t* rowptr, const int32_t* col,
                         const float* val, const float* X, int64_t ldx,
                         float* Y, int64_t ldy, int64_t n_rows, int64_t n_src,
                         int64_t K, int reduce, const float* bias,
                         float* stat_partial, const int32_t* chunk_rowptr,
                         int64_t n_chunks, int32_t hub_threshold,
                         int32_t seg_len, const int32_t* hub_rows,
                         const int32_t* hub_segptr, int64_t n_hub,
                         int64_t n_seg, float* hub_workspace, void* stream);
int b200gnn_spmm_csr_scatter_f32(const int32_t* rowptr, const int32_t* col, const float* val, const float* X,
                                 int64_t ldx, float* const* Y_ptrs, const int32_t* row_off, int32_t world,
                                 int64_t ldy_dst, int64_t col_dst, int64_t n_rows, int64_t n_src, int64_t K,
                                 int reduce, const float* bias, const int32_t* chunk_rowptr, int64_t n_chunks,
                                 int32_t hub_threshold, int32_t seg_len, const int32_t* hub_rows,
                                 const int32_t* hub_segptr, int64_t n_hub, int64_t n_seg,
                                 float* hub_workspace, void* stream);

int64_t b200gnn_rows_slots(int64_t n_rows);
int b200gnn_col_stats_f32(const float* Y, int64_t n_rows, int64_t K,
                          float* partial, int64_t slots, void* stream);
int b200gnn_col_sum_f32(const float* Y, int64_t n_rows, int64_t K, float* out,
                        float* partial, int64_t slots, void* stream);
int b200gnn_bn_finalize_f32(const float* partial, int64_t slots, int64_t K,
                            int64_t n_rows, const float* gamma,
                            const float* beta, float eps, float momentum,
                            float* running_mean, float* running_var,
                            float* mean_out, float* invstd_out,
                            float* scale_out, float* shift_out, void* stream);
int b200gnn_affine_relu_dropout_f32(const float* Y, float* out, int64_t n_rows,
                                    int64_t K, const float* scale,
                                    const float* shift, int relu, float p,
                                    uint64_t seed, uint64_t offset,
                                    const int32_t* step_dev, uint64_t step_mul,
                                    uint64_t row_offset, void* stream);
int b200gnn_affine_relu_dropout_mapped_f32(const float* Y, float* out, int64_t n_rows, int64_t K,
                                           const float* scale, const float* shift, int relu, float p,
                                           uint64_t seed, uint64_t offset, const int32_t* step_dev,
                                           uint64_t step_mul, const int32_t* rowmap, uint64_t row_offset,
                                           int64_t K_global, int64_t col_offset, void* stream);
int b200gnn_affine_relu_dropout_scatter_f32(const float* Y, float* out, int64_t n_rows, int64_t K,
                                            const float* scale, const float* shift, int relu, float p,
                                            uint64_t seed, uint64_t offset, const int32_t* step_dev,
                                            uint64_t step_mul, const int32_t* rowmap, uint64_t row_offset,
                                            int64_t K_global, int64_t col_offset, float* const* dst_ptrs,
                                            const int32_t* row_off, int32_t world, int64_t ld_dst, void* stream);
int b200gnn_dropout_mask_u8(uint8_t* mask, int64_t n_rows, int64_t K, float p,
                            uint64_t seed, uint64_t offset, void* stream);
int b200gnn_dropout_mask_step_u8(uint8_t* mask, int64_t n_rows, int64_t K, float p, uint64_t seed, uint64_t offset,
                                 const int32_t* step_dev, uint64_t step_mul, void* stream);
int b200gnn_dropout_bits_u32(uint32_t* bits, int64_t n_layers, int64_t n_rows, int64_t K, float p, uint64_t seed,
                             uint64_t offset, const int32_t* step_dev, uint64_t step_mul, void* stream);
int b200gnn_affine_relu_bits_f32(const float* Y, const uint32_t* bits, const float* scale, const float* shift,
                                 float p, float* out, int64_t n_rows, int64_t K, void* stream);
int b200gnn_gather_rows_act_f32(const float* X, int64_t ldx, const int64_t* idx, int64_t n_idx, int64_t K,
                                const uint32_t* bits, const float* scale, const float* shift, float p, float* out,
                                void* stream);
int b200gnn_relu_dropout_bwd_f32(const float* dOut, const float* Xout, float* dY,
                                 int64_t n_rows, int64_t K, float p, void* stream);
int b200gnn_bn_act_bwd_f32(const float* dOut, const float* Xout, const float* Y,
                           const float* mean, const float* invstd,
                           const float* gamma, int64_t n_rows, int64_t K,
                           float p, float* dY, float* dgamma, float* dbeta,
                           float* dbias, float* partial, int64_t slots,
                           float* coef, void* stream);
int b200gnn_bn_act_bwd_reduce_f32(const float* dOut, const float* Xout,
                                  const float* Y, const float* mean,
                                  const float* invstd, int64_t n_rows,
                                  int64_t K, float p, float* partial,
                                  int64_t slots, void* stream);
int b200gnn_bn_act_bwd_apply_f32(const float* dOut, const float* Xout,
                                 const float* Y, const float* mean,
                                 const float* invstd, const float* gamma,
                                 const float* sums, int64_t sum_slots,
                                 int64_t n_norm, int64_t n_rows, int64_t K,
                                 float p, float* dY, float* dgamma,
                                 float* dbeta, float* dbias, float* partial,
                                 int64_t slots, float* coef, void* stream);
int b200gnn_partial_reduce_f32(const float* partial, int64_t slots, int64_t K2,
                               float* out, void* stream);
int b200gnn_adam_step_f32(float* params, const float* grads, float* exp_avg,
                          float* exp_avg_sq, int64_t n, float lr, float beta1,
                          float beta2, float eps, int32_t* step, void* stream);
int b200gnn_rmsprop_step_f32(float* params, const float* grads, float* square_avg, int64_t n, double lr, int64_t warmup,
                             double alpha, double eps, double weight_decay, int32_t* step, void* stream);

int64_t b200gnn_teacher_slots(int64_t n_items);
int b200gnn_label_inputs_f32(float* X, int64_t ldx, int64_t col0, int64_t C, int64_t n_rows, const int32_t* row_pos,
                             const int64_t* labels, int eval, float mask_rate, uint64_t seed, uint64_t offset,
                             const int32_t* step_dev, uint64_t step_mul, const uint8_t* mask_in, int use_labels, uint8_t* role,
                             int32_t* cnt_part, void* stream);
int b200gnn_label_softmax_f32(const float* logits, int64_t ld, int64_t C, int64_t n_rows, const uint8_t* role, int role_mask,
                              float* out, int64_t ldo, void* stream);
int b200gnn_logce_fwd_bwd_f32(const float* logits, int64_t ld, int64_t C, const int64_t* train_idx, int64_t n_train,
                              const int64_t* labels, const uint8_t* role, const int32_t* cnt_part, int64_t n_cnt,
                              float* dlogits, int64_t ldd, float* loss_out, float* acc_out, double* partial, void* stream);
int b200gnn_split_eval_f32(const float* logits, int64_t ld, int64_t C, const int64_t* idx, int64_t n0, int64_t n1, int64_t n2,
                           const int64_t* labels, float* loss_out, float* acc_out, double* partial, void* stream);
int b200gnn_snapshot_if_better_f32(const float* cand, float* best, const float* src0, float* dst0, int64_t n0,
                                   const float* src1, float* dst1, int64_t n1, const float* src2, float* dst2, int64_t n2,
                                   void* stream);

int64_t b200gnn_kd_partials(int64_t n_train);
int b200gnn_kd_loss_fwd_bwd_f32(const float* logits, int64_t ld,
                                const int64_t* train_idx, int64_t n_train,
                                const int64_t* labels,
                                const float* teacher_logits, int64_t ldt,
                                int64_t C, float alpha, float T,
                                int64_t n_norm, float* dlogits, int64_t ldd,
                                float* loss_out, float* partial, void* stream);

int b200gnn_split_tf32_f32(const float* W, int64_t rows, int64_t cols,
                           int transpose, float* hi, float* lo, void* stream);
int b200gnn_gemm_tf32x3_f32(const float* A, int64_t lda, const float* B_hi,
                            const float* B_lo, int64_t ldb, float* C,
                            int64_t ldc, int64_t M, int64_t N, int64_t K,
                            const float* bias, void* stream);
int b200gnn_gemm_tf32x3_acc_f32(const float* A, int64_t lda, const float* B_hi, const float* B_lo,
                                int64_t ldb, float* C, int64_t ldc, int64_t M, int64_t N, int64_t K,
                                void* stream);
int b200gnn_gemm_tf32x3_rowidx_f32(const float* A, int64_t lda, const float* B_hi, const float* B_lo,
                                   int64_t ldb, float* C, int64_t ldc, int64_t M, int64_t N, int64_t K,
                                   const int64_t* row_idx, void* stream);
int64_t b200gnn_gemm_stat_slots(int64_t M, int64_t N);
void b200gnn_gemm_set_bnbwd_variant(int v);
int b200gnn_gemm_tf32x3_stats_f32(const float* A, int64_t lda, const float* B_hi, const float* B_lo, int64_t ldb,
                                  float* C, int64_t ldc, int64_t M, int64_t N, int64_t K, const float* bias,
                                  int accumulate, float* partial, int64_t slots, void* stream);
int b200gnn_gemm_tf32x3_bnbwd_f32(const float* A, int64_t lda, const float* B_hi, const float* B_lo, int64_t ldb,
                                  float* C, int64_t ldc, int64_t M, int64_t N, int64_t K, int accumulate,
                                  const float* Xout, const float* Y, const float* mean, const float* invstd, float p_drop,
                                  float* partial, int64_t slots, void* stream);
int b200gnn_gemm_tf32x3_bnbwd_bits_f32(const float* A, int64_t lda, const float* B_hi, const float* B_lo, int64_t ldb,
                                       float* C, int64_t ldc, int64_t M, int64_t N, int64_t K, int accumulate,
                                       const uint32_t* bits, const float* Y, const float* mean, const float* invstd,
                                       const float* scale, const float* shift, float p_drop, float* partial,
                                       int64_t slots, void* stream);
int b200gnn_gemm_tf32x3_act_f32(const float* Y, int64_t lda, const float* B_hi, const float* B_lo, int64_t ldb,
                                float* C, int64_t ldc, int64_t M, int64_t N, int64_t K, const float* bias,
                                const float* scale, const float* shift, const uint32_t* bits, float p_drop,
                                void* stream);
int b200gnn_gemm_tf32x3_scatter_f32(const float* A, int64_t lda, const float* B_hi, const float* B_lo,
                                    int64_t ldb, float* const* C_ptrs, int32_t world, int64_t row_off,
                                    int64_t M, int64_t N, int64_t K, const float* bias, void* stream);
int b200gnn_gemm_tf32x3_bcast_f32(const float* A, int64_t lda, const float* B_hi, const float* B_lo,
                                  int64_t ldb, float* const* C_ptrs, int32_t world, int64_t row_off, int64_t ldc,
                                  int64_t M, int64_t N, int64_t K, const float* bias, void* stream);

int64_t b200gnn_wgrad_workspace_floats(int64_t Kin, int64_t Nout);
int b200gnn_gemm_wgrad_tf32x3_f32(const float* X, int64_t ldx, const float* G,
                                  int64_t ldg, float* dW, int64_t Nn,
                                  int64_t Kin, int64_t Nout, float* workspace,
                                  void* stream);
int b200gnn_gemm_wgrad_tf32x3_act_f32(const float* Y, int64_t ldx, const float* G, int64_t ldg, float* dW,
                                      int64_t Nn, int64_t Kin, int64_t Nout, const float* scale, const float* shift,
                                      const uint32_t* bits, float p_drop, float* workspace, void* stream);

int b200gnn_gemm_tf32x3_prelu_f32(const float* Z, int64_t lda, const float* B_hi, const float* B_lo, int64_t ldb,
                                  float* C, int64_t ldc, int64_t M, int64_t N, int64_t K, const float* bias,
                                  const float* slope, const uint32_t* bits, float p_drop, void* stream);
int b200gnn_gemm_tf32x3_prelu_bwd_f32(const float* A, int64_t lda, const float* B_hi, const float* B_lo, int64_t ldb,
                                      float* C, int64_t ldc, int64_t M, int64_t N, int64_t K, int accumulate,
                                      const float* Z, const uint32_t* bits, const float* slope, float p_drop,
                                      float* slope_grad, int slope_accumulate, double* partial, int64_t slots,
                                      void* stream);
int b200gnn_gemm_wgrad_tf32x3_prelu_f32(const float* Z, int64_t ldz, const float* G, int64_t ldg, float* dW,
                                        int64_t Nn, int64_t Kin, int64_t Nout, const float* slope,
                                        const uint32_t* bits, int64_t ldbits, float p_drop, float* workspace,
                                        void* stream);
int b200gnn_prelu_bits_f32(const float* Z, int64_t ldz, const uint32_t* bits, int64_t ldbits, const float* slope, float p,
                           float* out, int64_t ldo, int64_t n_rows, int64_t K, void* stream);
int b200gnn_sign_gather_f32(const float* const* feats, int32_t n_hops, int64_t n_nodes, int64_t F, const int64_t* idx,
                            int64_t B, float p, uint64_t seed, uint64_t offset, const int32_t* step_dev,
                            uint64_t step_mul, float* out, const int64_t* labels, int64_t* labels_out,
                            const float* teacher, int64_t ldt, int64_t C, float* teacher_out, void* stream);
int64_t b200gnn_col_sum_ld_slots(int64_t n_rows);
int b200gnn_col_sum_ld_f32(const float* Y, int64_t ldy, int64_t n_rows, int64_t K, float* out, float* partial,
                           int64_t slots, void* stream);

int b200gnn_row_normalize_fwd_f32(const float* x, int64_t n, int64_t F, float eps,
                                  float scale, float* out, float* norm_out,
                                  void* stream);
int b200gnn_row_normalize_bwd_f32(const float* out, const float* norm,
                                  const float* d_out, int64_t n, int64_t F,
                                  float eps, float scale, float* d_x,
                                  int accumulate, void* stream);
int64_t b200gnn_reduce_slots(int64_t n);
int b200gnn_mse_fwd_bwd_f32(const float* a, const float* b, int64_t n,
                            float grad_weight, float* d_a, float* loss_out,
                            float* partial, void* stream);
int b200gnn_bce_logits_fwd_bwd_f32(const float* z, const float* target,
                                   int target_is_logits, int64_t n,
                                   float grad_weight, float* d_z, float* loss_out,
                                   float* partial, void* stream);
int b200gnn_row_sqnorm_f32(const float* x, int64_t n, int64_t F, float* out, void* stream);
int b200gnn_row_sqnorm_bwd_f32(const float* x, const float* d_out, int64_t n,
                               int64_t F, float* d_x, void* stream);
int b200gnn_nce_rows_f32(float* Z, int64_t S, float* loss_out, float* partial, void* stream);
int b200gnn_nce_rows_chunk_f32(float* Z, int64_t ldz, int64_t n_rows, int64_t S, int64_t row_offset,
                               float* partial, void* stream);
int b200gnn_nce_finish_f32(const float* partial, int64_t S, float* loss_out, void* stream);
int64_t b200gnn_gcrd_sample_workspace_bytes(int64_t n);
int b200gnn_gcrd_sample_i32(int64_t n, uint64_t seed, uint64_t offset, const int32_t* step_dev, int32_t* perm_out,
                            void* workspace, void* stream);
int b200gnn_gcrd_operands_f32(const int32_t* inds, int64_t S, int64_t P, const float* pre_s, const float* bn_s,
                              const float* pre_t, const float* bn_t, float inv_T, float eps, float* x_s, float* x_t,
                              float* norm_s, float* norm_t, void* stream);
int64_t b200gnn_gcrd_bwd_slots(void);
int b200gnn_gcrd_backward_f32(const int32_t* inds, int64_t S, int64_t P, const float* g_s, const float* g_t,
                              const float* x_s, const float* x_t, const float* norm_s, const float* norm_t, float inv_T,
                              float eps, const float* pre_s, const float* bn_s, const float* pre_t, const float* bn_t,
                              float beta, float* dz_s, float* dz_t, float* part_s, float* part_t, const float* loss_aux,
                              float* loss_total, void* stream);
int b200gnn_transpose_f32(const float* in, int64_t rows, int64_t cols, float* out, void* stream);
int b200gnn_gsp_pair_f32(float* Gs, const float* Gt, const float* ns, const float* nt,
                         int64_t S, int kernel, float* rowcoef, float* loss_out,
                         float* partial, void* stream);
int b200gnn_gsp_pair_chunk_f32(float* Gs, float* Gt, int64_t ld, int64_t n_rows, int64_t S, int64_t row_offset,
                               const float* ns, const float* nt, int kernel, float* rc_s, float* rc_t, float* partial,
                               void* stream);
int b200gnn_gsp_finish_f32(const float* partial, int64_t S, float* loss_out, void* stream);
int b200gnn_gsp_operands_f32(const int32_t* inds, int64_t S, int64_t P, int kernel, const float* pre_s, const float* bn_s,
                             const float* pre_t, const float* bn_t, float eps, float* x_s, float* x_t, float* norm_s,
                             float* norm_t, void* stream);
int b200gnn_gsp_backward_f32(const int32_t* inds, int64_t S, int64_t P, int kernel, const float* g_s, const float* g_t,
                             const float* x_s, const float* x_t, const float* norm_s, const float* norm_t, const float* rc_s,
                             const float* rc_t, float eps, const float* pre_s, const float* bn_s, const float* pre_t,
                             const float* bn_t, float beta, float* dz_s, float* dz_t, float* part_s, float* part_t,
                             const float* loss_aux, float* loss_total, void* stream);
#define B200GNN_GSP_ROWS_MAX_F 2048
int b200gnn_gsp_sim_chunk_f32(const float* G, int64_t ldg, int64_t n_rows, int64_t n, int64_t row_offset, const float* sq,
                              int kernel, float* sim, int64_t ld_sim, void* stream);
int b200gnn_gsp_pair_fixed_chunk_f32(float* Gs, int64_t ld, int64_t n_rows, int64_t S, int64_t row_offset, const float* ns,
                                     const float* sim_t, int64_t ld_t, int64_t n_t, const int32_t* inds, int kernel,
                                     float* rc_s, float* partial, void* stream);
int b200gnn_gsp_rows_operands_f32(const float* feat, int64_t ldf, const int32_t* inds, int64_t S, int64_t F, int kernel,
                                  float eps, float* x, int64_t ldx, float* norm, void* stream);
int b200gnn_gsp_rows_backward_f32(const int32_t* inds, int64_t S, int64_t F, int kernel, const float* g, const float* x,
                                  int64_t ldx, const float* norm, const float* rc, float eps, float beta, float* d_feat,
                                  int64_t ldd, const float* loss_aux, float* loss_total, void* stream);
int b200gnn_row_axpy_f32(const float* x, const float* coef, int64_t n, int64_t F,
                         float alpha, float* y, void* stream);

int b200gnn_edge_sim_f32(const float* feat, int64_t F, const int32_t* src,
                         const int32_t* dst, int64_t E, int kernel, float* sim,
                         void* stream);
int64_t b200gnn_lsp_partials(int64_t n_seg);
int b200gnn_lsp_segment_f32(const float* sim_s, const float* sim_t,
                            const int32_t* rowptr, int64_t n_seg, int64_t E,
                            int criterion, float* g, float* loss_out,
                            float* partial, void* stream);
int b200gnn_edge_sim_bwd_f32(const float* feat, int64_t F, const int32_t* src,
                             const int32_t* dst, int64_t E, int kernel,
                             const float* sim, const float* g, float* dfeat,
                             void* stream);
int b200gnn_lsp_bwd_values_f32(const float* feat, int64_t F, const int32_t* src, const int32_t* dst,
                               int64_t E, int kernel, const float* sim, const float* g,
                               const int32_t* pos_dst, const int32_t* pos_src,
                               const int32_t* comb_rowptr, const int32_t* diag_pos, int64_t n_nodes,
                               float* val, float* selfc, void* stream);
#define B200GNN_LSP_MAX_F 512
int b200gnn_lsp_student_f32(const float* feat, int64_t F, const int32_t* src, const int32_t* dst, const int32_t* rowptr,
                            int64_t n_seg, int64_t E, const float* sim_t, int kernel, const int32_t* pos_dst,
                            const int32_t* pos_src, const int32_t* comb_rowptr, const int32_t* diag_pos, int64_t n_nodes,
                            float* sim_s, float* scratch, float* val, float* selfc, float* loss_out, float* partial,
                            void* stream);
int b200gnn_scatter_rows_scaled_f32(const float* src, const int64_t* idx, int64_t n, int64_t K, float scale, float* dst,
                                    int64_t ldd, const float* loss_aux, float* loss_total, void* stream);

int b200gnn_gat_edge_softmax_f32(const int32_t* rowptr, const int32_t* col,
                                 const float* el, const float* er, int64_t n_rows,
                                 int64_t H, float negative_slope, float softmax_eps,
                                 float* a, const uint8_t* edge_keep, void* stream);
int b200gnn_gat_aggregate_f32(const int32_t* rowptr, const int32_t* col,
                              const int32_t* eidx, const float* a, const float* ft,
                              int64_t ldf, float* out, int64_t ldo, int64_t n_rows,
                              int64_t H, int64_t D, const int32_t* chunk_rowptr,
                              int64_t n_chunks, int32_t hub_threshold, int32_t seg_len,
                              const int32_t* hub_rows, const int32_t* hub_segptr,
                              int64_t n_hub, int64_t n_seg, float* hub_workspace,
                              void* stream);
int b200gnn_gat_bwd_rows_f32(const int32_t* rowptr, const int32_t* col, const float* a,
                             const float* ft, int64_t ldf, const float* dout,
                             int64_t ldd, const float* el, const float* er,
                             int64_t n_rows, int64_t H, int64_t D,
                             float negative_slope, float* dpre, float* der,
                             const int32_t* chunk_rowptr, int64_t n_chunks,
                             int32_t hub_threshold, int32_t seg_len,
                             const int32_t* hub_rows, const int32_t* hub_segptr,
                             int64_t n_hub, int64_t n_seg, float* hub_workspace,
                             const float* attn_scale, void* stream);
int b200gnn_segment_sum_heads_f32(const int32_t* rowptr, const int32_t* eidx,
                                  const float* vals, int64_t n_rows, int64_t H,
                                  float* out, void* stream);

int b200gnn_gat_scores_f32(const float* ft, int64_t ldf, const float* attn_l, const float* attn_r,
                           const float* src_scale, int64_t n_rows, int64_t H, int64_t D, float* el, float* er,
                           void* stream);
int64_t b200gnn_gat_scores_slots(int64_t n_rows);
int b200gnn_gat_scores_bwd_f32(const float* ft, int64_t ldf, const float* attn_l, const float* attn_r,
                               const float* src_scale, const float* d_el, const float* d_er, int64_t n_rows,
                               int64_t H, int64_t D, float* dft, int64_t ldd, float* d_attn_l, float* d_attn_r,
                               float* partial, int64_t slots, void* stream);
int64_t b200gnn_gat_stat_slots(int64_t n_chunks, int64_t n_hub);
int b200gnn_gat_aggregate_epi_f32(const int32_t* rowptr, const int32_t* col, const int32_t* eidx, const float* a,
                                  const float* ft, int64_t ldf, float* out, int64_t ldo, int64_t n_rows, int64_t H,
                                  int64_t D, const float* src_scale, const float* row_scale, const float* res,
                                  int64_t ldr, const float* bias, float* stat_partial, int64_t stat_slots,
                                  const int32_t* chunk_rowptr, int64_t n_chunks, int32_t hub_threshold,
                                  int32_t seg_len, const int32_t* hub_rows, const int32_t* hub_segptr, int64_t n_hub,
                                  int64_t n_seg, float* hub_workspace, void* stream);

int b200gnn_gat_aggregate_elu_f32(const int32_t* rowptr, const int32_t* col, const int32_t* eidx, const float* a,
                                  const float* ft, int64_t ldf, float* out, int64_t ldo, float* act, int64_t lda,
                                  int64_t n_rows, int64_t H, int64_t D, const float* res, int64_t ldr,
                                  const float* bias, const int32_t* chunk_rowptr, int64_t n_chunks,
                                  int32_t hub_threshold, int32_t seg_len, const int32_t* hub_rows,
                                  const int32_t* hub_segptr, int64_t n_hub, int64_t n_seg, float* hub_workspace,
                                  void* stream);
int b200gnn_elu_bwd_f32(const float* dA, int64_t ldda, const float* Z, int64_t ldz, float* dZ, int64_t lddz,
                        int64_t n_rows, int64_t K, void* stream);
int64_t b200gnn_ppi_tail_slots(int64_t n_rows);
int b200gnn_ppi_logits_loss_f32(const float* agg, int64_t lda, const float* res, int64_t ldr, const float* b_conv,
                                const float* b_lin, int64_t n_rows, int64_t H, int64_t Dp, int64_t C,
                                float* logits, int64_t ldl, const float* labels, int64_t ldy,
                                const float* teacher_logits, int64_t ldt, float alpha, float T, float* d_agg,
                                int64_t ldga, float* d_res, int64_t ldgr, float* loss_out, double* partial,
                                int64_t slots, void* stream);

typedef struct b200gnn_copy2d {
  float* dst;
  const float* src;
  int64_t ld_dst;
  int64_t ld_src;
  int64_t rows;
} b200gnn_copy2d;
int b200gnn_arena_alloc(int64_t bytes, void** out);
int b200gnn_arena_free(void* ptr);
int b200gnn_ipc_get_handle(const void* dev_ptr, void* handle64);
int b200gnn_ipc_open_handle(const void* handle64, void** out);
int b200gnn_ipc_close_handle(void* ptr);
int b200gnn_peer_copy2d_f32(const b200gnn_copy2d* copies, int32_t n, int64_t width, void* stream);
int b200gnn_peer_barrier(uint64_t* const* peer_flags, int32_t rank, int32_t world,
                         uint64_t* epoch, int32_t* error, void* stream);
int b200gnn_peer_exchange_f32(const b200gnn_copy2d* copies, int32_t n, int64_t width,
                              uint64_t* const* peer_flags, int32_t rank, int32_t world, uint64_t* epoch,
                              int32_t* error, uint32_t* ticket, void* stream);

int b200gnn_typed_gather_f32(const float* const* tables, const int64_t* table_rows, int32_t n_tables,
                             const int64_t* node_type, const int64_t* local_idx, int64_t n, int64_t F,
                             float* out, int64_t ldo, int32_t* error_flag, void* stream);
int b200gnn_embedding_adam_f32(const float* d_out, int64_t ldd, const int64_t* node_type,
                               const int64_t* local_idx, const int64_t* order, int64_t n,
                               int64_t table_type, float* table, float* exp_avg, float* exp_avg_sq,
                               int64_t rows, int64_t F, int32_t* head, float lr, float beta1,
                               float beta2, float eps, const int32_t* step, void* stream);
int b200gnn_typed_scatter_f32(const float* d_out, int64_t ldd, const int64_t* node_type,
                              const int64_t* local_idx, const int64_t* order, int64_t n, int64_t F,
                              float* const* d_tables, const int64_t* table_rows, int32_t n_tables,
                              void* stream);

int64_t b200gnn_graph_sort_workspace_bytes(int64_t n);
int b200gnn_graph_argsort_i64(const int64_t* major, const int64_t* minor, int64_t n, int64_t major_size,
                              int64_t minor_size, int32_t* perm_out, void* workspace, void* stream);
int b200gnn_graph_coalesce_i64(const int64_t* row, const int64_t* col, int64_t n, int64_t n_rows,
                               int64_t n_cols, int64_t* out_row, int64_t* out_col, int32_t* src_out,
                               int64_t* rowptr_out, int64_t* nnz_out, void* workspace, void* stream);

int b200gnn_random_walk_i64(const int32_t* rowptr, const int32_t* col, int64_t n_nodes, const int64_t* start,
                            int64_t n_walks, int32_t walk_length, uint64_t seed, uint64_t offset, int64_t* out,
                            void* stream);
int b200gnn_saint_subgraph_count_i64(const int32_t* rowptr, const int32_t* col, const int64_t* nodes, int64_t n_sel,
                                     int32_t* node_map, int64_t* counts, void* stream);
int b200gnn_saint_subgraph_fill_i64(const int32_t* rowptr, const int32_t* col, const int64_t* eid, const int64_t* nodes,
                                    int64_t n_sel, const int32_t* node_map, const int64_t* out_ptr, int64_t* out_row,
                                    int64_t* out_col, int64_t* out_eid, void* stream);

#ifdef __cplusplus
}
#endif
#endif
```

Before: 3.963 billion.

## Fuse batchnorm backward dY computation and bias grad into wgrad GEMM

Adds a BNBWD variant of the TF32x3 weight-gradient kernel. It loads dZ and Y through TMA, recomputes the batchnorm-backward dY on the fly before splitting into hi/lo, and accumulates the bias gradient in slot-partitioned partials that the reduce kernel sums. A separate bn_bwd_finalize entry point lets the model compute the coefficients without materializing dY for the weight gradient, removing a full read/write pass. The BNBWD path uses fewer pipeline stages (3 instead of 5) to make room for Y tiles, and it adds complex bias-span bookkeeping and extra producer iterations for the bias tail.

```diff
diff --git a/efficient-gnns_b200/csrc/common.cuh b/efficient-gnns_b200/csrc/common.cuh
--- a/efficient-gnns_b200/csrc/common.cuh
+++ b/efficient-gnns_b200/csrc/common.cuh
@@ -27,6 +27,11 @@
   const float vi = b2 * v + (1.f - b2) * g * g;
   m = mi; v = vi;
   p -= step_size * mi / (sqrtf(vi) * inv_sqrt_bc2 + eps);
+}
+
+__device__ __forceinline__ float bn_bwd_dy(float dz, float y, float mean, float invstd, float c1, float c2, float c3) {
+  const float xhat = __fmul_rn(__fsub_rn(y, mean), invstd);
+  return __fmul_rn(c1, __fmaf_rn(-xhat, c3, __fsub_rn(dz, c2)));
 }
 
 template <typename V> struct VecTraits;
diff --git a/efficient-gnns_b200/csrc/dense_rows.cu b/efficient-gnns_b200/csrc/dense_rows.cu
--- a/efficient-gnns_b200/csrc/dense_rows.cu
+++ b/efficient-gnns_b200/csrc/dense_rows.cu
@@ -387,10 +387,10 @@
         g.z = x.z > 0.f ? g.z * inv_keep : 0.f; g.w = x.w > 0.f ? g.w * inv_keep : 0.f;
       }
       float4 d;
-      d.x = c1.x * (g.x - c2.x - (y.x - mu.x) * is.x * c3.x);
-      d.y = c1.y * (g.y - c2.y - (y.y - mu.y) * is.y * c3.y);
-      d.z = c1.z * (g.z - c2.z - (y.z - mu.z) * is.z * c3.z);
-      d.w = c1.w * (g.w - c2.w - (y.w - mu.w) * is.w * c3.w);
+      d.x = bn_bwd_dy(g.x, y.x, mu.x, is.x, c1.x, c2.x, c3.x);
+      d.y = bn_bwd_dy(g.y, y.y, mu.y, is.y, c1.y, c2.y, c3.y);
+      d.z = bn_bwd_dy(g.z, y.z, mu.z, is.z, c1.z, c2.z, c3.z);
+      d.w = bn_bwd_dy(g.w, y.w, mu.w, is.w, c1.w, c2.w, c3.w);
       st4(dY + o, d);
       s.x += d.x; s.y += d.y; s.z += d.z; s.w += d.w;
     }
@@ -683,6 +683,16 @@
   return B200GNN_OK;
 }
 
+extern "C" int b200gnn_bn_bwd_finalize_f32(const float* sums, int64_t sum_slots, int64_t n_norm, int64_t K, const float* gamma,
+                                           const float* invstd, float* dgamma, float* dbeta, float* coef, void* stream) {
+  if (!sums || !gamma || !invstd || !dgamma || !dbeta || !coef || sum_slots < 1 || sum_slots >= INT32_MAX || n_norm < 1 ||
+      K < 1 || K >= INT32_MAX / 3)
+    return B200GNN_ERR_BAD_ARG;
+  bn_bwd_finalize_kernel<<<(int)((K + FIN_COLS - 1) / FIN_COLS), 256, 0, (cudaStream_t)stream>>>(
+      sums, (int)sum_slots, (int)K, n_norm, gamma, invstd, dgamma, dbeta, coef);
+  return check_launch();
+}
+
 extern "C" int b200gnn_bn_act_bwd_f32(const float* dOut, const float* Xout, const float* Y, const float* mean,
                                       const float* invstd, const float* gamma, int64_t n_rows, int64_t K, float p,
                                       float* dY, float* dgamma, float* dbeta, float* dbias, float* partial,
diff --git a/efficient-gnns_b200/csrc/gemm_wgrad_tf32x3.cu b/efficient-gnns_b200/csrc/gemm_wgrad_tf32x3.cu
--- a/efficient-gnns_b200/csrc/gemm_wgrad_tf32x3.cu
+++ b/efficient-gnns_b200/csrc/gemm_wgrad_tf32x3.cu
@@ -1,5 +1,7 @@
 #include "common.cuh"
 #include "tc_common.cuh"
+
+#include <type_traits>
 
 namespace b200gnn {
 namespace wgrad {
@@ -8,17 +10,21 @@
 constexpr int BKN = 32;
 constexpr int TM = 128, TN = 128;
 constexpr int THREADS = 384;
-constexpr int STAGES = 5;
 constexpr int X_BOX = 8;
-constexpr int RAW_BYTES = BKN * (TM + TN) * 4;
 constexpr int OP_BYTES = 128 * BKN * 4;
 constexpr int T_BYTES = 2 * OP_BYTES;
 constexpr int SS_BYTES = TM / 2 * 16;
-constexpr int SMEM_BYTES = STAGES * RAW_BYTES + 2 * T_BYTES + 256 + SS_BYTES + 1024;
+constexpr int MAX_RG = 8;
+constexpr int CB_BYTES = (5 + MAX_RG) * TN * 4 + 16;
+template <bool BNBWD> struct Ring {
+  static constexpr int STAGES = BNBWD ? 3 : 5;
+  static constexpr int RAW_BYTES = BKN * (TM + TN * (BNBWD ? 2 : 1)) * 4;
+  static constexpr int SMEM_BYTES = STAGES * RAW_BYTES + 2 * T_BYTES + 256 + SS_BYTES + (BNBWD ? CB_BYTES : 0) + 1024;
+  static_assert(SMEM_BYTES <= 232448, "shared memory");
+};
 constexpr int MAX_RANGES = 132;
 constexpr int64_t MAX_PARTIAL_FLOATS = (int64_t)MAX_RANGES * 256 * 256;
 constexpr int MAX_KIN = 2048, MAX_NOUT = 512;
-static_assert(SMEM_BYTES <= 232448, "shared memory");
 
 struct Params {
   float* partial;
@@ -31,23 +37,41 @@
   float inv_keep;
   const float* act_slope;
   int32_t act_ld;
+  const float* bn_mean;
+  const float* bn_invstd;
+  const float* bn_coef;
+  float* bias_partial;
+  int32_t bias_slots, bias_per, bias_rg;
 };
 
-template <bool ACT, bool PRELU = false>
+__device__ __forceinline__ void bias_span(const Params& p, int kb0, int kb1, int& s_a, int& s_b, int& kbe) {
+  const int64_t n0 = (int64_t)kb0 * BKN, n1 = min((int64_t)kb1 * BKN, (int64_t)p.Nn);
+  s_a = (int)((n0 + p.bias_per - 1) / p.bias_per);
+  s_b = min((int)((n1 + p.bias_per - 1) / p.bias_per) - 1, p.bias_slots - 1);
+  const int64_t end = s_a <= s_b ? min((int64_t)(s_b + 1) * p.bias_per, (int64_t)p.Nn) : 0;
+  kbe = max(kb1, (int)((end + BKN - 1) / BKN));
+}
+
+template <bool ACT, bool PRELU = false, bool BNBWD = false>
 __global__ void __launch_bounds__(THREADS, 1)
-wgrad_tf32x3_kernel(const __grid_constant__ CUtensorMap tmX, const __grid_constant__ CUtensorMap tmG, const Params p) {
+wgrad_tf32x3_kernel(const __grid_constant__ CUtensorMap tmX, const __grid_constant__ CUtensorMap tmG,
+                    const __grid_constant__ CUtensorMap tmY, const Params p) {
+  constexpr int STAGES = Ring<BNBWD>::STAGES, RAW_BYTES = Ring<BNBWD>::RAW_BYTES;
   extern __shared__ uint8_t smem_raw[];
   uint8_t* smem = reinterpret_cast<uint8_t*>((reinterpret_cast<uintptr_t>(smem_raw) + 1023) & ~(uintptr_t)1023);
   uint8_t* tbuf = smem + STAGES * RAW_BYTES;
   uint64_t* full = reinterpret_cast<uint64_t*>(tbuf + 2 * T_BYTES);
   uint64_t* empty = full + STAGES;
   float4* act_ss = reinterpret_cast<float4*>(tbuf + 2 * T_BYTES + 256);
+  float* cb = reinterpret_cast<float*>(tbuf + 2 * T_BYTES + 256 + SS_BYTES);
+  int* span = reinterpret_cast<int*>(cb + (5 + MAX_RG) * TN);
 
   const int tiles = (p.Kpad / TM) * p.n_tn;
   const int tile = (int)blockIdx.x % tiles, range = (int)blockIdx.x / tiles;
   const int mt = tile / p.n_tn, nt = tile % p.n_tn;
   const int kb0 = (int)((int64_t)p.num_kb * range / p.n_ranges);
   const int kb1 = (int)((int64_t)p.num_kb * (range + 1) / p.n_ranges);
+  const bool bias = BNBWD && mt == 0;
 
   const int warp = threadIdx.x >> 5, lane = threadIdx.x & 31;
   if (threadIdx.x == 0) {
@@ -60,13 +84,18 @@
     regs_dec<40>();
     if (threadIdx.x == 0) {
       int s = 0; uint32_t ph = 0;
-      for (int kb = kb0; kb < kb1; ++kb) {
+      int kbe = kb1;
+      if (bias) { int s_a, s_b; bias_span(p, kb0, kb1, s_a, s_b, kbe); }
+      for (int kb = kb0; kb < kbe; ++kb) {
         mbar_wait(&empty[s], ph ^ 1);
         uint8_t* st = smem + s * RAW_BYTES;
-        mbar_expect_tx(&full[s], RAW_BYTES);
-        for (int j = 0; j < TM / X_BOX; ++j)
-          tma_load_2d(&tmX, &full[s], st + j * BKN * X_BOX * 4, mt * TM + j * X_BOX, kb * BKN);
+        const bool x = kb < kb1;
+        mbar_expect_tx(&full[s], x ? RAW_BYTES : 2 * BKN * TN * 4);
+        if (x)
+          for (int j = 0; j < TM / X_BOX; ++j)
+            tma_load_2d(&tmX, &full[s], st + j * BKN * X_BOX * 4, mt * TM + j * X_BOX, kb * BKN);
         tma_load_2d(&tmG, &full[s], st + BKN * TM * 4, nt * TN, kb * BKN);
+        if (BNBWD) tma_load_2d(&tmY, &full[s], st + BKN * (TM + TN) * 4, nt * TN, kb * BKN);
         if (++s == STAGES) { s = 0; ph ^= 1; }
       }
     }
@@ -98,6 +127,70 @@
     if (kb0 < kb1) wnext = act_word(kb0);
     named_sync(1, 256);
   }
+  if (BNBWD) {
+    if (ct < TN) {
+      const int c = nt * TN + ct;
+      const bool in = c < p.Nout;
+      cb[ct] = in ? __ldg(p.bn_mean + c) : 0.f;
+      cb[TN + ct] = in ? __ldg(p.bn_invstd + c) : 0.f;
+      cb[2 * TN + ct] = in ? __ldg(p.bn_coef + c) : 0.f;
+      cb[3 * TN + ct] = in ? __ldg(p.bn_coef + p.Nout + c) : 0.f;
+      cb[4 * TN + ct] = in ? __ldg(p.bn_coef + 2 * p.Nout + c) : 0.f;
+    }
+    if (bias) {
+      for (int g = ct >> 7; g < p.bias_rg; g += 2) cb[(5 + g) * TN + (ct & (TN - 1))] = 0.f;
+      if (ct == 0) { int kbe; bias_span(p, kb0, kb1, span[0], span[1], kbe); }
+    }
+    named_sync(1, 256);
+  }
+  auto bias_rows = [&](auto rc, int kb, const float* rg) {
+    constexpr int R = decltype(rc)::value, H = R / 2;
+    const int s_a = span[0], s_b = span[1];
+    if (s_a > s_b) return;
+    const int h = ct >> 7, k = ct & (TN - 1), col = nt * TN + k;
+    const int per = p.bias_per, bs0 = s_a * per, bs1 = min((s_b + 1) * per, p.Nn);
+    const int nb0 = kb * BKN;
+    const int sc = max(nb0, bs0) / per;
+    const int nbd = (sc + 1) * per;
+    float c[H];
+#pragma unroll
+    for (int t = 0; t < H; ++t) c[t] = cb[(5 + h * H + t) * TN + k];
+    auto flush = [&](int sl) {
+      const int off = ((sl & (R - 1)) * (per & (R - 1))) & (R - 1);
+#pragma unroll
+      for (int t = 0; t < H; ++t) {
+        if (col < p.Nout) p.bias_partial[((size_t)sl * R + ((h * H + t - off) & (R - 1))) * p.Nout + col] = c[t];
+        c[t] = 0.f;
+      }
+    };
+    if (nb0 > bs0 && nb0 < bs1 && nb0 % per == 0) flush(nb0 / per - 1);
+    const float m = cb[k], is = cb[TN + k], c1 = cb[2 * TN + k], c2 = cb[3 * TN + k], c3 = cb[4 * TN + k];
+    bool flushed = false;
+#pragma unroll
+    for (int q = 0; q < BKN; q += R)
+#pragma unroll
+      for (int t = 0; t < H; ++t) {
+        const int j = q + h * H + t, n = nb0 + j;
+        const float g = bn_bwd_dy(rg[j * TN + k], rg[(BKN + j) * TN + k], m, is, c1, c2, c3);
+        if (n >= bs0 && n < bs1) {
+          if (n >= nbd && !flushed) { flush(sc); flushed = true; }
+          c[t] += g;
+        }
+      }
+    if (!flushed && nbd < nb0 + BKN && nbd < bs1) flush(sc);
+#pragma unroll
+    for (int t = 0; t < H; ++t) cb[(5 + h * H + t) * TN + k] = c[t];
+  };
+  auto bias_block = [&](int kb, const float* rg) {
+    if (p.bias_rg == 4) bias_rows(std::integral_constant<int, 4>{}, kb, rg);
+    else bias_rows(std::integral_constant<int, 8>{}, kb, rg);
+  };
+  auto flush_last = [&](int sl) {
+    const int R = p.bias_rg, H = R / 2, h = ct >> 7, k = ct & (TN - 1), col = nt * TN + k;
+    const int off = (int)(((int64_t)sl * p.bias_per) & (R - 1));
+    for (int t = 0; t < H; ++t)
+      if (col < p.Nout) p.bias_partial[((size_t)sl * R + ((h * H + t - off) & (R - 1))) * p.Nout + col] = cb[(5 + h * H + t) * TN + k];
+  };
   float acc[64], sum[64];
 #pragma unroll
   for (int i = 0; i < 64; ++i) sum[i] = acc[i] = 0.f;
@@ -119,14 +212,24 @@
     if (PRELU) asm volatile("" : "+r"(l4));
     const uint32_t sraw = smem_u32(smem + s * RAW_BYTES);
     const float* rg = reinterpret_cast<const float*>(smem + s * RAW_BYTES + BKN * TM * 4);
+    const int rem = p.Nn - (kb0 + i) * BKN;
     uint8_t* T = tbuf + (i & 1) * T_BYTES;
-#pragma unroll
+#pragma unroll (BNBWD ? 1 : 4)
     for (int u = 0; u < 4; ++u) {
       const int idx = u * 256 + ct;
       const int r = idx & 127, c = idx >> 7;
       const float* src = rg + (4 * c) * 128 + r;
-      const uint4 v = make_uint4(__float_as_uint(src[0]), __float_as_uint(src[128]), __float_as_uint(src[256]),
-                                 __float_as_uint(src[384]));
+      uint4 v = make_uint4(__float_as_uint(src[0]), __float_as_uint(src[128]), __float_as_uint(src[256]),
+                           __float_as_uint(src[384]));
+      if (BNBWD) {
+        const float* ys = src + BKN * TN;
+        const float m = cb[r], is = cb[TN + r], c1 = cb[2 * TN + r], c2 = cb[3 * TN + r], c3 = cb[4 * TN + r];
+        const float g0 = 4 * c < rem ? bn_bwd_dy(__uint_as_float(v.x), ys[0], m, is, c1, c2, c3) : 0.f;
+        const float g1 = 4 * c + 1 < rem ? bn_bwd_dy(__uint_as_float(v.y), ys[128], m, is, c1, c2, c3) : 0.f;
+        const float g2 = 4 * c + 2 < rem ? bn_bwd_dy(__uint_as_float(v.z), ys[256], m, is, c1, c2, c3) : 0.f;
+        const float g3 = 4 * c + 3 < rem ? bn_bwd_dy(__uint_as_float(v.w), ys[384], m, is, c1, c2, c3) : 0.f;
+        v = make_uint4(__float_as_uint(g0), __float_as_uint(g1), __float_as_uint(g2), __float_as_uint(g3));
+      }
       uint4 hv, lv;
       split4(v, hv, lv);
       *reinterpret_cast<uint4*>(T + swz128(r, c)) = hv;
@@ -150,13 +253,20 @@
         }
         split1(v, h[k][j], l[k][j]);
       }
-    asm volatile("fence.proxy.async.shared::cta;" ::: "memory");
-    mbar_arrive(&empty[s]);
+    if (!bias) {
+      asm volatile("fence.proxy.async.shared::cta;" ::: "memory");
+      mbar_arrive(&empty[s]);
+    }
     if (i > 0) {
       wgmma_wait<0>();
       acc_fence(acc);
 #pragma unroll
       for (int j = 0; j < 64; ++j) sum[j] += acc[j];
+    }
+    if (bias) {
+      bias_block(kb0 + i, rg);
+      asm volatile("fence.proxy.async.shared::cta;" ::: "memory");
+      mbar_arrive(&empty[s]);
     }
     named_sync(1, 256);
     reg_fence(h); reg_fence(l);
@@ -183,6 +293,18 @@
 #pragma unroll
     for (int j = 0; j < 64; ++j) sum[j] += acc[j];
   }
+  if (bias) {
+    int s_a, s_b, kbe;
+    bias_span(p, kb0, kb1, s_a, s_b, kbe);
+    for (int kb = kb1; kb < kbe; ++kb) {
+      mbar_wait(&full[s], ph);
+      bias_block(kb, reinterpret_cast<const float*>(smem + s * RAW_BYTES + BKN * TM * 4));
+      asm volatile("fence.proxy.async.shared::cta;" ::: "memory");
+      mbar_arrive(&empty[s]);
+      if (++s == STAGES) { s = 0; ph ^= 1; }
+    }
+    if (s_a <= s_b) flush_last(s_b);
+  }
   float* out = p.partial + (size_t)range * p.Kpad * p.Npad;
   const int row0 = mt * TM + cw * 64 + (warp & 3) * 16 + (lane >> 2);
 #pragma unroll
@@ -196,12 +318,40 @@
 }
 
 constexpr int RED_VECS = 32, RED_GROUPS = 8;
+constexpr int FIN_COLS = 4, FIN_GROUPS = 64;
+template <bool BIAS>
 __global__ void __launch_bounds__(RED_VECS * RED_GROUPS) wgrad_reduce_kernel(const float4* __restrict__ partial, int n_part,
                                                                              int Kin, int Kpad, int Nout, int Npad,
-                                                                             float* __restrict__ out) {
+                                                                             float* __restrict__ out,
+                                                                             const float* __restrict__ bias_part, int bias_slots,
+                                                                             int bias_per, int bias_rg, int Nn,
+                                                                             float* __restrict__ dbias) {
   __shared__ float4 sh[RED_GROUPS][RED_VECS];
   const int64_t n_vec = (int64_t)Kpad * Npad / 4;
   const int v = threadIdx.x % RED_VECS, g = threadIdx.x / RED_VECS;
+  if constexpr (BIAS) {
+    const int main_blocks = (int)((n_vec + RED_VECS - 1) / RED_VECS);
+    if ((int)blockIdx.x >= main_blocks) {
+      __shared__ double shb[FIN_GROUPS][FIN_COLS];
+      const int c = threadIdx.x % FIN_COLS, fg = threadIdx.x / FIN_COLS;
+      const int k = ((int)blockIdx.x - main_blocks) * FIN_COLS + c;
+      double a = 0.0;
+      if (k < Nout)
+        for (int j = fg; j < bias_slots; j += FIN_GROUPS) {
+          float P = 0.f;
+          if ((int64_t)j * bias_per < Nn)
+            for (int r = 0; r < bias_rg; ++r) P += __ldcs(bias_part + ((size_t)j * bias_rg + r) * Nout + k);
+          a += (double)P;
+        }
+      shb[fg][c] = a;
+      __syncthreads();
+      if (fg != 0 || k >= Nout) return;
+      a = 0.0;
+      for (int j = 0; j < FIN_GROUPS; ++j) a += shb[j][c];
+      dbias[k] = (float)a;
+      return;
+    }
+  }
   const int64_t i = (int64_t)blockIdx.x * RED_VECS + v;
   float4 acc = make_float4(0.f, 0.f, 0.f, 0.f);
   if (i < n_vec)
@@ -252,23 +402,28 @@
   return wgrad::range_cap(Kin, Nout) * wgrad::pad_k(Kin) * wgrad::pad_n(Nout);
 }
 
-template <bool ACT, bool PRELU = false>
+template <bool ACT, bool PRELU = false, bool BNBWD = false>
 static int wgrad_launch(const float* X, int64_t ldx, const float* G, int64_t ldg, float* dW, int64_t Nn, int64_t Kin, int64_t Nout,
-                        float* workspace, const wgrad::Params& act, void* stream) {
-  if (!X || !G || !dW || !workspace || Nn <= 0 || Kin <= 0 || Nout <= 0 || ldx < Kin || ldg < Nout || Nn >= INT32_MAX)
+                        float* workspace, const wgrad::Params& act, void* stream, const float* Y = nullptr,
+                        float* dbias = nullptr) {
+  using Ring = wgrad::Ring<BNBWD>;
+  if (!X || !G || !dW || !workspace || Nn <= 0 || Kin <= 0 || Nout <= 0 || ldx < Kin || ldg < Nout || Nn >= INT32_MAX ||
+      (BNBWD && (!Y || !dbias)))
     return B200GNN_ERR_BAD_ARG;
   if (Kin % 4 || Kin > wgrad::MAX_KIN || Nout % 4 || Nout > wgrad::MAX_NOUT || ldx % 4 || ldg % 4 || !aligned_to(X, 16) || !aligned_to(G, 16) ||
-      !aligned_to(dW, 16) || !aligned_to(workspace, 16))
+      !aligned_to(dW, 16) || !aligned_to(workspace, 16) || (BNBWD && !aligned_to(Y, 16)))
     return B200GNN_ERR_UNSUPPORTED;
-  CUtensorMap tX, tG;
+  CUtensorMap tX, tG, tY;
   if (!wgrad::make_map_rows(&tX, X, Nn, Kin, ldx, wgrad::X_BOX) || !wgrad::make_map_rows(&tG, G, Nn, Nout, ldg, wgrad::TN))
     return B200GNN_ERR_UNSUPPORTED;
+  if (BNBWD ? !wgrad::make_map_rows(&tY, Y, Nn, Nout, ldg, wgrad::TN) : false) return B200GNN_ERR_UNSUPPORTED;
+  if (!BNBWD) tY = tG;
   int dev = 0, sms = 132;
   cudaGetDevice(&dev);
   static bool attr_set[64] = {};
   if (dev >= 0 && dev < 64 && !attr_set[dev]) {
-    cudaError_t e = cudaFuncSetAttribute(wgrad::wgrad_tf32x3_kernel<ACT, PRELU>, cudaFuncAttributeMaxDynamicSharedMemorySize,
-                                         wgrad::SMEM_BYTES);
+    cudaError_t e = cudaFuncSetAttribute(wgrad::wgrad_tf32x3_kernel<ACT, PRELU, BNBWD>, cudaFuncAttributeMaxDynamicSharedMemorySize,
+                                         Ring::SMEM_BYTES);
     if (e != cudaSuccess) { set_cuda_error(e); return B200GNN_ERR_CUDA; }
     attr_set[dev] = true;
   }
@@ -287,12 +442,22 @@
   if (ranges > p.num_kb) ranges = p.num_kb;
   if (ranges < 1) ranges = 1;
   p.n_ranges = ranges;
+  float* bias_part = workspace + (size_t)cap * p.Kpad * p.Npad;
+  if (BNBWD) {
+    p.bias_partial = bias_part;
+    p.bias_slots = (int32_t)b200gnn_rows_slots(Nn);
+    p.bias_per = (int32_t)((Nn + p.bias_slots - 1) / p.bias_slots);
+    p.bias_rg = (int32_t)(1024 / Nout);
+  }
   int rc;
-  wgrad::wgrad_tf32x3_kernel<ACT, PRELU><<<tiles * ranges, wgrad::THREADS, wgrad::SMEM_BYTES, st>>>(tX, tG, p);
+  wgrad::wgrad_tf32x3_kernel<ACT, PRELU, BNBWD><<<tiles * ranges, wgrad::THREADS, Ring::SMEM_BYTES, st>>>(tX, tG, tY, p);
   if ((rc = check_launch())) return rc;
   const int64_t n_vec = (int64_t)p.Kpad * p.Npad / 4;
-  wgrad::wgrad_reduce_kernel<<<(int)((n_vec + wgrad::RED_VECS - 1) / wgrad::RED_VECS), wgrad::RED_VECS * wgrad::RED_GROUPS, 0, st>>>(
-      reinterpret_cast<const float4*>(workspace), ranges, (int)Kin, p.Kpad, (int)Nout, p.Npad, dW);
+  const int red_blocks = (int)((n_vec + wgrad::RED_VECS - 1) / wgrad::RED_VECS);
+  const int bias_blocks = BNBWD ? (int)((Nout + wgrad::FIN_COLS - 1) / wgrad::FIN_COLS) : 0;
+  wgrad::wgrad_reduce_kernel<BNBWD><<<red_blocks + bias_blocks, wgrad::RED_VECS * wgrad::RED_GROUPS, 0, st>>>(
+      reinterpret_cast<const float4*>(workspace), ranges, (int)Kin, p.Kpad, (int)Nout, p.Npad, dW, bias_part, p.bias_slots,
+      p.bias_per, p.bias_rg, (int)Nn, dbias);
   return check_launch();
 }
 
@@ -322,3 +487,20 @@
   act.inv_keep = p_drop > 0.f ? 1.f / (1.f - p_drop) : 1.f;
   return wgrad_launch<false, true>(Z, ldz, G, ldg, dW, Nn, Kin, Nout, workspace, act, stream);
 }
+
+constexpr int64_t BIAS_CHAIN_FLOATS = 528 * 1024;
+extern "C" int64_t b200gnn_wgrad_bnbwd_workspace_floats(int64_t Kin, int64_t Nout) {
+  const int64_t w = b200gnn_wgrad_workspace_floats(Kin, Nout);
+  return w < 0 ? w : w + BIAS_CHAIN_FLOATS;
+}
+
+extern "C" int b200gnn_gemm_wgrad_tf32x3_bnbwd_f32(const float* X, int64_t ldx, const float* dZ, const float* Y, int64_t ldg,
+                                                   float* dW, float* dbias, int64_t Nn, int64_t Kin, int64_t Nout,
+                                                   const float* mean, const float* invstd, const float* coef, float* workspace,
+                                                   void* stream) {
+  if (!mean || !invstd || !coef) return B200GNN_ERR_BAD_ARG;
+  if ((Nout != 128 && Nout != 256) || Nn >= (1 << 30)) return B200GNN_ERR_UNSUPPORTED;
+  wgrad::Params bn{};
+  bn.bn_mean = mean; bn.bn_invstd = invstd; bn.bn_coef = coef;
+  return wgrad_launch<false, false, true>(X, ldx, dZ, ldg, dW, Nn, Kin, Nout, workspace, bn, stream, Y, dbias);
+}
diff --git a/efficient-gnns_b200/engine.py b/efficient-gnns_b200/engine.py
--- a/efficient-gnns_b200/engine.py
+++ b/efficient-gnns_b200/engine.py
@@ -37,7 +37,8 @@
     def __init__(self, adj: SparseTensor, dims: List[int], dropout: float = 0.5, lr: float = 0.01, seed: int = 0,
                  alpha: float = 0.9, kd_T: float = 4.0, bn_eps: float = 1e-5, bn_momentum: float = 0.1,
                  aggregate_first: Optional[bool] = None, tensor_core_gemm: bool = True, overlap_wgrad: bool = True,
-                 fuse_row_passes: bool = True, fuse_activations: bool = True, _prebuilt_graph: Optional[CsrGraph] = None, _rows_alloc: Optional[int] = None,
+                 fuse_row_passes: bool = True, fuse_activations: bool = True, fuse_bn_wgrad: bool = True,
+                 _prebuilt_graph: Optional[CsrGraph] = None, _rows_alloc: Optional[int] = None,
                  gcrd=None, lsp=None, gsp=None):
         self.objective = one_objective(gcrd, lsp, gsp)
         assert adj.is_cuda(), "the engine runs on a CUDA device"
@@ -84,8 +85,10 @@
         self.W_split = [(torch.empty(dims[l], dims[l + 1], device=dev), torch.empty(dims[l], dims[l + 1], device=dev))
                         for l in range(self.L)]
         wg = [ops.wgrad_supported(dims[l], dims[l + 1]) for l in range(self.L)]
-        self.wgrad_ws = (torch.empty(max(ops.wgrad_workspace_floats(dims[l], dims[l + 1]) for l in range(self.L) if wg[l]), device=dev)
-                         if self.tc_gemm and any(wg) else None)
+        ws = [ops.wgrad_workspace_floats(dims[l], dims[l + 1]) for l in range(self.L) if wg[l]]
+        if ops.wgrad_bnbwd_supported(dims[0], dims[1]):
+            ws.append(ops.wgrad_bnbwd_workspace_floats(dims[0], dims[1]))
+        self.wgrad_ws = torch.empty(max(ws), device=dev) if self.tc_gemm and any(wg) else None
         self.running_mean = [torch.zeros(d, device=dev) for d in dims[1:-1]]
         self.running_var = [torch.ones(d, device=dev) for d in dims[1:-1]]
         self.reset_parameters(seed)
@@ -118,6 +121,8 @@
                          and all(ops.wgrad_supported(dims[l], dims[l + 1]) for l in range(1, self.L)))
         self.keep_bits = (torch.zeros(self.L - 1, N, (hid[0] + 31) // 32, dtype=torch.int32, device=dev)
                           if self.fuse_act else None)
+        self.fuse_bn_wgrad = (bool(fuse_bn_wgrad) and self.agg_first and ops.wgrad_bnbwd_supported(dims[0], dims[1])
+                              and dims[1] in self._gemm_part)
         self._act_stale = False
         self._fwd_fused = False
         self._ev_bits = torch.cuda.Event()
@@ -252,7 +257,8 @@
             if l == self.L - 1:
                 ops.col_sum(self.dY[l], out=self.gb[l], partial=self._part(self.dims[l + 1]))
             if l == 0 and self.agg_first:
-                self._wgrad_async(0, self.AX, self.dY[0])
+                if not self.fuse_bn_wgrad:
+                    self._wgrad_async(0, self.AX, self.dY[0])
                 continue
             ops.spmm_csr(self.Gt, self.dY[l], "sum", out=self.dH[l])
             d_prev = self.dA[l - 1] if l > 0 else None
@@ -275,7 +281,10 @@
             if l > 0:
                 k = self.dims[l]
                 part = self._part(k)
-                if gp is not None:
+                if gp is not None and l == 1 and self.fuse_bn_wgrad:
+                    ops.bn_bwd_finalize(gp, self.N, self.gamma[0], self.bn[0][1], self.ggamma[0], self.gbeta[0], self._coef(k))
+                    self._wgrad_async(0, self.AX, d_prev, bn=True)
+                elif gp is not None:
                     ops.bn_act_bwd_apply(d_prev, None, self.Y[l - 1], self.bn[l - 1][0], self.bn[l - 1][1], self.gamma[l - 1],
                                          gp, self.N, self.p, self.dY[l - 1], self.ggamma[l - 1], self.gbeta[l - 1],
                                          self.gb[l - 1], part, self._coef(k))
@@ -285,13 +294,13 @@
                                    d_beta=self.gbeta[l - 1], d_bias=self.gb[l - 1], partial=part, coef=self._coef(k))
         self._wgrad_join()
 
-    def _wgrad_async(self, l: int, inp: Optional[torch.Tensor], d_out: torch.Tensor, act=None):
+    def _wgrad_async(self, l: int, inp: Optional[torch.Tensor], d_out: torch.Tensor, act=None, bn: bool = False):
         if self._side is None:
-            return self._linear_wgrad(l, inp, d_out, act)
+            return self._linear_wgrad(l, inp, d_out, act, bn)
         self._ev_fork.record(torch.cuda.current_stream())
         self._side.wait_event(self._ev_fork)
         with torch.cuda.stream(self._side):
-            self._linear_wgrad(l, inp, d_out, act)
+            self._linear_wgrad(l, inp, d_out, act, bn)
 
     def _wgrad_join(self):
         if self._side is not None:
@@ -319,8 +328,11 @@
         else:
             torch.mm(d_out, self.W[l].t(), out=d_inp)
 
-    def _linear_wgrad(self, l: int, inp: Optional[torch.Tensor], d_out: torch.Tensor, act=None):
-        if act is not None:
+    def _linear_wgrad(self, l: int, inp: Optional[torch.Tensor], d_out: torch.Tensor, act=None, bn: bool = False):
+        if bn:
+            ops.gemm_wgrad_tf32x3_bnbwd(inp, d_out, self.Y[l], self.bn[l][0], self.bn[l][1], self._coef(self.dims[l + 1]),
+                                        out=self.gW[l], d_bias=self.gb[l], workspace=self.wgrad_ws)
+        elif act is not None:
             ops.gemm_wgrad_tf32x3_act(*act, self.p, d_out, out=self.gW[l], workspace=self.wgrad_ws)
         elif self.tc_gemm and ops.wgrad_supported(self.dims[l], self.dims[l + 1]):
             ops.gemm_wgrad_tf32x3(inp, d_out, out=self.gW[l], workspace=self.wgrad_ws)
diff --git a/efficient-gnns_b200/lib.py b/efficient-gnns_b200/lib.py
--- a/efficient-gnns_b200/lib.py
+++ b/efficient-gnns_b200/lib.py
@@ -63,6 +63,7 @@
     "b200gnn_bn_act_bwd_reduce_f32": (_int, [_f32p, _f32p, _f32p, _f32p, _f32p, _i64, _i64, _f32, _f32p, _i64, _ptr]),
     "b200gnn_bn_act_bwd_apply_f32": (_int, [_f32p, _f32p, _f32p, _f32p, _f32p, _f32p, _f32p, _i64, _i64, _i64, _i64, _f32,
                                             _f32p, _f32p, _f32p, _f32p, _f32p, _i64, _f32p, _ptr]),
+    "b200gnn_bn_bwd_finalize_f32": (_int, [_f32p, _i64, _i64, _i64, _f32p, _f32p, _f32p, _f32p, _f32p, _ptr]),
     "b200gnn_partial_reduce_f32": (_int, [_f32p, _i64, _i64, _f32p, _ptr]),
     "b200gnn_adam_step_f32": (_int, [_f32p, _f32p, _f32p, _f32p, _i64, _f32, _f32, _f32, _f32, _i32p, _ptr]),
     "b200gnn_rmsprop_step_f32": (_int, [_f32p, _f32p, _f32p, _i64, _f64, _i64, _f64, _f64, _f64, _i32p, _ptr]),
@@ -100,6 +101,9 @@
     "b200gnn_gemm_wgrad_tf32x3_f32": (_int, [_f32p, _i64, _f32p, _i64, _f32p, _i64, _i64, _i64, _f32p, _ptr]),
     "b200gnn_gemm_wgrad_tf32x3_act_f32": (_int, [_f32p, _i64, _f32p, _i64, _f32p, _i64, _i64, _i64, _f32p, _f32p, _ptr, _f32,
                                                  _f32p, _ptr]),
+    "b200gnn_wgrad_bnbwd_workspace_floats": (_i64, [_i64, _i64]),
+    "b200gnn_gemm_wgrad_tf32x3_bnbwd_f32": (_int, [_f32p, _i64, _f32p, _f32p, _i64, _f32p, _f32p, _i64, _i64, _i64, _f32p, _f32p,
+                                                   _f32p, _f32p, _ptr]),
     "b200gnn_gemm_tf32x3_prelu_f32": (_int, [_f32p, _i64, _f32p, _f32p, _i64, _f32p, _i64, _i64, _i64, _i64, _f32p,
                                              _f32p, _ptr, _f32, _ptr]),
     "b200gnn_gemm_tf32x3_prelu_bwd_f32": (_int, [_f32p, _i64, _f32p, _f32p, _i64, _f32p, _i64, _i64, _i64, _i64, _int,
diff --git a/efficient-gnns_b200/ops.py b/efficient-gnns_b200/ops.py
--- a/efficient-gnns_b200/ops.py
+++ b/efficient-gnns_b200/ops.py
@@ -475,6 +475,47 @@
                                                   float(p), _f32(workspace, "workspace"), lib.stream_ptr()),
               "gemm_wgrad_tf32x3_act_f32")
     return out
+
+
+def wgrad_bnbwd_supported(k_in: int, n_out: int) -> bool:
+    return wgrad_supported(k_in, n_out) and n_out in (128, 256)
+
+
+def wgrad_bnbwd_workspace_floats(k_in: int, n_out: int) -> int:
+    return int(lib.load().b200gnn_wgrad_bnbwd_workspace_floats(k_in, n_out))
+
+
+def gemm_wgrad_tf32x3_bnbwd(x: torch.Tensor, dz: torch.Tensor, y: torch.Tensor, mean: torch.Tensor, invstd: torch.Tensor,
+                            coef: torch.Tensor, out: Optional[torch.Tensor] = None, d_bias: Optional[torch.Tensor] = None,
+                            workspace: Optional[torch.Tensor] = None) -> Tuple[torch.Tensor, torch.Tensor]:
+    nn_, k_in = x.shape
+    n_out = dz.shape[1]
+    assert dz.shape[0] == nn_ and y.shape == dz.shape and y.stride(0) == dz.stride(0)
+    if not wgrad_bnbwd_supported(k_in, n_out):
+        raise lib.B200GnnError(f"gemm_wgrad_tf32x3_bnbwd: Kin={k_in}, Nout={n_out}: Kin must be 128 or 256 and Nout 128 or 256")
+    L = lib.load()
+    if out is None:
+        out = torch.empty(k_in, n_out, dtype=torch.float32, device=x.device)
+    if d_bias is None:
+        d_bias = torch.empty(n_out, dtype=torch.float32, device=x.device)
+    if workspace is None:
+        workspace = torch.empty(wgrad_bnbwd_workspace_floats(k_in, n_out), dtype=torch.float32, device=x.device)
+    lib.check(L.b200gnn_gemm_wgrad_tf32x3_bnbwd_f32(_f32(x, "x"), x.stride(0), _f32(dz, "dz"), _f32(y, "y"), dz.stride(0),
+                                                    _f32(out, "out"), _f32(d_bias, "d_bias"), nn_, k_in, n_out,
+                                                    _f32(mean, "mean"), _f32(invstd, "invstd"), _f32(coef, "coef"),
+                                                    _f32(workspace, "workspace"), lib.stream_ptr()),
+              "gemm_wgrad_tf32x3_bnbwd_f32")
+    return out, d_bias
+
+
+def bn_bwd_finalize(sums: torch.Tensor, n_norm: int, gamma: torch.Tensor, invstd: torch.Tensor, d_gamma: torch.Tensor,
+                    d_beta: torch.Tensor, coef: torch.Tensor) -> torch.Tensor:
+    K = gamma.numel()
+    sum_slots = sums.numel() // (2 * K)
+    lib.check(lib.load().b200gnn_bn_bwd_finalize_f32(_f32(sums, "sums"), sum_slots, n_norm, K, _f32(gamma, "gamma"),
+                                                     _f32(invstd, "invstd"), _f32(d_gamma, "d_gamma"), _f32(d_beta, "d_beta"),
+                                                     _f32(coef, "coef"), lib.stream_ptr()), "bn_bwd_finalize_f32")
+    return coef
 
 
 def partial_reduce(partial: torch.Tensor, out: Optional[torch.Tensor] = None) -> torch.Tensor:
diff --git a/include/b200gnn.h b/include/b200gnn.h
--- a/include/b200gnn.h
+++ b/include/b200gnn.h
@@ -116,6 +116,8 @@
                                  float p, float* dY, float* dgamma,
                                  float* dbeta, float* dbias, float* partial,
                                  int64_t slots, float* coef, void* stream);
+int b200gnn_bn_bwd_finalize_f32(const float* sums, int64_t sum_slots, int64_t n_norm, int64_t K, const float* gamma,
+                                const float* invstd, float* dgamma, float* dbeta, float* coef, void* stream);
 int b200gnn_partial_reduce_f32(const float* partial, int64_t slots, int64_t K2,
                                float* out, void* stream);
 int b200gnn_adam_step_f32(float* params, const float* grads, float* exp_avg,
@@ -194,6 +196,11 @@
 int b200gnn_gemm_wgrad_tf32x3_act_f32(const float* Y, int64_t ldx, const float* G, int64_t ldg, float* dW,
                                       int64_t Nn, int64_t Kin, int64_t Nout, const float* scale, const float* shift,
                                       const uint32_t* bits, float p_drop, float* workspace, void* stream);
+int64_t b200gnn_wgrad_bnbwd_workspace_floats(int64_t Kin, int64_t Nout);
+int b200gnn_gemm_wgrad_tf32x3_bnbwd_f32(const float* X, int64_t ldx, const float* dZ, const float* Y, int64_t ldg,
+                                        float* dW, float* dbias, int64_t Nn, int64_t Kin, int64_t Nout,
+                                        const float* mean, const float* invstd, const float* coef, float* workspace,
+                                        void* stream);
 
 int b200gnn_gemm_tf32x3_prelu_f32(const float* Z, int64_t lda, const float* B_hi, const float* B_lo, int64_t ldb,
                                   float* C, int64_t ldc, int64_t M, int64_t N, int64_t K, const float* bias,
```

Measured after the change: 4.000 billion (median of 6 runs). No clear change (+0.9%).
